# MarQuisCheshire/Pets-Face-Recognition

Measured on AMD Instinct MI355X. Metric: FE train images/sec @224^2 bs=256/GPU, higher is better.
Workload: dtype bf16; 1 GPU; resnet50 FE + ArcFace(s=64,m=0.5) + CE, 10000 ids, 224x224x3, fwd+bwd+SGD(momentum 0.9, param groups of the reference recipe); global_batch=256, per_gpu_batch=256, parallelism=dp1, rccl_ranks=0

## Files before the change

### include/pfr_hip.h

```cpp
#ifndef PFR_HIP_H
#define PFR_HIP_H
#include <stddef.h>
#include <stdint.h>

#ifdef __cplusplus
extern "C" {
#endif

#define PFR_F32 0
#define PFR_BF16 1
#define PFR_I8 2
#define PFR_OK 0
#define PFR_ERR_ARG (-1)
#define PFR_ERR_HIP (-2)
#define PFR_ERR_UNSUPPORTED (-3)

typedef void* pfr_stream_t;

const char* pfr_last_error(void);
int pfr_version(void);
int pfr_device_arch(char* buf, int buflen);
int pfr_set_tuning(const char* key, int value);
int pfr_get_tuning(const char* key, int* value);
int pfr_tuning_epoch(void);

int pfr_plan_thunk_index(const char* name);
void* pfr_plan_create(int n_events);
int pfr_plan_destroy(void* plan);
int pfr_plan_append(void* plan, int kind, int thunk, int ev, const unsigned long long* args, int nargs);
int pfr_plan_size(void* plan);
int pfr_plan_run(void* plan, int begin, int end, pfr_stream_t main_stream, pfr_stream_t side_stream, int hook_stops);

int pfr_conv2d_mtile(int N, int H, int W, int C, int Cout, int R, int S, int stride, int pad, int OH, int OW, int dtype,
                     int out_dtype, int fused_prologue);
int pfr_gemm_act_mtile(long M, int K, int N, int dtype);
int pfr_conv2d_fwd(const void* x, const void* w, void* y, int dtype, int out_dtype, int N, int H, int W, int C,
                   int Cout, int R, int S, int stride, int pad, int idil_log2, int OH, int OW, int ldy,
                   const float* bias, const void* residual, int accumulate, int out_relu, const float* pro_scale,
                   const float* pro_shift, int pro_relu, float* stats_part, pfr_stream_t stream);
int pfr_conv2d_dgrad_join(const void* dy, const void* wt, void* dx, int dtype, int N, int H, int W, int C, int Cout, int R,
                          int S, int pad, int idil_log2, int OH, int OW, const void* res, const unsigned char* res_mask,
                          pfr_stream_t stream);

int pfr_conv2d_dgrad_bn_parts(int dtype, int N, int H, int W, int C, int Cout, int R, int S, int idil_log2, int OH, int OW);
int pfr_conv2d_dgrad_bn(const void* dy, const void* wt, void* dx, int dtype, int N, int H, int W, int C, int Cout, int R, int S,
                        int pad, int idil_log2, int OH, int OW, const void* res, const unsigned char* res_mask, int accumulate,
                        const void* bn_x, const float* bn_coef, const unsigned char* bn_mask, float* bn_part, const void* bn2_x,
                        const float* bn2_coef, float* bn2_part, pfr_stream_t stream);

int pfr_conv2d_dgrad_bn_sub(const void* dy, const void* wt, void* dx, int dtype, int N, int H, int W, int C, int Cout, int OH, int OW,
                            const void* res_compact, const void* bn_x, const float* bn_coef, const unsigned char* bn_mask,
                            float* bn_part, pfr_stream_t stream);

int pfr_conv1x1_tail_mtile(int dtype, int N, int H, int W, int C, int Cout);
int pfr_conv1x1_stats(const void* x, const void* w, int dtype, int N, int H, int W, int C, int Cout, float* stats_part,
                      pfr_stream_t stream);
int pfr_conv1x1_bn_tail(const void* x, const void* w, void* y, unsigned char* mask, int dtype, int N, int H, int W, int C, int Cout,
                        const float* a1, const float* b1, const void* res, const float* a2, const float* b2, pfr_stream_t stream);

int pfr_conv2d_dgrad_bn_ex(const void* dy, const void* wt, void* dx, int dtype, int N, int H, int W, int C, int Cout, int R, int S,
                           int pad, int idil_log2, int OH, int OW, const void* res, const unsigned char* res_mask, int accumulate,
                           const void* bn_x, const float* bn_coef, const unsigned char* bn_mask, float* bn_part, const void* bn2_x,
                           const float* bn2_coef, float* bn2_part, int flags, pfr_stream_t stream);
int pfr_conv2d_dgrad_bn_sub_ex(const void* dy, const void* wt, void* dx, int dtype, int N, int H, int W, int C, int Cout, int OH, int OW,
                               const void* res_compact, const void* bn_x, const float* bn_coef, const unsigned char* bn_mask,
                               float* bn_part, int flags, pfr_stream_t stream);

int pfr_bn3_bwd_coef(const float* part, int nparts, const float* G1, const float* zsum, const void* W, int wdtype, const float* gamma,
                     const float* invstd, int C, int K, float count, float* dgamma, float* dbeta, float* coef, int accumulate,
                     pfr_stream_t stream);
int pfr_bn3_bwd_weights(const float* coef, const float* G1, const float* G2, const float* zsum, const void* W, int wdtype, int C, int K, float count,
                        float* dW, void* wa_t, void* S, float* bias, int accumulate, pfr_stream_t stream);
int pfr_conv1x1_dgrad2_bn_parts(int dtype, int N, int H, int W, int C1, int C2, int Cout);
int pfr_conv1x1_dgrad2_bn(const void* g, const void* z, const void* wcat, const float* bias, void* dx, int dtype, int N, int H, int W,
                          int C1, int C2, int Cout, const void* bn_x, const float* bn_coef, float* bn_part, pfr_stream_t stream);

int pfr_bn_stats_from_gram(const float* gram, const void* W, int dtype, int C, int K, float count, float* part, float eps, int* cancel_flag,
                           pfr_stream_t stream);
int pfr_bn_finalize_from_gram(const float* gram, const void* W, int dtype, int C, int K, float count, const float* gamma, const float* beta,
                              float eps, float momentum, float* running_mean, float* running_var, float* mean, float* invstd, float* scale,
                              float* shift, int* cancel_flag, pfr_stream_t stream);
long pfr_gram_ws_floats(long M, int Q);
int pfr_gram_colsum(const void* x, int dtype, long M, int Q, float* out, float* workspace, pfr_stream_t stream);

int pfr_conv2d_wgrad_splits(int M, int Cout, int KK);
int pfr_conv2d_wgrad(const void* x, const void* dy, float* dw, float* workspace, int dtype, int N, int H, int W, int C,
                     int Cout, int R, int S, int stride, int pad, int OH, int OW, int lddy, const float* pro_scale,
                     const float* pro_shift, int pro_relu, float scale, int accumulate, pfr_stream_t stream);

int pfr_nchw_to_nhwc(const float* x, void* y, int dtype, int N, int C, int H, int W, int Cp, pfr_stream_t stream);
int pfr_cast(const void* x, int src_dtype, void* y, int dst_dtype, size_t n, pfr_stream_t stream);
int pfr_weight_dgrad_layout(const void* w, void* wt, int dtype, int O, int R, int S, int I, pfr_stream_t stream);
int pfr_weight_dgrad_layout_batch(const void* descs, int n_layers, int dtype, pfr_stream_t stream);
int pfr_add(const void* a, const void* b, void* y, int dtype, size_t n, pfr_stream_t stream);
long pfr_colsum_ws_floats(long rows, int C);
int pfr_colsum(const void* x, int dtype, long rows, int C, float* out, int accumulate, float* workspace, pfr_stream_t stream);
int pfr_colsum_parts(int dtype, long rows, int C);
int pfr_colsum_partial(const void* x, int dtype, long rows, int C, float* workspace, pfr_stream_t stream);
int pfr_colsum_final_batch(const void* descs, int n, int max_C, pfr_stream_t stream);
int pfr_copy2d_f32(const float* src, int ld_src, float* dst, int ld_dst, long rows, int cols, float scale, int accumulate,
                   pfr_stream_t stream);

int pfr_colreduce_blocks(int C, int dtype, long rows);
int pfr_bn_stats(const void* x, int dtype, long rows, int C, float* part, pfr_stream_t stream);
long pfr_bn_stats_rows_per_part(int C, int dtype, long rows);
long pfr_bn_finalize_ws_floats(int nparts, int C);
int pfr_bn_finalize(const float* part, int nparts, long rows_per_part, int C, float count, const float* gamma,
                    const float* beta, float eps, float momentum, float* running_mean, float* running_var, float* mean,
                    float* invstd, float* scale, float* shift, float* workspace, pfr_stream_t stream);
int pfr_fold_bn(const void* descs, int ndesc, int dtype, pfr_stream_t stream);
int pfr_fold_bn_cached(const void* descs, int ndesc, int dtype, const float* master, size_t n_master, void* shadow,
                       unsigned long long* state, pfr_stream_t stream);
int pfr_bn_eval_coeff(int C, const float* gamma, const float* beta, const float* running_mean, const float* running_var,
                      float eps, float* scale, float* shift, pfr_stream_t stream);
int pfr_bn_act(const void* x1, const float* a1, const float* b1, const void* x2, const float* a2, const float* b2, void* y,
               int dtype, long rows, int C, int relu, pfr_stream_t stream);
int pfr_bn_act_mask(const void* x1, const float* a1, const float* b1, const void* x2, const float* a2, const float* b2,
                    void* y, unsigned char* mask, int dtype, long rows, int C, int relu, pfr_stream_t stream);
int pfr_bn_bwd_reduce(const void* dout, const void* out, const void* x, const float* mean, const float* invstd,
                      const float* scale, const float* shift, int mask_mode, int dtype, long rows, int C, float* part,
                      pfr_stream_t stream);
int pfr_bn_bwd_finalize(const float* part, int nparts, int C, float count, const float* gamma, const float* mean,
                        const float* invstd, float* dgamma, float* dbeta, float* coef, int accumulate, pfr_stream_t stream);
int pfr_bn_bwd_apply(const void* dout, const void* out, const void* x, const float* coef, const float* scale,
                     const float* shift, int mask_mode, void* dx, void* gres, int dtype, long rows, int C,
                     pfr_stream_t stream);

int pfr_bn_relu_maxpool_fwd(const void* x, const float* scale, const float* shift, void* y, uint8_t* idx, int dtype, int N,
                            int H, int W, int C, int relu, pfr_stream_t stream);
int pfr_maxpool_bwd(const void* dy, const uint8_t* idx, void* dz, int dtype, int N, int H, int W, int C, pfr_stream_t stream);
int pfr_avgpool_fwd(const void* x, void* y, int dtype, int N, int HW, int C, pfr_stream_t stream);
int pfr_avgpool_bwd(const void* dy, void* dx, int dtype, int N, int HW, int C, pfr_stream_t stream);

int pfr_s2d_input(const float* x, void* y, int dtype, int N, int C, int H, int W, int Cp, pfr_stream_t stream);
int pfr_s2d_weight(const float* w, void* ws, int dtype, int Cout, int C, int Cp, pfr_stream_t stream);
int pfr_s2d_wgrad(const float* dws, float* dw, int Cout, int C, int Cp, int accumulate, pfr_stream_t stream);
int pfr_transpose2d(const void* x, void* y, int dtype, int rows, int cols, pfr_stream_t stream);
int pfr_l2norm_dual(const float* x, void* xn_bf16, float* xn_f32, float* inv_norm, int rows, int D, float eps,
                    pfr_stream_t stream);
int pfr_l2norm_fwd(const void* x, int in_dtype, void* xn, void* xnT, int out_dtype, float* inv_norm, int rows, int D,
                   int ldt, float eps, pfr_stream_t stream);
int pfr_l2norm_bwd(const void* x, int in_dtype, const float* inv_norm, const float* dxn, void* dx, int out_dtype, int rows,
                   int D, int accumulate, pfr_stream_t stream);
int pfr_margin_ce(const float* cosv, const int64_t* label, int B, int C, int ldc, int mode, float s, float m, float gamma,
                  float grad_scale, const float* grad_scale_dev, float* logits, float* loss_rows, void* dcos, int dcos_dtype,
                  pfr_stream_t stream);
int pfr_margin_bwd(const float* cosv, const int64_t* label, int B, int C, int ldc, int mode, float s, float m,
                   const float* dlogits, void* dcos, int dcos_dtype, pfr_stream_t stream);
int pfr_mean(const float* x, float* out, int n, pfr_stream_t stream);

int pfr_sgd_step(float* p, const float* g, float* mom, void* shadow, int shadow_dtype, size_t n, float lr, float momentum,
                 float weight_decay, float grad_scale, int first_step, pfr_stream_t stream);
int pfr_adamw_step(float* p, const float* g, float* m, float* v, void* shadow, int shadow_dtype, size_t n, float lr,
                   float beta1, float beta2, float eps, float weight_decay, int step, float grad_scale, pfr_stream_t stream);
int pfr_sgd_step_clip(float* p, const float* g, float* mom, void* shadow, int shadow_dtype, size_t n, float lr, float momentum,
                      float weight_decay, float grad_scale, int first_step, const float* clip_coef, float clip_value,
                      pfr_stream_t stream);
int pfr_adamw_step_clip(float* p, const float* g, float* m, float* v, void* shadow, int shadow_dtype, size_t n, float lr,
                        float beta1, float beta2, float eps, float weight_decay, int step, float grad_scale,
                        const float* clip_coef, float clip_value, pfr_stream_t stream);
int pfr_grad_norm_chunk_elems(void);
int pfr_grad_norm(const void* segs, const int* chunk_seg, int nseg, long nchunks, float norm_p, float max_norm, double* ws,
                  float* out, pfr_stream_t stream);

int pfr_layernorm_fwd(const void* x, const float* gamma, const float* beta, void* y, float* mean, float* rstd, int dtype,
                      long rows, int C, float eps, pfr_stream_t stream);
int pfr_layernorm_bwd_blocks(long rows);
int pfr_layernorm_bwd(const void* dy, const void* x, const float* mean, const float* rstd, const float* gamma,
                      const void* dres, void* dx, float* part, int dtype, long rows, int C, pfr_stream_t stream);
int pfr_layernorm_bwd_dxsum(const void* dy, const void* x, const float* mean, const float* rstd, const float* gamma,
                            const void* dres, void* dx, float* part, float* dxsum_part, int dtype, long rows, int C,
                            pfr_stream_t stream);
int pfr_layernorm_bwd_dxsum_ok(int dtype, int C);
int pfr_gelu_fwd(const void* x, void* y, int dtype, size_t n, pfr_stream_t stream);
int pfr_gelu_bwd(const void* x, const void* dy, void* dx, int dtype, size_t n, pfr_stream_t stream);
long pfr_window_bias_table_floats(int window);
int pfr_window_bias_table(const float* pos, float* tab, int window, int shift, pfr_stream_t stream);
int pfr_window_bias_table_batch(const void* descs, int n, pfr_stream_t stream);
int pfr_window_attn_fwd(const void* qkv, const float* pos, void* out, int dtype, int B, int H, int W, int heads, int head_dim,
                        int window, int shift, float scale, pfr_stream_t stream);
int pfr_window_attn_bwd(const void* qkv, const float* pos, const void* dout, void* dqkv, float* dpos_part, int dtype, int B,
                        int H, int W, int heads, int head_dim, int window, int shift, float scale, pfr_stream_t stream);
int pfr_nhwc_to_nchw_f32(const float* x, float* y, int N, int C, int HW, int Cp, int accumulate, pfr_stream_t stream);

long pfr_topk_state_bytes(int rows, int K);
int pfr_topk_reset(void* state, int rows, int K, pfr_stream_t stream);
int pfr_topk_update(const float* scores, int rows, int ld, int n, int col0, int K, void* state, const int* self_idx,
                    pfr_stream_t stream);
int pfr_match_scores_filter(const void* q, const void* g, int dtype, int Q, int n, int D, int col0, int K, void* state,
                            void* cand, int cap, int exclude_self, pfr_stream_t stream);
int pfr_topk_merge(const void* cand, int cap, int rows, int K, void* state, pfr_stream_t stream);
int pfr_quantize_rows_i8(const float* x, void* q, int ldq, float* scale, float* xn_f32, float* inv_norm, int rows, int D, int normalize,
                         float eps, pfr_stream_t stream);
int pfr_match_scores_i8(const void* q, const float* q_scale, const void* g, const float* g_scale, int Q, int n, int Dp, float* out, int ld,
                        pfr_stream_t stream);
int pfr_match_scores_filter_i8(const void* q, const float* q_scale, const void* g, const float* g_scale, int Q, int n, int Dp, int col0,
                               int K, void* state, void* cand, int cap, int exclude_self, pfr_stream_t stream);
int pfr_topk_flags(const void* state, int rows, int K, int* out_host, pfr_stream_t stream);
int pfr_topk_finish(const void* state, int rows, int K, float* out_scores, int* out_idx, pfr_stream_t stream);
int pfr_topk_rescore(const float* q, const float* g, const float* g_scale, int rows, int D, const int* cand, int KC, int K,
                     float* out_scores, int* out_idx, pfr_stream_t stream);
int pfr_topk_rescore_cert(const float* q, const float* g, const float* g_scale, int rows, int D, const int* cand, const float* cand_scores,
                          int KC, int K, float* out_scores, int* out_idx, float* cert, pfr_stream_t stream);
int pfr_pair_similarity(const float* emb, int D, const long* idx_a, const long* idx_b, int P, float eps, float* out,
                        pfr_stream_t stream);

long pfr_pair_curve_ws_bytes(int P);
int pfr_pair_curve(const float* scores, const int* labels, int P, void* workspace, float* sorted_scores, int* cum_tp,
                   unsigned char* run_end, pfr_stream_t stream);

int pfr_card_centroids(const float* emb, const long* seg, int ncards, int D, float eps, float* cent32, void* cent,
                       int cent_dtype, pfr_stream_t stream);

int pfr_card_fuse_scores(float* head_scores, const float* body_scores, int rows, int ld, int n, int col0,
                         const unsigned char* q_flags, const unsigned char* g_flags, const float* thresholds, int n_types,
                         pfr_stream_t stream);

int pfr_augment_params(const int* flags, const float* angles, int N, int out_w, int out_h, int* records);
long pfr_augment_ws_bytes(int N, int H, int W);
int pfr_augment_train(const unsigned char* x, int N, int H, int W, int crop_h, int crop_w, int out_h, int out_w,
                      const int* records, float* y, void* ws, pfr_stream_t stream);

int pfr_gemm_act(const void* x, const void* w, void* y, int dtype, long M, int K, int N, const float* bias, int act,
                 void* y2, pfr_stream_t stream);
int pfr_gemm_act_colstats(const void* x, const void* w, void* y, int dtype, long M, int K, int N, const float* bias, int act,
                          void* y2, float* stats_part, pfr_stream_t stream);
int pfr_gemm_act_colsum_parts(long M, int K, int N, int dtype);
int pfr_gemm_act_colsums(const void* x, const void* w, void* y, int dtype, long M, int K, int N, void* y2, float* sums_part,
                         pfr_stream_t stream);

int pfr_comm_unique_id(void* id128);
void* pfr_comm_init(int rank, int world, const void* id128);
int pfr_comm_allreduce(void* comm, void* buf, size_t count, int dtype, int average, pfr_stream_t stream);
int pfr_comm_destroy(void* comm);

#ifdef __cplusplus
}
#endif
#endif
```

### pets-face-recognition_amd/_hip/lib.py

```python
import ctypes
import os
import re

PFR_F32, PFR_BF16, PFR_I8 = 0, 1, 2

_HERE = os.path.dirname(os.path.abspath(__file__))
_PKG = os.path.dirname(_HERE)
_ROOT = os.path.dirname(_PKG)
LIB_PATH = os.environ.get("PFR_LIB_PATH") or os.path.join(_PKG, "csrc", "libpfr_hip.so")
HEADER_PATH = os.path.join(_ROOT, "include", "pfr_hip.h")


class PfrError(RuntimeError):
    pass


_CTYPES = {
    "int": ctypes.c_int,
    "long": ctypes.c_long,
    "size_t": ctypes.c_size_t,
    "float": ctypes.c_float,
    "pfr_stream_t": ctypes.c_void_p,
}


def _ctype_of(decl: str):
    decl = decl.strip()
    if "*" in decl:
        if decl.replace("const", "").strip().startswith("char"):
            return ctypes.c_char_p
        return ctypes.c_void_p
    base = decl.replace("const", "").split()[0]
    return _CTYPES[base]


def parse_header(path=HEADER_PATH):
    src = open(path).read()
    src = re.sub(r"/\*.*?\*/", "", src, flags=re.S)
    src = re.sub(r"//[^\n]*", "", src)
    protos = {}
    for m in re.finditer(r"(const\s+char\s*\*|void\s*\*|int|long)\s+(pfr_\w+)\s*\(([^)]*)\)\s*;", src):
        ret, name, args = m.group(1), m.group(2), m.group(3).strip()
        restype = ctypes.c_char_p if "char" in ret else (ctypes.c_void_p if "void" in ret else (ctypes.c_long if ret == "long" else ctypes.c_int))
        argtypes, argnames = [], []
        if args and args != "void":
            for a in args.split(","):
                a = a.strip()
                nm = re.search(r"(\w+)$", a).group(1)
                argnames.append(nm)
                argtypes.append(_ctype_of(a[: -len(nm)]))
        protos[name] = (restype, argtypes, argnames)
    return protos


class _Lib:
    def __init__(self):
        self._dll = None
        self._protos = None

    def _load(self):
        if self._dll is not None:
            return
        if not os.path.exists(LIB_PATH):
            raise PfrError(
                f"{LIB_PATH} not found: build it with `python -c 'import __graft_entry__ as g; g.build()'` "
                f"(or pets-face-recognition_amd/csrc/build.sh). There is no CPU/PyTorch fallback for the HIP path."
            )
        import torch
        self._dll = ctypes.CDLL(LIB_PATH)
        self._protos = parse_header()
        for name, (restype, argtypes, _names) in self._protos.items():
            try:
                fn = getattr(self._dll, name)
            except AttributeError as e:
                raise PfrError(f"libpfr_hip.so does not export {name} declared in include/pfr_hip.h") from e
            fn.restype = restype
            fn.argtypes = argtypes
        for item in filter(None, (os.environ.get("PFR_TUNING") or "").replace(";", ",").split(",")):
            k, _, v = item.partition("=")
            if self._dll.pfr_set_tuning(k.strip().encode(), int(v)) != 0:
                raise PfrError(f"PFR_TUNING: {self._dll.pfr_last_error().decode()}")

    def __getattr__(self, name):
        if name.startswith("_"):
            raise AttributeError(name)
        self._load()
        if name not in self._protos:
            raise AttributeError(f"{name} is not declared in include/pfr_hip.h")
        fn = getattr(self._dll, name)
        if self._protos[name][0] is ctypes.c_int and name not in _NO_CHECK:
            def checked(*args, _fn=fn, _name=name):
                tr = _TRACER[0]
                if tr is not None:
                    tr.before(_name, args)
                rc = _fn(*args)
                if tr is not None:
                    tr.after(_name, args)
                if rc != 0:
                    raise PfrError(f"{_name} failed (rc={rc}): {self._dll.pfr_last_error().decode()}")
                return rc
            checked.__name__ = name
            setattr(self, name, checked)
            return checked
        setattr(self, name, fn)
        return fn

    def symbols(self):
        self._load()
        return dict(self._protos)


_NO_CHECK = {"pfr_version", "pfr_grad_norm_chunk_elems", "pfr_conv1x1_dgrad2_bn_parts", "pfr_tuning_epoch", "pfr_gram_ws_floats", "pfr_conv1x1_tail_mtile", "pfr_bn_stats_rows_per_part", "pfr_bn_finalize_ws_floats", "pfr_topk_state_bytes", "pfr_layernorm_bwd_blocks", "pfr_window_bias_table_floats", "pfr_colsum_ws_floats", "pfr_conv2d_mtile", "pfr_gemm_act_mtile", "pfr_conv2d_dgrad_bn_parts", "pfr_plan_thunk_index", "pfr_plan_size", "pfr_plan_run", "pfr_conv2d_wgrad_splits", "pfr_colreduce_blocks", "pfr_match_ws_bytes", "pfr_pair_curve_ws_bytes", "pfr_augment_ws_bytes", "pfr_colsum_parts", "pfr_layernorm_bwd_dxsum_ok", "pfr_gemm_act_colsum_parts"}

lib = _Lib()

_TRACER = [None]


def set_tracer(tracer):
    _TRACER[0] = tracer


class EventTracer:

    def __init__(self):
        import torch
        self._torch = torch
        self.records = []

    def before(self, name, args):
        e = self._torch.cuda.Event(enable_timing=True)
        e.record()
        self._cur = e

    def after(self, name, args):
        e = self._torch.cuda.Event(enable_timing=True)
        e.record()
        self.records.append((name, args, self._cur, e))

    def summary(self):
        self._torch.cuda.synchronize()
        out = {}
        for name, args, a, b in self.records:
            o = out.setdefault(name, [0, 0.0])
            o[0] += 1
            o[1] += a.elapsed_time(b)
        return out


def is_available() -> bool:
    return os.path.exists(LIB_PATH)


def dtype_id(torch_dtype_):
    import torch

    if torch_dtype_ == torch.float32:
        return PFR_F32
    if torch_dtype_ == torch.bfloat16:
        return PFR_BF16
    if torch_dtype_ == torch.int8:
        return PFR_I8
    raise PfrError(f"unsupported dtype {torch_dtype_}")


def torch_dtype(dtype_id_):
    import torch

    return {PFR_F32: torch.float32, PFR_BF16: torch.bfloat16, PFR_I8: torch.int8}[dtype_id_]
```

### pets-face-recognition_amd/_hip/ops.py

```python
import torch

from .lib import lib, dtype_id, PFR_F32, PFR_BF16, PfrError


def _p(t):
    return 0 if t is None else t.data_ptr()


def _stream():
    return torch.cuda.current_stream().cuda_stream


def _chk(t, name):
    if t is not None:
        if not t.is_cuda:
            raise PfrError(f"{name}: expected a CUDA (HIP) tensor — the HIP path has no CPU fallback")
        if not t.is_contiguous():
            raise PfrError(f"{name}: tensor must be contiguous")


def kpack(dtype):
    return 8 if dtype == torch.bfloat16 else 4


def conv_out_hw(H, W, R, S, stride, pad):
    return (H + 2 * pad - R) // stride + 1, (W + 2 * pad - S) // stride + 1


def conv2d_fwd(x, w, stride=1, pad=0, idil_log2=0, out_hw=None, out=None, out_dtype=None, bias=None, accumulate=False,
               out_relu=False, pro=None, stats=False, stats_buf=None, residual=None):
    _chk(x, "x"); _chk(w, "w")
    N, H, W, C = x.shape
    Cout, R, S, Cw = w.shape
    assert Cw == C, (Cw, C)
    if out_hw is None:
        OH, OW = conv_out_hw(H, W, R, S, stride, pad)
    else:
        OH, OW = out_hw
    odt = out_dtype or x.dtype
    if out is None:
        out = torch.empty((N, OH, OW, Cout), dtype=odt, device=x.device)
    ldy = out.shape[-1]
    M = N * OH * OW
    part = None
    if stats:
        mt = lib.pfr_conv2d_mtile(N, H, W, C, Cout, R, S, stride, pad, OH, OW, dtype_id(x.dtype), dtype_id(out.dtype), int(pro is not None))
        nt = (M + mt - 1) // mt
        conv2d_fwd.last_mt = mt
        part = stats_buf if stats_buf is not None else torch.empty((nt, 2, Cout), dtype=torch.float32, device=x.device)
        assert part.numel() >= nt * 2 * Cout
    ps = psh = None
    prelu = 0
    if pro is not None:
        ps, psh, prelu = pro
    lib.pfr_conv2d_fwd(_p(x), _p(w), _p(out), dtype_id(x.dtype), dtype_id(out.dtype), N, H, W, C, Cout, R, S, stride, pad,
                       idil_log2, OH, OW, ldy, _p(bias), _p(residual), int(accumulate), int(out_relu), _p(ps), _p(psh), int(prelu),
                       _p(part), _stream())
    return out, part


def conv2d_dgrad(dy, wt, in_hw, stride, pad, R, S, out=None, accumulate=False, out_dtype=None):
    H, W = in_hw
    log2 = {1: 0, 2: 1, 4: 2}[stride]
    y, _ = conv2d_fwd(dy, wt, stride=1, pad=R - 1 - pad, idil_log2=log2, out_hw=(H, W), out=out, accumulate=accumulate,
                      out_dtype=out_dtype)
    return y


def _conv2d_dgrad_geom_check(dy, in_hw, stride, pad, R):
    return True


def weight_dgrad_layout(w, out=None):
    O, R, S, I = w.shape
    if out is None:
        out = torch.empty((I, R, S, O), dtype=w.dtype, device=w.device)
    lib.pfr_weight_dgrad_layout(_p(w), _p(out), dtype_id(w.dtype), O, R, S, I, _stream())
    return out


def conv2d_wgrad(x, dy, R, S, stride, pad, out=None, pro=None, scale=1.0, accumulate=False, workspace=None):
    _chk(x, "x"); _chk(dy, "dy")
    N, H, W, C = x.shape
    _, OH, OW, Cout = dy.shape
    if out is None:
        out = torch.empty((Cout, R, S, C), dtype=torch.float32, device=x.device)
    KK = R * S * C
    splits = lib.pfr_conv2d_wgrad_splits(N * OH * OW, Cout, KK)
    need = splits * Cout * KK
    if workspace is None or workspace.numel() < need:
        workspace = torch.empty(need, dtype=torch.float32, device=x.device)
    ps = psh = None
    prelu = 0
    if pro is not None:
        ps, psh, prelu = pro
    lib.pfr_conv2d_wgrad(_p(x), _p(dy), _p(out), _p(workspace), dtype_id(x.dtype), N, H, W, C, Cout, R, S, stride, pad, OH,
                         OW, Cout, _p(ps), _p(psh), int(prelu), float(scale), int(accumulate), _stream())
    return out


def nchw_to_nhwc(x, dtype, cpad):
    N, C, H, W = x.shape
    assert x.dtype == torch.float32
    _chk(x, "x")
    y = torch.empty((N, H, W, cpad), dtype=dtype, device=x.device)
    lib.pfr_nchw_to_nhwc(_p(x), _p(y), dtype_id(dtype), N, C, H, W, cpad, _stream())
    return y


def cast(x, dtype, out=None):
    if out is None:
        out = torch.empty(x.shape, dtype=dtype, device=x.device)
    lib.pfr_cast(_p(x), dtype_id(x.dtype), _p(out), dtype_id(dtype), x.numel(), _stream())
    return out


def add(a, b, out=None):
    if out is None:
        out = torch.empty_like(a)
    lib.pfr_add(_p(a), _p(b), _p(out), dtype_id(a.dtype), a.numel(), _stream())
    return out


def colsum(x, out=None, accumulate=False):
    rows, C = x.shape
    if out is None:
        out = torch.empty(C, dtype=torch.float32, device=x.device)
    nws = lib.pfr_colsum_ws_floats(rows, C)
    ws = torch.empty(nws, dtype=torch.float32, device=x.device) if nws else None
    lib.pfr_colsum(_p(x), dtype_id(x.dtype), rows, C, _p(out), int(accumulate), _p(ws), _stream())
    return out


def bn_stats(x):
    C = x.shape[-1]
    rows = x.numel() // C
    nb = lib.pfr_colreduce_blocks(C, dtype_id(x.dtype), rows)
    part = torch.empty((nb, 2, C), dtype=torch.float32, device=x.device)
    lib.pfr_bn_stats(_p(x), dtype_id(x.dtype), rows, C, _p(part), _stream())
    return part, lib.pfr_bn_stats_rows_per_part(C, dtype_id(x.dtype), rows)


def bn_finalize(part, rows_per_part, count, gamma, beta, eps, momentum, running_mean, running_var, out=None):
    C = part.shape[-1]
    nparts = part.numel() // (2 * C)
    if out is None:
        out = torch.empty((4, C), dtype=torch.float32, device=part.device)
    nws = lib.pfr_bn_finalize_ws_floats(nparts, C)
    ws = torch.empty(nws, dtype=torch.float32, device=part.device) if nws else None
    lib.pfr_bn_finalize(_p(part), nparts, int(rows_per_part), C, float(count), _p(gamma), _p(beta), float(eps), float(momentum),
                        _p(running_mean), _p(running_var), _p(out[0]), _p(out[1]), _p(out[2]), _p(out[3]), _p(ws), _stream())
    return out


def bn_eval_coeff(gamma, beta, running_mean, running_var, eps, out=None):
    C = running_mean.numel()
    if out is None:
        out = torch.empty((2, C), dtype=torch.float32, device=running_mean.device)
    lib.pfr_bn_eval_coeff(C, _p(gamma), _p(beta), _p(running_mean), _p(running_var), float(eps), _p(out[0]), _p(out[1]), _stream())
    return out


def bn_act(x1, a1, b1, x2=None, a2=None, b2=None, relu=True, out=None, want_mask=False):
    C = x1.shape[-1]
    rows = x1.numel() // C
    if out is None:
        out = torch.empty_like(x1)
    if want_mask:
        kp = 8 if x1.dtype == torch.bfloat16 else 4
        mask = torch.empty((rows, C // kp), dtype=torch.uint8, device=x1.device)
        lib.pfr_bn_act_mask(_p(x1), _p(a1), _p(b1), _p(x2), _p(a2), _p(b2), _p(out), _p(mask), dtype_id(x1.dtype), rows, C,
                            int(relu), _stream())
        return out, mask
    lib.pfr_bn_act(_p(x1), _p(a1), _p(b1), _p(x2), _p(a2), _p(b2), _p(out), dtype_id(x1.dtype), rows, C, int(relu), _stream())
    return out


def bn_bwd(dout, x, mean, invstd, gamma, count, mask_mode=0, out_act=None, scale=None, shift=None, dgamma=None,
           dbeta=None, want_gres=False, dx=None, gres=None, accumulate_param_grads=False):
    C = x.shape[-1]
    rows = x.numel() // C
    did = dtype_id(x.dtype)
    nb = lib.pfr_colreduce_blocks(C, did, rows)
    part = torch.empty((nb, 2, C), dtype=torch.float32, device=x.device)
    lib.pfr_bn_bwd_reduce(_p(dout), _p(out_act), _p(x), _p(mean), _p(invstd), _p(scale), _p(shift), mask_mode, did, rows, C,
                          _p(part), _stream())
    coef = torch.empty((3, C), dtype=torch.float32, device=x.device)
    if dgamma is None:
        dgamma = torch.empty(C, dtype=torch.float32, device=x.device)
    if dbeta is None:
        dbeta = torch.empty(C, dtype=torch.float32, device=x.device)
    lib.pfr_bn_bwd_finalize(_p(part), nb, C, float(count), _p(gamma), _p(mean), _p(invstd), _p(dgamma), _p(dbeta), _p(coef),
                            int(accumulate_param_grads), _stream())
    if dx is None:
        dx = torch.empty_like(x)
    if want_gres and gres is None:
        gres = torch.empty_like(x)
    lib.pfr_bn_bwd_apply(_p(dout), _p(out_act), _p(x), _p(coef), _p(scale), _p(shift), mask_mode, _p(dx), _p(gres), did, rows,
                         C, _stream())
    return dx, gres, dgamma, dbeta


def bn_relu_maxpool_fwd(x, scale, shift, relu=True, want_idx=True):
    N, H, W, C = x.shape
    OH, OW = (H + 2 - 3) // 2 + 1, (W + 2 - 3) // 2 + 1
    y = torch.empty((N, OH, OW, C), dtype=x.dtype, device=x.device)
    idx = torch.empty((N, OH, OW, C), dtype=torch.uint8, device=x.device) if want_idx else None
    lib.pfr_bn_relu_maxpool_fwd(_p(x), _p(scale), _p(shift), _p(y), _p(idx), dtype_id(x.dtype), N, H, W, C, int(relu), _stream())
    return y, idx


def maxpool_bwd(dy, idx, in_hw):
    N, OH, OW, C = dy.shape
    H, W = in_hw
    dz = torch.empty((N, H, W, C), dtype=dy.dtype, device=dy.device)
    lib.pfr_maxpool_bwd(_p(dy), _p(idx), _p(dz), dtype_id(dy.dtype), N, H, W, C, _stream())
    return dz


def avgpool_fwd(x):
    N, H, W, C = x.shape
    y = torch.empty((N, C), dtype=x.dtype, device=x.device)
    lib.pfr_avgpool_fwd(_p(x), _p(y), dtype_id(x.dtype), N, H * W, C, _stream())
    return y


def avgpool_bwd(dy, hw):
    N, C = dy.shape
    H, W = hw
    dx = torch.empty((N, H, W, C), dtype=dy.dtype, device=dy.device)
    lib.pfr_avgpool_bwd(_p(dy), _p(dx), dtype_id(dy.dtype), N, H * W, C, _stream())
    return dx


def l2norm_fwd(x, out_dtype, want_t=False, ldt=None, xn=None, xnT=None, inv=None):
    rows, D = x.shape
    if xn is None:
        xn = torch.empty((rows, D), dtype=out_dtype, device=x.device)
    if want_t and xnT is None:
        xnT = torch.zeros((D, ldt or rows), dtype=out_dtype, device=x.device)
    if inv is None:
        inv = torch.empty(rows, dtype=torch.float32, device=x.device)
    lib.pfr_l2norm_fwd(_p(x), dtype_id(x.dtype), _p(xn), _p(xnT), dtype_id(out_dtype), _p(inv), rows, D,
                       0 if xnT is None else xnT.shape[1], 1e-12, _stream())
    return xn, xnT, inv


def l2norm_bwd(x, inv, dxn, out_dtype, out=None, accumulate=False):
    rows, D = x.shape
    assert dxn.dtype == torch.float32
    if out is None:
        out = torch.empty((rows, D), dtype=out_dtype, device=x.device)
    lib.pfr_l2norm_bwd(_p(x), dtype_id(x.dtype), _p(inv), _p(dxn), _p(out), dtype_id(out.dtype), rows, D, int(accumulate), _stream())
    return out


MARGIN_MODES = {"arc": 0, "arc_easy": 1, "cos": 2, "none": 3}


def margin_ce(cosv, label, C, mode, s, m, gamma=0.0, grad_scale=1.0, grad_scale_dev=None, want_logits=True, dcos_dtype=None, dcos=None,
              logits=None, loss_rows=None):
    B, ldc = cosv.shape
    assert cosv.dtype == torch.float32 and label.dtype == torch.int64
    if want_logits and logits is None:
        logits = torch.empty((B, C), dtype=torch.float32, device=cosv.device)
    if loss_rows is None:
        loss_rows = torch.empty(B, dtype=torch.float32, device=cosv.device)
    if dcos_dtype is not None and dcos is None:
        dcos = torch.zeros((B, ldc), dtype=dcos_dtype, device=cosv.device)
    lib.pfr_margin_ce(_p(cosv), _p(label), B, C, ldc, MARGIN_MODES[mode], float(s), float(m), float(gamma), float(grad_scale),
                      _p(grad_scale_dev), _p(logits), _p(loss_rows), _p(dcos), PFR_F32 if dcos is None else dtype_id(dcos.dtype), _stream())
    return logits, loss_rows, dcos


def mean(x, out=None):
    if out is None:
        out = torch.empty((), dtype=torch.float32, device=x.device)
    lib.pfr_mean(_p(x), _p(out), x.numel(), _stream())
    return out


def sgd_step(p, g, mom, shadow, lr, momentum, weight_decay, grad_scale=1.0, first_step=False):
    lib.pfr_sgd_step(_p(p), _p(g), _p(mom), _p(shadow), PFR_F32 if shadow is None else dtype_id(shadow.dtype), p.numel(),
                     float(lr), float(momentum), float(weight_decay), float(grad_scale), int(first_step), _stream())


def adamw_step(p, g, m, v, shadow, lr, beta1, beta2, eps, weight_decay, step, grad_scale=1.0):
    lib.pfr_adamw_step(_p(p), _p(g), _p(m), _p(v), _p(shadow), PFR_F32 if shadow is None else dtype_id(shadow.dtype), p.numel(),
                       float(lr), float(beta1), float(beta2), float(eps), float(weight_decay), int(step), float(grad_scale),
                       _stream())


def sgd_step_clip(p, g, mom, shadow, lr, momentum, weight_decay, clip_coef, clip_value, grad_scale=1.0, first_step=False):
    lib.pfr_sgd_step_clip(_p(p), _p(g), _p(mom), _p(shadow), PFR_F32 if shadow is None else dtype_id(shadow.dtype), p.numel(),
                          float(lr), float(momentum), float(weight_decay), float(grad_scale), int(first_step), _p(clip_coef),
                          float(clip_value), _stream())


def adamw_step_clip(p, g, m, v, shadow, lr, beta1, beta2, eps, weight_decay, step, clip_coef, clip_value, grad_scale=1.0):
    lib.pfr_adamw_step_clip(_p(p), _p(g), _p(m), _p(v), _p(shadow), PFR_F32 if shadow is None else dtype_id(shadow.dtype),
                            p.numel(), float(lr), float(beta1), float(beta2), float(eps), float(weight_decay), int(step),
                            float(grad_scale), _p(clip_coef), float(clip_value), _stream())


def grad_norm(segs, chunk_seg, nseg, nchunks, norm_p, max_norm, ws, out):
    assert ws.dtype == torch.float64 and ws.numel() >= nchunks + nseg and out.dtype == torch.float32 and out.numel() >= nseg + 2
    lib.pfr_grad_norm(_p(segs), _p(chunk_seg), int(nseg), int(nchunks), float(norm_p), float(max_norm), _p(ws), _p(out), _stream())


def grad_norm_chunk_elems():
    return lib.pfr_grad_norm_chunk_elems()
```

### pets-face-recognition_amd/csrc/pfr_api.hip

```cpp
#include "pfr_common.h"
#include <stdarg.h>
#include <string.h>

static thread_local char g_err[512] = "";

thread_local hipEvent_t pfr_tls_stop_event = nullptr;

void pfr_set_error(const char* fmt, ...) {
  va_list ap;
  va_start(ap, fmt);
  vsnprintf(g_err, sizeof(g_err), fmt, ap);
  va_end(ap);
}

extern "C" const char* pfr_last_error(void) { return g_err; }
extern "C" int pfr_version(void) { return 100; }

extern "C" int pfr_device_arch(char* buf, int buflen) {
  int dev = 0;
  if (hipGetDevice(&dev) != hipSuccess) { pfr_set_error("pfr_device_arch: no HIP device"); return PFR_ERR_HIP; }
  hipDeviceProp_t prop;
  if (hipGetDeviceProperties(&prop, dev) != hipSuccess) { pfr_set_error("pfr_device_arch: hipGetDeviceProperties failed"); return PFR_ERR_HIP; }
  strncpy(buf, prop.gcnArchName, buflen - 1);
  buf[buflen - 1] = 0;
  return PFR_OK;
}

static const struct { const char* name; int def; } kKnobs[KNOB_COUNT] = {
  {"igemm_p", 1}, {"igemm_ptile", -1}, {"igemm_pkch", 8}, {"igemm_ppf", 0}, {"igemm_tile", -1}, {"igemm_kch", 0}, {"igemm_big", 1},
  {"sconv", 1}, {"sconv3", 1}, {"bnb", 0}, {"swgrad", 1}, {"wgrad_big", 0}, {"wgrad_tile", -1}, {"wgrad_splits", 0}, {"wgrad9", 1},
  {"wgrad9_slots", 256}, {"attn_mfma", 1}, {"bnb_tile3", 0}, {"slin", 1}, {"slin_np", 0}, {"match_order", 1},
  {"ln_rb", 4}, {"sstem", 1}, {"igemm_dma", 0x101}, {"igemm_krot", 0},
};
int g_pfr_knob[KNOB_COUNT];
static const bool g_knobs_ready = [] { for (int k = 0; k < KNOB_COUNT; ++k) g_pfr_knob[k] = kKnobs[k].def; return true; }();
static int g_tuning_epoch = 0;
extern "C" int pfr_tuning_epoch(void) { return g_tuning_epoch; }
extern "C" int pfr_set_tuning(const char* key, int value) {
  PFR_CHECK_ARG(key, "pfr_set_tuning: null key");
  for (int k = 0; k < KNOB_COUNT; ++k)
    if (!strcmp(kKnobs[k].name, key)) {
      if (g_pfr_knob[k] != value) { g_pfr_knob[k] = value; ++g_tuning_epoch; }
      return PFR_OK;
    }
  pfr_set_error("pfr_set_tuning: unknown key %s", key);
  return PFR_ERR_ARG;
}
extern "C" int pfr_get_tuning(const char* key, int* value) {
  PFR_CHECK_ARG(key && value, "pfr_get_tuning: null pointer");
  for (int k = 0; k < KNOB_COUNT; ++k)
    if (!strcmp(kKnobs[k].name, key)) { *value = g_pfr_knob[k]; return PFR_OK; }
  pfr_set_error("pfr_get_tuning: unknown key %s", key);
  return PFR_ERR_ARG;
}
```

### pets-face-recognition_amd/csrc/pfr_common.h

```cpp
#pragma once
#include <hip/hip_runtime.h>
#include <stdint.h>
#include <stdio.h>

typedef __bf16 bf16_t;
typedef __bf16 bf16x8 __attribute__((ext_vector_type(8)));
typedef __bf16 bf16x4 __attribute__((ext_vector_type(4)));
typedef __bf16 bf16x2 __attribute__((ext_vector_type(2)));
typedef float f32x2 __attribute__((ext_vector_type(2)));
typedef float f32x4 __attribute__((ext_vector_type(4)));
typedef float f32x16 __attribute__((ext_vector_type(16)));
typedef uint32_t u32x4 __attribute__((ext_vector_type(4)));
typedef int32_t i32x4 __attribute__((ext_vector_type(4)));
typedef int32_t i32x16 __attribute__((ext_vector_type(16)));
typedef uint32_t u32x2 __attribute__((ext_vector_type(2)));

#define PFR_F32 0
#define PFR_BF16 1
#define PFR_I8 2

#define PFR_OK 0
#define PFR_ERR_ARG (-1)
#define PFR_ERR_HIP (-2)
#define PFR_ERR_UNSUPPORTED (-3)

void pfr_set_error(const char* fmt, ...);

enum PfrKnob {
  KNOB_IGEMM_P,
  KNOB_IGEMM_PTILE,
  KNOB_IGEMM_PKCH,
  KNOB_IGEMM_PPF,
  KNOB_IGEMM_TILE,
  KNOB_IGEMM_KCH,
  KNOB_IGEMM_BIG,
  KNOB_SCONV,
  KNOB_SCONV3,
  KNOB_BNB,
  KNOB_SWGRAD,
  KNOB_WGRAD_BIG,
  KNOB_WGRAD_TILE,
  KNOB_WGRAD_SPLITS,
  KNOB_WGRAD9,
  KNOB_WGRAD9_SLOTS,
  KNOB_ATTN_MFMA,
  KNOB_BNB_TILE3,
  KNOB_SLIN,
  KNOB_SLIN_NP,
  KNOB_MATCH_ORDER,
  KNOB_LN_RB,
  KNOB_SSTEM,
  KNOB_IGEMM_DMA,
  KNOB_IGEMM_KROT,
  KNOB_COUNT
};
extern int g_pfr_knob[KNOB_COUNT];
static inline int pfr_knob(int k) { return g_pfr_knob[k]; }

#include <atomic>
static inline bool pfr_lds_attr_needed(std::atomic<unsigned long long>& done, unsigned long long* bit) {
  int dev = 0;
  (void)hipGetDevice(&dev);
  *bit = 1ull << (dev & 63);
  return !(done.load(std::memory_order_acquire) & *bit);
}
#define PFR_MAX_LDS_ONCE(done, bytes, ...)                                                                          \
  do {                                                                                                              \
    unsigned long long bit_;                                                                                        \
    if (pfr_lds_attr_needed(done, &bit_)) {                                                                         \
      const void* fns_[] = {__VA_ARGS__};                                                                           \
      for (const void* f_ : fns_) (void)hipFuncSetAttribute(f_, hipFuncAttributeMaxDynamicSharedMemorySize, bytes); \
      done.fetch_or(bit_, std::memory_order_release);                                                               \
    }                                                                                                               \
  } while (0)

extern thread_local hipEvent_t pfr_tls_stop_event;

#define PFR_CHECK_ARG(cond, ...)            \
  do {                                      \
    if (!(cond)) {                          \
      pfr_set_error(__VA_ARGS__);           \
      return PFR_ERR_ARG;                   \
    }                                       \
  } while (0)

#define PFR_CHECK_LAUNCH()                                            \
  do {                                                                \
    hipError_t e_ = hipGetLastError();                                \
    if (e_ != hipSuccess) {                                           \
      pfr_set_error("%s:%d: %s", __FILE__, __LINE__, hipGetErrorString(e_)); \
      return PFR_ERR_HIP;                                             \
    }                                                                 \
  } while (0)

__device__ __forceinline__ void gelu_cdf_pdf(float z, float& cdf, float& pdf) {
  const float ax = fabsf(z) * 0.70710678118654752f;
  const float ex = __expf(-ax * ax);
  const float t = __builtin_amdgcn_rcpf(fmaf(0.3275911f, ax, 1.f));
  float p = fmaf(1.061405429f, t, -1.453152027f);
  p = fmaf(p, t, 1.421413741f);
  p = fmaf(p, t, -0.284496736f);
  p = fmaf(p, t, 0.254829592f);
  const float half_erfc = 0.5f * p * t * ex;
  cdf = z >= 0.f ? 1.f - half_erfc : half_erfc;
  pdf = 0.3989422804014327f * ex;
}

template <typename T> struct DT;
template <> struct DT<float> {
  static constexpr int KPACK = 4;
  static constexpr int ID = PFR_F32;
};
template <> struct DT<bf16_t> {
  static constexpr int KPACK = 8;
  static constexpr int ID = PFR_BF16;
};
template <> struct DT<int8_t> {
  static constexpr int KPACK = 16;
  static constexpr int ID = PFR_I8;
};

__device__ __forceinline__ float to_f32(float v) { return v; }
__device__ __forceinline__ float to_f32(bf16_t v) { return (float)v; }
template <typename T> __device__ __forceinline__ T from_f32(float v);
template <> __device__ __forceinline__ float from_f32<float>(float v) { return v; }
template <> __device__ __forceinline__ bf16_t from_f32<bf16_t>(float v) { return (bf16_t)v; }

template <typename T> struct Chunk;
template <> struct Chunk<float> {
  static constexpr int N = 4;
  __device__ __forceinline__ static void unpack(const u32x4& c, float* f) {
    f[0] = __uint_as_float(c[0]); f[1] = __uint_as_float(c[1]);
    f[2] = __uint_as_float(c[2]); f[3] = __uint_as_float(c[3]);
  }
  __device__ __forceinline__ static u32x4 pack(const float* f) {
    u32x4 c;
    c[0] = __float_as_uint(f[0]); c[1] = __float_as_uint(f[1]);
    c[2] = __float_as_uint(f[2]); c[3] = __float_as_uint(f[3]);
    return c;
  }
};
template <> struct Chunk<bf16_t> {
  static constexpr int N = 8;
  __device__ __forceinline__ static void unpack(const u32x4& c, float* f) {
#pragma unroll
    for (int i = 0; i < 4; ++i) {
      f[2 * i] = __uint_as_float(c[i] << 16);
      f[2 * i + 1] = __uint_as_float(c[i] & 0xffff0000u);
    }
  }
  __device__ __forceinline__ static u32x4 pack(const float* f) {
    u32x4 c;
#pragma unroll
    for (int i = 0; i < 4; ++i) {
      bf16x2 p;
      p[0] = (bf16_t)f[2 * i];
      p[1] = (bf16_t)f[2 * i + 1];
      c[i] = __builtin_bit_cast(uint32_t, p);
    }
    return c;
  }
};

__device__ __forceinline__ uint32_t fkey(float s) {
  const uint32_t u = __float_as_uint(s);
  return (u & 0x80000000u) ? ~u : (u | 0x80000000u);
}
__device__ __forceinline__ float fkey_inv(uint32_t k) {
  const uint32_t u = (k & 0x80000000u) ? (k & 0x7fffffffu) : ~k;
  return __uint_as_float(u);
}
struct TopkState {
  unsigned long long* cur;
  int* cur_n;
  int* flags;
  uint32_t* thrk;
  int* ccnt;
};
__host__ __device__ __forceinline__ TopkState topk_state(void* state, int rows, int K) {
  TopkState t;
  char* b = reinterpret_cast<char*>(state);
  t.cur = reinterpret_cast<unsigned long long*>(b);
  t.cur_n = reinterpret_cast<int*>(b + (size_t)rows * K * 8);
  t.flags = t.cur_n + rows;
  t.thrk = reinterpret_cast<uint32_t*>(reinterpret_cast<char*>(t.flags) + 64);
  t.ccnt = reinterpret_cast<int*>(t.thrk + rows);
  return t;
}

__device__ __forceinline__ u32x4 ld16(const void* p) { return *reinterpret_cast<const u32x4*>(p); }
__device__ __forceinline__ void st16(void* p, const u32x4& v) { *reinterpret_cast<u32x4*>(p) = v; }
#ifdef PFR_NO_NT
__device__ __forceinline__ u32x4 ld16_nt(const void* p) { return *reinterpret_cast<const u32x4*>(p); }
#else
__device__ __forceinline__ u32x4 ld16_nt(const void* p) { return __builtin_nontemporal_load(reinterpret_cast<const u32x4*>(p)); }
#endif

__device__ __forceinline__ float wave_sum(float v) {
#pragma unroll
  for (int o = 32; o > 0; o >>= 1) v += __shfl_xor(v, o, 64);
  return v;
}
__device__ __forceinline__ float wave_max(float v) {
#pragma unroll
  for (int o = 32; o > 0; o >>= 1) v = fmaxf(v, __shfl_xor(v, o, 64));
  return v;
}

struct FastDiv {
  uint32_t d, mul, shr;
};
static inline FastDiv make_fastdiv(uint32_t d) {
  FastDiv f;
  f.d = d;
  if (d == 1) { f.mul = 0; f.shr = 0; return f; }
  uint32_t l = 0;
  while ((1u << l) < d) ++l;
  uint64_t m = ((uint64_t(1) << (32 + l)) + d - 1) / d;
  f.mul = (uint32_t)(m - (uint64_t(1) << 32));
  f.shr = l;
  return f;
}
__device__ __forceinline__ uint32_t fdiv(uint32_t n, const FastDiv& f) {
  if (f.d == 1) return n;
  uint32_t t = __umulhi(n, f.mul);
  return (uint32_t)(((uint64_t)t + n) >> f.shr);
}

__device__ __forceinline__ uint32_t xcd_remap(uint32_t bid, uint32_t nblk) {
  const uint32_t NX = 8;
  uint32_t xcd = bid % NX, q = nblk / NX, r = nblk % NX;
  uint32_t base = (xcd < r) ? xcd * (q + 1) : r * (q + 1) + (xcd - r) * q;
  return base + bid / NX;
}
```

### pets-face-recognition_amd/csrc/pfr_elementwise.hip

```cpp
#include "pfr_common.h"
#include <hip/hip_ext.h>

template <typename T>
__global__ void nchw_to_nhwc_kernel(const float* __restrict__ x, T* __restrict__ y, int N, int C, int HW, int Cp) {
  constexpr int KP = DT<T>::KPACK;
  const size_t i = (size_t)blockIdx.x * blockDim.x + threadIdx.x;
  if (Cp % KP == 0) {
    const int cpr = Cp / KP;
    if (i >= (size_t)N * HW * cpr) return;
    const int chunk = (int)(i % cpr);
    const size_t np = i / cpr, n = np / HW, pix = np % HW;
    const int c0 = chunk * KP;
    float v[KP];
    if (C == 3) {
      const float* src = x + n * 3 * HW + pix;
      const float r = src[0], g = src[HW], b = src[2 * (size_t)HW];
#pragma unroll
      for (int e = 0; e < KP; ++e) v[e] = 0.f;
      v[0] = r; v[1] = g; v[2] = b;
      st16(y + np * Cp + c0, Chunk<T>::pack(v));
      return;
    }
#pragma unroll
    for (int e = 0; e < KP; ++e) v[e] = x[(n * C + min(c0 + e, C - 1)) * HW + pix];
// ... 829 lines not shown
  const int kp = dtype == PFR_BF16 ? 8 : 4;
  PFR_CHECK_ARG(C % kp == 0, "pfr_bn_bwd_apply: C %% %d != 0", kp);
  ColGeom g = col_geom(C, kp, (size_t)rows, 256);
  hipEvent_t stop = pfr_tls_stop_event;
  pfr_tls_stop_event = nullptr;
#define PFR_BNA(TT, M)                                                                                                                        \
  do {                                                                                                                                        \
    if (stop) hipExtLaunchKernelGGL((bn_bwd_apply_kernel<TT, M>), dim3(g.gx, g.gy), dim3(256), 0, st, nullptr, stop, 0, (const TT*)dout, (const TT*)out, (const TT*)x, coef, scale, shift, (TT*)dx, (TT*)gres, (size_t)rows, C, g.cw, g.rl, g.cpr); \
    else hipLaunchKernelGGL((bn_bwd_apply_kernel<TT, M>), dim3(g.gx, g.gy), dim3(256), 0, st, (const TT*)dout, (const TT*)out, (const TT*)x, coef, scale, shift, (TT*)dx, (TT*)gres, (size_t)rows, C, g.cw, g.rl, g.cpr); \
  } while (0)
#define PFR_BNA4(TT) do { switch (mask_mode) { case 0: PFR_BNA(TT, 0); break; case 1: PFR_BNA(TT, 1); break; case 2: PFR_BNA(TT, 2); break; default: PFR_BNA(TT, 3); } } while (0)
  if (dtype == PFR_BF16) PFR_BNA4(bf16_t); else PFR_BNA4(float);
#undef PFR_BNA4
#undef PFR_BNA
  PFR_CHECK_LAUNCH();
  return PFR_OK;
}

template <typename T>
__global__ __launch_bounds__(256) void transpose2d_kernel(const T* __restrict__ x, T* __restrict__ y, int rows, int cols) {
  __shared__ T tile[64][65];
  const int r0 = blockIdx.y * 64, c0 = blockIdx.x * 64;
  const int tx = threadIdx.x & 63, ty = threadIdx.x >> 6;
  for (int i = ty; i < 64; i += 4)
    if (r0 + i < rows && c0 + tx < cols) tile[i][tx] = x[(size_t)(r0 + i) * cols + c0 + tx];
  __syncthreads();
  for (int i = ty; i < 64; i += 4)
    if (c0 + i < cols && r0 + tx < rows) y[(size_t)(c0 + i) * rows + r0 + tx] = tile[tx][i];
}
extern "C" int pfr_transpose2d(const void* x, void* y, int dtype, int rows, int cols, hipStream_t st) {
  PFR_CHECK_ARG(x && y && rows > 0 && cols > 0, "pfr_transpose2d: bad args");
  const dim3 grid((cols + 63) / 64, (rows + 63) / 64);
  if (dtype == PFR_BF16) hipLaunchKernelGGL(transpose2d_kernel<bf16_t>, grid, dim3(256), 0, st, (const bf16_t*)x, (bf16_t*)y, rows, cols);
  else hipLaunchKernelGGL(transpose2d_kernel<float>, grid, dim3(256), 0, st, (const float*)x, (float*)y, rows, cols);
  PFR_CHECK_LAUNCH();
  return PFR_OK;
}

template <typename T>
__global__ __launch_bounds__(256) void s2d_input_kernel(const float* __restrict__ x, T* __restrict__ y, int N, int C, int H, int W,
                                                        int Cp) {
  const int H2 = H >> 1, W2 = W >> 1;
  const size_t npix = (size_t)N * H2 * W2;
  for (size_t i = (size_t)blockIdx.x * 256 + threadIdx.x; i < npix; i += (size_t)gridDim.x * 256) {
    const int j2 = (int)(i % W2);
    const int i2 = (int)((i / W2) % H2);
    const size_t n = i / ((size_t)W2 * H2);
    constexpr int KP = DT<T>::KPACK;
    T* o = y + i * Cp;
    for (int c0 = 0; c0 < Cp; c0 += KP) {
      float v[KP];
#pragma unroll
      for (int e = 0; e < KP; ++e) {
        const int ch = c0 + e;
        v[e] = 0.f;
        if (ch < 4 * C) {
          const int pq = ch / C, c = ch - pq * C;
          v[e] = x[((n * C + c) * H + 2 * i2 + (pq >> 1)) * W + 2 * j2 + (pq & 1)];
        }
      }
      st16(o + c0, Chunk<T>::pack(v));
    }
  }
}
__global__ __launch_bounds__(256) void s2d_input3_kernel(const float* __restrict__ x, bf16_t* __restrict__ y, int N, int H, int W) {
  const int H2 = H >> 1, W4 = W >> 2;
  const size_t npair = (size_t)N * H2 * W4;
  for (size_t i = (size_t)blockIdx.x * 256 + threadIdx.x; i < npair; i += (size_t)gridDim.x * 256) {
    const int j4 = (int)(i % W4);
    const int i2 = (int)((i / W4) % H2);
    const size_t n = i / ((size_t)W4 * H2);
    f32x4 v[3][2];
#pragma unroll
    for (int c = 0; c < 3; ++c)
#pragma unroll
      for (int r = 0; r < 2; ++r)
        v[c][r] = __builtin_nontemporal_load(reinterpret_cast<const f32x4*>(x + ((n * 3 + c) * H + 2 * i2 + r) * W + 4 * j4));
    bf16_t* o = y + ((n * H2 + i2) * (size_t)(W >> 1) + 2 * j4) * 16;
#pragma unroll
    for (int px = 0; px < 2; ++px) {
      float a[8], b[8];
#pragma unroll
      for (int ch = 0; ch < 16; ++ch) {
        float val = 0.f;
        if (ch < 12) {
          const int pq = ch / 3, c = ch - pq * 3;
          val = v[c][pq >> 1][2 * px + (pq & 1)];
        }
        if (ch < 8) a[ch] = val; else b[ch - 8] = val;
      }
      st16(o + px * 16, Chunk<bf16_t>::pack(a));
      st16(o + px * 16 + 8, Chunk<bf16_t>::pack(b));
    }
  }
}
template <typename T>
__global__ void s2d_weight_kernel(const float* __restrict__ w, T* __restrict__ ws, int Co, int C, int Cp) {
  const int i = blockIdx.x * blockDim.x + threadIdx.x;
  if (i >= Co * 16 * Cp) return;
  const int ch = i % Cp, b = (i / Cp) % 4, a = (i / (4 * Cp)) % 4, co = i / (16 * Cp);
  float v = 0.f;
  if (ch < 4 * C) {
    const int pq = ch / C, c = ch - pq * C;
    const int r = 2 * a + (pq >> 1) - 1, s = 2 * b + (pq & 1) - 1;
    if (r >= 0 && r < 7 && s >= 0 && s < 7) v = w[((co * 7 + r) * 7 + s) * C + c];
  }
  ws[i] = from_f32<T>(v);
}
__global__ void s2d_wgrad_kernel(const float* __restrict__ dws, float* __restrict__ dw, int Co, int C, int Cp, int accumulate) {
  const int i = blockIdx.x * blockDim.x + threadIdx.x;
  if (i >= Co * 49 * C) return;
  const int c = i % C, s = (i / C) % 7, r = (i / (7 * C)) % 7, co = i / (49 * C);
  const int a = (r + 1) >> 1, p = (r + 1) & 1, b = (s + 1) >> 1, q = (s + 1) & 1;
  const float v = dws[((co * 4 + a) * 4 + b) * Cp + (p * 2 + q) * C + c];
  dw[i] = accumulate ? dw[i] + v : v;
}
extern "C" int pfr_s2d_input(const float* x, void* y, int dtype, int N, int C, int H, int W, int Cp, hipStream_t st) {
  PFR_CHECK_ARG(x && y && N > 0 && C > 0 && H > 0 && W > 0 && (H % 2) == 0 && (W % 2) == 0 && Cp >= 4 * C && Cp % (dtype == PFR_BF16 ? 8 : 4) == 0, "pfr_s2d_input: bad geometry");
  const size_t npix = (size_t)N * (H / 2) * (W / 2);
  unsigned blocks = (unsigned)((npix + 255) / 256);
  if (blocks > 16384) blocks = 16384;
  if (dtype == PFR_BF16 && C == 3 && Cp == 16 && W % 4 == 0 && H % 2 == 0) {
    const size_t npair = npix / 2;
    unsigned b2 = (unsigned)((npair + 255) / 256);
    if (b2 > 16384) b2 = 16384;
    hipLaunchKernelGGL(s2d_input3_kernel, dim3(b2), dim3(256), 0, st, x, (bf16_t*)y, N, H, W);
  } else if (dtype == PFR_BF16) hipLaunchKernelGGL(s2d_input_kernel<bf16_t>, dim3(blocks), dim3(256), 0, st, x, (bf16_t*)y, N, C, H, W, Cp);
  else hipLaunchKernelGGL(s2d_input_kernel<float>, dim3(blocks), dim3(256), 0, st, x, (float*)y, N, C, H, W, Cp);
  PFR_CHECK_LAUNCH();
  return PFR_OK;
}
extern "C" int pfr_s2d_weight(const float* w, void* ws, int dtype, int Cout, int C, int Cp, hipStream_t st) {
  PFR_CHECK_ARG(w && ws && Cout > 0 && C > 0 && Cp >= 4 * C, "pfr_s2d_weight: bad args");
  const int n = Cout * 16 * Cp;
  if (dtype == PFR_BF16) hipLaunchKernelGGL(s2d_weight_kernel<bf16_t>, dim3((n + 255) / 256), dim3(256), 0, st, w, (bf16_t*)ws, Cout, C, Cp);
  else hipLaunchKernelGGL(s2d_weight_kernel<float>, dim3((n + 255) / 256), dim3(256), 0, st, w, (float*)ws, Cout, C, Cp);
  PFR_CHECK_LAUNCH();
  return PFR_OK;
}
extern "C" int pfr_s2d_wgrad(const float* dws, float* dw, int Cout, int C, int Cp, int accumulate, hipStream_t st) {
  PFR_CHECK_ARG(dws && dw && Cout > 0 && C > 0 && Cp >= 4 * C, "pfr_s2d_wgrad: bad args");
  const int n = Cout * 49 * C;
  hipLaunchKernelGGL(s2d_wgrad_kernel, dim3((n + 255) / 256), dim3(256), 0, st, dws, dw, Cout, C, Cp, accumulate);
  PFR_CHECK_LAUNCH();
  return PFR_OK;
}

template <typename T>
__global__ void add_kernel(const T* __restrict__ a, const T* __restrict__ b, T* __restrict__ y, size_t nchunks) {
  constexpr int KP = DT<T>::KPACK;
  size_t i = (size_t)blockIdx.x * blockDim.x + threadIdx.x;
  const size_t stride = (size_t)gridDim.x * blockDim.x;
  for (; i < nchunks; i += stride) {
    float f[KP], g[KP];
    Chunk<T>::unpack(ld16(a + i * KP), f);
    Chunk<T>::unpack(ld16(b + i * KP), g);
#pragma unroll
    for (int e = 0; e < KP; ++e) f[e] += g[e];
    st16(y + i * KP, Chunk<T>::pack(f));
  }
}
extern "C" int pfr_add(const void* a, const void* b, void* y, int dtype, size_t n, hipStream_t st) {
  PFR_CHECK_ARG(a && b && y, "pfr_add: null pointer");
  const int kp = dtype == PFR_BF16 ? 8 : 4;
  PFR_CHECK_ARG(n % kp == 0, "pfr_add: n %% %d != 0", kp);
  const size_t nch = n / kp;
  unsigned blocks = (unsigned)((nch + 255) / 256);
  if (blocks > 8192) blocks = 8192;
  if (dtype == PFR_BF16)
    hipLaunchKernelGGL(add_kernel<bf16_t>, dim3(blocks), dim3(256), 0, st, (const bf16_t*)a, (const bf16_t*)b, (bf16_t*)y, nch);
  else
    hipLaunchKernelGGL(add_kernel<float>, dim3(blocks), dim3(256), 0, st, (const float*)a, (const float*)b, (float*)y, nch);
  PFR_CHECK_LAUNCH();
  return PFR_OK;
}

template <typename T>
__global__ __launch_bounds__(256) void bn_relu_maxpool_fwd_kernel(const T* __restrict__ x, const float* __restrict__ scale,
                                                                  const float* __restrict__ shift, T* __restrict__ y,
                                                                  uint8_t* __restrict__ idx, int N, int H, int W, int C,
                                                                  int OH, int OW, int relu) {
  constexpr int KP = DT<T>::KPACK;
  const int cpr = C / KP;
  const size_t nch = (size_t)N * OH * OW * cpr;
  size_t i = (size_t)blockIdx.x * blockDim.x + threadIdx.x;
  const size_t stride = (size_t)gridDim.x * blockDim.x;
  for (; i < nch; i += stride) {
    const int cc = (int)(i % cpr);
    size_t pix = i / cpr;
    const int ow = (int)(pix % OW); pix /= OW;
    const int oh = (int)(pix % OH);
    const int n = (int)(pix / OH);
    float best[KP], sc[KP], sh[KP];
    int bi[KP];
#pragma unroll
    for (int e = 0; e < KP; ++e) {
      best[e] = -INFINITY; bi[e] = 0;
      sc[e] = scale ? scale[cc * KP + e] : 1.f;
      sh[e] = shift ? shift[cc * KP + e] : 0.f;
    }
    u32x4 tv[9];
    bool tok[9];
#pragma unroll
    for (int t = 0; t < 9; ++t) {
      const int ih = oh * 2 - 1 + t / 3, iw = ow * 2 - 1 + t % 3;
      tok[t] = (unsigned)ih < (unsigned)H && (unsigned)iw < (unsigned)W;
      const int ihc = min(max(ih, 0), H - 1), iwc = min(max(iw, 0), W - 1);
      tv[t] = ld16(x + (((size_t)n * H + ihc) * W + iwc) * C + cc * KP);
    }
#pragma unroll
    for (int t = 0; t < 9; ++t) {
      float f[KP];
      Chunk<T>::unpack(tv[t], f);
#pragma unroll
      for (int e = 0; e < KP; ++e) {
        float z = fmaf(f[e], sc[e], sh[e]);
        if (relu) z = fmaxf(z, 0.f);
        z = to_f32(from_f32<T>(z));
        if (tok[t] && z > best[e]) { best[e] = z; bi[e] = t; }
      }
    }
    st16(y + i * KP, Chunk<T>::pack(best));
    if (idx) {
      if constexpr (KP == 8) {
        uint64_t pk = 0;
#pragma unroll
        for (int e = 0; e < 8; ++e) pk |= (uint64_t)bi[e] << (8 * e);
        *reinterpret_cast<uint64_t*>(idx + i * 8) = pk;
      } else {
        uint32_t pk = 0;
#pragma unroll
        for (int e = 0; e < 4; ++e) pk |= (uint32_t)bi[e] << (8 * e);
        *reinterpret_cast<uint32_t*>(idx + i * 4) = pk;
      }
    }
  }
}

extern "C" int pfr_bn_relu_maxpool_fwd(const void* x, const float* scale, const float* shift, void* y, uint8_t* idx,
                                       int dtype, int N, int H, int W, int C, int relu, hipStream_t st) {
  PFR_CHECK_ARG(x && y, "pfr_bn_relu_maxpool_fwd: null pointer");
  const int kp = dtype == PFR_BF16 ? 8 : 4;
  PFR_CHECK_ARG(C % kp == 0, "pfr_bn_relu_maxpool_fwd: C %% %d != 0", kp);
  const int OH = (H + 2 - 3) / 2 + 1, OW = (W + 2 - 3) / 2 + 1;
  const size_t nch = (size_t)N * OH * OW * (C / kp);
  unsigned blocks = (unsigned)((nch + 255) / 256);
  if (blocks > 16384) blocks = 16384;
  if (dtype == PFR_BF16)
    hipLaunchKernelGGL(bn_relu_maxpool_fwd_kernel<bf16_t>, dim3(blocks), dim3(256), 0, st, (const bf16_t*)x, scale, shift, (bf16_t*)y, idx, N, H, W, C, OH, OW, relu);
  else
    hipLaunchKernelGGL(bn_relu_maxpool_fwd_kernel<float>, dim3(blocks), dim3(256), 0, st, (const float*)x, scale, shift, (float*)y, idx, N, H, W, C, OH, OW, relu);
  PFR_CHECK_LAUNCH();
  return PFR_OK;
}

template <typename T>
__global__ __launch_bounds__(256) void maxpool_bwd_kernel(const T* __restrict__ dy, const uint8_t* __restrict__ idx,
                                                          T* __restrict__ dz, int N, int H, int W, int C, int OH, int OW) {
  constexpr int KP = DT<T>::KPACK;
  const int cpr = C / KP;
  const size_t nch = (size_t)N * H * W * cpr;
  size_t i = (size_t)blockIdx.x * blockDim.x + threadIdx.x;
  const size_t stride = (size_t)gridDim.x * blockDim.x;
  for (; i < nch; i += stride) {
    const int cc = (int)(i % cpr);
    size_t pix = i / cpr;
    const int w = (int)(pix % W); pix /= W;
    const int h = (int)(pix % H);
    const int n = (int)(pix / H);
    float acc[KP];
#pragma unroll
    for (int e = 0; e < KP; ++e) acc[e] = 0.f;
    const int oh0 = (h + 1) >> 1, r0 = h + 1 - 2 * oh0, ow0 = (w + 1) >> 1, s0 = w + 1 - 2 * ow0;
    u32x4 gv[4];
    uint64_t pk[4];
    int tap[4];
    bool ok[4];
#pragma unroll
    for (int q = 0; q < 4; ++q) {
      const int dh = q >> 1, dw = q & 1;
      const int oh = oh0 - dh, ow = ow0 - dw;
      const int r = r0 + 2 * dh, sx = s0 + 2 * dw;
      ok[q] = oh >= 0 && oh < OH && ow >= 0 && ow < OW && r < 3 && sx < 3;
      tap[q] = r * 3 + sx;
      const int ohc = min(max(oh, 0), OH - 1), owc = min(max(ow, 0), OW - 1);
      const size_t o = (((size_t)n * OH + ohc) * OW + owc) * cpr + cc;
      gv[q] = ld16(dy + o * KP);
      if constexpr (KP == 8) pk[q] = *reinterpret_cast<const uint64_t*>(idx + o * 8);
      else pk[q] = *reinterpret_cast<const uint32_t*>(idx + o * 4);
    }
#pragma unroll
    for (int q = 0; q < 4; ++q) {
      float g[KP];
      Chunk<T>::unpack(gv[q], g);
#pragma unroll
      for (int e = 0; e < KP; ++e)
        acc[e] += (ok[q] && (int)((pk[q] >> (8 * e)) & 0xff) == tap[q]) ? g[e] : 0.f;
    }
    st16(dz + i * KP, Chunk<T>::pack(acc));
  }
}

template <typename T>
__global__ __launch_bounds__(256) void maxpool_bwd2x2_kernel(const T* __restrict__ dy, const uint8_t* __restrict__ idx,
                                                             T* __restrict__ dz, int N, int H, int W, int C, int OH, int OW) {
  constexpr int KP = DT<T>::KPACK;
  const int cpr = C / KP, H2 = H >> 1, W2 = W >> 1;
  const size_t nblk = (size_t)N * H2 * W2 * cpr;
  size_t i = (size_t)blockIdx.x * blockDim.x + threadIdx.x;
  const size_t stride = (size_t)gridDim.x * blockDim.x;
  for (; i < nblk; i += stride) {
    const int cc = (int)(i % cpr);
    size_t t = i / cpr;
    const int b = (int)(t % W2); t /= W2;
    const int a = (int)(t % H2);
    const int n = (int)(t / H2);
    u32x4 gv[4];
    uint64_t pk[4];
    bool ok[4];
#pragma unroll
    for (int q = 0; q < 4; ++q) {
      const int oh = a + (q >> 1), ow = b + (q & 1);
      ok[q] = oh < OH && ow < OW;
      const size_t o = (((size_t)n * OH + min(oh, OH - 1)) * OW + min(ow, OW - 1)) * cpr + cc;
      gv[q] = ld16(dy + o * KP);
      if constexpr (KP == 8) pk[q] = *reinterpret_cast<const uint64_t*>(idx + o * 8);
      else pk[q] = *reinterpret_cast<const uint32_t*>(idx + o * 4);
    }
    float g[4][KP];
#pragma unroll
    for (int q = 0; q < 4; ++q) Chunk<T>::unpack(gv[q], g[q]);
    constexpr int NWIN[4] = {1, 2, 2, 4};
    constexpr int WIN[4][4] = {{0, 0, 0, 0}, {1, 0, 0, 0}, {2, 0, 0, 0}, {3, 2, 1, 0}};
    constexpr int TAP[4][4] = {{4, 0, 0, 0}, {3, 5, 0, 0}, {1, 7, 0, 0}, {0, 2, 6, 8}};
#pragma unroll
    for (int px = 0; px < 4; ++px) {
      float acc[KP];
#pragma unroll
      for (int e = 0; e < KP; ++e) acc[e] = 0.f;
#pragma unroll
      for (int k = 0; k < NWIN[px]; ++k) {
        const int q = WIN[px][k], tap = TAP[px][k];
#pragma unroll
        for (int e = 0; e < KP; ++e) acc[e] += (ok[q] && (int)((pk[q] >> (8 * e)) & 0xff) == tap) ? g[q][e] : 0.f;
      }
      const size_t o = (((size_t)n * H + 2 * a + (px >> 1)) * W + 2 * b + (px & 1)) * cpr + cc;
      st16(dz + o * KP, Chunk<T>::pack(acc));
    }
  }
}

extern "C" int pfr_maxpool_bwd(const void* dy, const uint8_t* idx, void* dz, int dtype, int N, int H, int W, int C,
                               hipStream_t st) {
  PFR_CHECK_ARG(dy && idx && dz, "pfr_maxpool_bwd: null pointer");
  const int kp = dtype == PFR_BF16 ? 8 : 4;
  const int OH = (H + 2 - 3) / 2 + 1, OW = (W + 2 - 3) / 2 + 1;
  const size_t nch = (size_t)N * H * W * (C / kp);
  unsigned blocks = (unsigned)((nch + 255) / 256);
  if (blocks > 16384) blocks = 16384;
  if (H % 2 == 0 && W % 2 == 0) {
    unsigned b2 = (unsigned)((nch / 4 + 255) / 256);
    if (b2 > 16384) b2 = 16384;
    if (dtype == PFR_BF16)
      hipLaunchKernelGGL(maxpool_bwd2x2_kernel<bf16_t>, dim3(b2), dim3(256), 0, st, (const bf16_t*)dy, idx, (bf16_t*)dz, N, H, W, C, OH, OW);
    else
      hipLaunchKernelGGL(maxpool_bwd2x2_kernel<float>, dim3(b2), dim3(256), 0, st, (const float*)dy, idx, (float*)dz, N, H, W, C, OH, OW);
    PFR_CHECK_LAUNCH();
    return PFR_OK;
  }
  if (dtype == PFR_BF16)
    hipLaunchKernelGGL(maxpool_bwd_kernel<bf16_t>, dim3(blocks), dim3(256), 0, st, (const bf16_t*)dy, idx, (bf16_t*)dz, N, H, W, C, OH, OW);
  else
    hipLaunchKernelGGL(maxpool_bwd_kernel<float>, dim3(blocks), dim3(256), 0, st, (const float*)dy, idx, (float*)dz, N, H, W, C, OH, OW);
  PFR_CHECK_LAUNCH();
  return PFR_OK;
}


template <typename T>
__global__ void avgpool_fwd_kernel(const T* __restrict__ x, T* __restrict__ y, int N, int HW, int C) {
  constexpr int KP = DT<T>::KPACK;
  const int cpr = C / KP;
  const size_t i = (size_t)blockIdx.x * blockDim.x + threadIdx.x;
  if (i >= (size_t)N * cpr) return;
  const int n = (int)(i / cpr), cc = (int)(i % cpr);
  float a[KP];
#pragma unroll
  for (int e = 0; e < KP; ++e) a[e] = 0.f;
  for (int p = 0; p < HW; ++p) {
    float f[KP];
    Chunk<T>::unpack(ld16(x + ((size_t)n * HW + p) * C + cc * KP), f);
#pragma unroll
    for (int e = 0; e < KP; ++e) a[e] += f[e];
  }
  const float inv = 1.f / HW;
#pragma unroll
  for (int e = 0; e < KP; ++e) a[e] *= inv;
  st16(y + i * KP, Chunk<T>::pack(a));
}
template <typename T>
__global__ void avgpool_bwd_kernel(const T* __restrict__ dy, T* __restrict__ dx, int N, int HW, int C) {
  constexpr int KP = DT<T>::KPACK;
  const int cpr = C / KP;
  const size_t nch = (size_t)N * HW * cpr;
  size_t i = (size_t)blockIdx.x * blockDim.x + threadIdx.x;
  const size_t stride = (size_t)gridDim.x * blockDim.x;
  const float inv = 1.f / HW;
  for (; i < nch; i += stride) {
    const int cc = (int)(i % cpr);
    const size_t n = i / ((size_t)HW * cpr);
    float f[KP];
    Chunk<T>::unpack(ld16(dy + (n * cpr + cc) * KP), f);
#pragma unroll
    for (int e = 0; e < KP; ++e) f[e] *= inv;
    st16(dx + i * KP, Chunk<T>::pack(f));
  }
}
extern "C" int pfr_avgpool_fwd(const void* x, void* y, int dtype, int N, int HW, int C, hipStream_t st) {
  PFR_CHECK_ARG(x && y, "pfr_avgpool_fwd: null pointer");
  const int kp = dtype == PFR_BF16 ? 8 : 4;
  const size_t n = (size_t)N * (C / kp);
  const unsigned blocks = (unsigned)((n + 63) / 64);
  if (dtype == PFR_BF16)
    hipLaunchKernelGGL(avgpool_fwd_kernel<bf16_t>, dim3(blocks), dim3(64), 0, st, (const bf16_t*)x, (bf16_t*)y, N, HW, C);
  else
    hipLaunchKernelGGL(avgpool_fwd_kernel<float>, dim3(blocks), dim3(64), 0, st, (const float*)x, (float*)y, N, HW, C);
  PFR_CHECK_LAUNCH();
  return PFR_OK;
}
extern "C" int pfr_avgpool_bwd(const void* dy, void* dx, int dtype, int N, int HW, int C, hipStream_t st) {
  PFR_CHECK_ARG(dy && dx, "pfr_avgpool_bwd: null pointer");
  const int kp = dtype == PFR_BF16 ? 8 : 4;
  const size_t nch = (size_t)N * HW * (C / kp);
  unsigned blocks = (unsigned)((nch + 255) / 256);
  if (blocks > 8192) blocks = 8192;
  if (dtype == PFR_BF16)
    hipLaunchKernelGGL(avgpool_bwd_kernel<bf16_t>, dim3(blocks), dim3(256), 0, st, (const bf16_t*)dy, (bf16_t*)dx, N, HW, C);
  else
    hipLaunchKernelGGL(avgpool_bwd_kernel<float>, dim3(blocks), dim3(256), 0, st, (const float*)dy, (float*)dx, N, HW, C);
  PFR_CHECK_LAUNCH();
  return PFR_OK;
}

template <typename T>
__global__ __launch_bounds__(256) void colsum_kernel(const T* __restrict__ x, float* __restrict__ out, int rows, int C,
                                                     int accumulate) {
  const int c = blockIdx.x * 64 + (threadIdx.x & 63);
  const int rl = threadIdx.x >> 6;
  __shared__ float l[4][64];
  float a = 0.f;
  if (c < C) {
    float a1 = 0.f, a2 = 0.f, a3 = 0.f;
    int r = rl;
    for (; r + 12 < rows; r += 16) {
      a += to_f32(x[(size_t)r * C + c]);
      a1 += to_f32(x[(size_t)(r + 4) * C + c]);
      a2 += to_f32(x[(size_t)(r + 8) * C + c]);
      a3 += to_f32(x[(size_t)(r + 12) * C + c]);
    }
    for (; r < rows; r += 4) a += to_f32(x[(size_t)r * C + c]);
    a = (a + a1) + (a2 + a3);
  }
  l[rl][threadIdx.x & 63] = a;
  __syncthreads();
  if (rl == 0 && c < C) {
    a = l[0][threadIdx.x] + l[1][threadIdx.x] + l[2][threadIdx.x] + l[3][threadIdx.x];
    out[c] = accumulate ? out[c] + a : a;
  }
}
__global__ __launch_bounds__(256) void colsum_final_kernel(const float* __restrict__ part, float* __restrict__ out, int n, int C,
                                                           int accumulate) {
  const int cl = threadIdx.x & 15, rl = threadIdx.x >> 4;
  const int c = blockIdx.x * 16 + cl;
  __shared__ float l[16][17];
  float a0 = 0.f, a1 = 0.f, a2 = 0.f, a3 = 0.f;
  if (c < C) {
    int r = rl;
    for (; r + 48 < n; r += 64) {
      a0 += part[(size_t)r * C + c];
      a1 += part[(size_t)(r + 16) * C + c];
      a2 += part[(size_t)(r + 32) * C + c];
      a3 += part[(size_t)(r + 48) * C + c];
    }
    for (; r < n; r += 16) a0 += part[(size_t)r * C + c];
  }
  l[rl][cl] = (a0 + a1) + (a2 + a3);
  __syncthreads();
  if (rl == 0 && c < C) {
    float a = 0.f;
#pragma unroll
    for (int r = 0; r < 16; ++r) a += l[r][cl];
    out[c] = accumulate ? out[c] + a : a;
  }
}
template <typename T>
__global__ __launch_bounds__(256) void colsum_part_kernel(const T* __restrict__ x, float* __restrict__ part, long rows, int C,
                                                          long rows_per_block) {
  const int c = blockIdx.x * 64 + (threadIdx.x & 63);
  const int rl = threadIdx.x >> 6;
  __shared__ float l[4][64];
  const long r0 = (long)blockIdx.y * rows_per_block;
  const long r1 = r0 + rows_per_block < rows ? r0 + rows_per_block : rows;
  float a0 = 0.f, a1 = 0.f;
  if (c < C) {
    long r = r0 + rl;
    for (; r + 28 < r1; r += 32) {
      float v[8];
#pragma unroll
      for (int k = 0; k < 8; ++k) v[k] = to_f32(x[(size_t)(r + 4 * k) * C + c]);
      __builtin_amdgcn_sched_barrier(0);
#pragma unroll
      for (int k = 0; k < 8; k += 2) { a0 += v[k]; a1 += v[k + 1]; }
    }
    for (; r + 4 < r1; r += 8) {
      a0 += to_f32(x[(size_t)r * C + c]);
      a1 += to_f32(x[(size_t)(r + 4) * C + c]);
    }
    for (; r < r1; r += 4) a0 += to_f32(x[(size_t)r * C + c]);
  }
  l[rl][threadIdx.x & 63] = a0 + a1;
  __syncthreads();
  if (rl == 0 && c < C) part[(size_t)blockIdx.y * C + c] = l[0][threadIdx.x] + l[1][threadIdx.x] + l[2][threadIdx.x] + l[3][threadIdx.x];
}

template <typename T>
__global__ __launch_bounds__(256) void colsum_chunk_kernel(const T* __restrict__ x, float* __restrict__ part, size_t rows, int C,
                                                           int cw, int rl, int cpr) {
  constexpr int KP = DT<T>::KPACK;
  extern __shared__ __attribute__((aligned(16))) float lds[];
  const int col = threadIdx.x % cw, rlane = threadIdx.x / cw;
  const int cglob = blockIdx.y * cw + col;
  float v[2][KP];
#pragma unroll
  for (int e = 0; e < KP; ++e) { v[0][e] = 0.f; v[1][e] = 0.f; }
  if (cglob < cpr) {
    const size_t step = (size_t)gridDim.x * rl;
    size_t r = (size_t)blockIdx.x * rl + rlane;
    for (; r + 3 * step < rows; r += 4 * step) {
      u32x4 q[4];
#pragma unroll
      for (int u = 0; u < 4; ++u) q[u] = ld16(x + (r + u * step) * C + cglob * KP);
#pragma unroll
      for (int u = 0; u < 4; ++u) {
        float a[KP];
        Chunk<T>::unpack(q[u], a);
#pragma unroll
        for (int e = 0; e < KP; ++e) v[u & 1][e] += a[e];
      }
    }
    for (; r < rows; r += step) {
      float a[KP];
      Chunk<T>::unpack(ld16(x + r * C + cglob * KP), a);
#pragma unroll
      for (int e = 0; e < KP; ++e) v[0][e] += a[e];
    }
  }
  float w[1][KP];
#pragma unroll
  for (int e = 0; e < KP; ++e) w[0][e] = v[0][e] + v[1][e];
  col_block_reduce<1, KP>(w, lds, cw, rl, col, rlane, cglob, cpr, part + (size_t)blockIdx.x * C, C);
}

static long colsum_blocks(long rows, int C) {
  if (rows <= 256) return 0;
  long want = 2048 / ((C + 63) / 64);
  if (want < 8) want = 8;
  const long maxb = (rows + 255) / 256;
  return want < maxb ? want : maxb;
}
extern "C" long pfr_colsum_ws_floats(long rows, int C) {
  const long a = colsum_blocks(rows, C);
  return (a > 512 ? a : (a ? 512 : 0)) * C;
}

extern "C" int pfr_colsum(const void* x, int dtype, long rows, int C, float* out, int accumulate, float* workspace,
                          hipStream_t st) {
  PFR_CHECK_ARG(x && out, "pfr_colsum: null pointer");
  const long nblk = (workspace || rows > 2048) ? colsum_blocks(rows, C) : 0;
  if (nblk > 0) {
    PFR_CHECK_ARG(workspace, "pfr_colsum: workspace of pfr_colsum_ws_floats(rows, C) floats required for %ld rows", rows);
    const int kp = dtype == PFR_BF16 ? 8 : 4;
    if (C % kp == 0) {
      ColGeom g = col_geom(C, kp, (size_t)rows, 512);
      const size_t shb = (size_t)256 * kp * sizeof(float);
      if (dtype == PFR_BF16)
        hipLaunchKernelGGL(colsum_chunk_kernel<bf16_t>, dim3(g.gx, g.gy), dim3(256), shb, st, (const bf16_t*)x, workspace, (size_t)rows, C, g.cw, g.rl, g.cpr);
      else
        hipLaunchKernelGGL(colsum_chunk_kernel<float>, dim3(g.gx, g.gy), dim3(256), shb, st, (const float*)x, workspace, (size_t)rows, C, g.cw, g.rl, g.cpr);
      PFR_CHECK_LAUNCH();
      hipLaunchKernelGGL(colsum_final_kernel, dim3((C + 15) / 16), dim3(256), 0, st, (const float*)workspace, out, g.gx, C, accumulate);
      PFR_CHECK_LAUNCH();
      return PFR_OK;
    }
    const long rpb = (rows + nblk - 1) / nblk;
    const dim3 grid((C + 63) / 64, (unsigned)nblk);
    if (dtype == PFR_BF16)
      hipLaunchKernelGGL(colsum_part_kernel<bf16_t>, grid, dim3(256), 0, st, (const bf16_t*)x, workspace, rows, C, rpb);
    else
      hipLaunchKernelGGL(colsum_part_kernel<float>, grid, dim3(256), 0, st, (const float*)x, workspace, rows, C, rpb);
    PFR_CHECK_LAUNCH();
    hipLaunchKernelGGL(colsum_final_kernel, dim3((C + 15) / 16), dim3(256), 0, st, (const float*)workspace, out, (int)nblk, C, accumulate);
    PFR_CHECK_LAUNCH();
    return PFR_OK;
  }
  if (dtype == PFR_BF16)
    hipLaunchKernelGGL(colsum_kernel<bf16_t>, dim3((C + 63) / 64), dim3(256), 0, st, (const bf16_t*)x, out, (int)rows, C, accumulate);
  else
    hipLaunchKernelGGL(colsum_kernel<float>, dim3((C + 63) / 64), dim3(256), 0, st, (const float*)x, out, (int)rows, C, accumulate);
  PFR_CHECK_LAUNCH();
  return PFR_OK;
}

extern "C" int pfr_colsum_parts(int dtype, long rows, int C) {
  const long nblk = colsum_blocks(rows, C);
  if (nblk <= 0) return 0;
  const int kp = dtype == PFR_BF16 ? 8 : 4;
  return C % kp == 0 ? col_geom(C, kp, (size_t)rows, 512).gx : (int)nblk;
}
extern "C" int pfr_colsum_partial(const void* x, int dtype, long rows, int C, float* workspace, hipStream_t st) {
  PFR_CHECK_ARG(x && workspace && colsum_blocks(rows, C) > 0, "pfr_colsum_partial: null pointer or too few rows (%ld) for the partial path", rows);
  const long nblk = colsum_blocks(rows, C);
  const int kp = dtype == PFR_BF16 ? 8 : 4;
  if (C % kp == 0) {
    ColGeom g = col_geom(C, kp, (size_t)rows, 512);
    const size_t shb = (size_t)256 * kp * sizeof(float);
    if (dtype == PFR_BF16)
      hipLaunchKernelGGL(colsum_chunk_kernel<bf16_t>, dim3(g.gx, g.gy), dim3(256), shb, st, (const bf16_t*)x, workspace, (size_t)rows, C, g.cw, g.rl, g.cpr);
    else
      hipLaunchKernelGGL(colsum_chunk_kernel<float>, dim3(g.gx, g.gy), dim3(256), shb, st, (const float*)x, workspace, (size_t)rows, C, g.cw, g.rl, g.cpr);
    PFR_CHECK_LAUNCH();
    return PFR_OK;
  }
  const long rpb = (rows + nblk - 1) / nblk;
  const dim3 grid((C + 63) / 64, (unsigned)nblk);
  if (dtype == PFR_BF16)
    hipLaunchKernelGGL(colsum_part_kernel<bf16_t>, grid, dim3(256), 0, st, (const bf16_t*)x, workspace, rows, C, rpb);
  else
    hipLaunchKernelGGL(colsum_part_kernel<float>, grid, dim3(256), 0, st, (const float*)x, workspace, rows, C, rpb);
  PFR_CHECK_LAUNCH();
  return PFR_OK;
}

struct ColsumDesc {
  const float* part;
  float* out;
  int n, C, accumulate;
  int mt, rows, pad;
};
__global__ __launch_bounds__(256) void colsum_final_batch_kernel(const ColsumDesc* __restrict__ descs) {
  const ColsumDesc d = descs[blockIdx.y];
  const int cl = threadIdx.x & 15, rl = threadIdx.x >> 4;
  const int c = blockIdx.x * 16 + cl;
  if (blockIdx.x * 16 >= d.C) return;
  __shared__ float l[16][17];
  float acc[8];
#pragma unroll
  for (int k = 0; k < 8; ++k) acc[k] = 0.f;
  if (c < d.C) {
    const size_t rs = d.mt > 0 ? (size_t)2 * d.C : (size_t)d.C;
    for (int r0 = rl; r0 < d.n; r0 += 16 * 8) {
      float v[8];
#pragma unroll
      for (int k = 0; k < 8; ++k) v[k] = d.part[(size_t)min(r0 + 16 * k, d.n - 1) * rs + c];
#pragma unroll
      for (int k = 0; k < 8; ++k) {
        const int r = r0 + 16 * k;
        if (r < d.n) acc[k] = d.mt > 0 ? fmaf(v[k], (float)min(d.mt, d.rows - r * d.mt), acc[k]) : acc[k] + v[k];
      }
    }
  }
  const float a0 = acc[0] + acc[1], a1 = acc[2] + acc[3], a2 = acc[4] + acc[5], a3 = acc[6] + acc[7];
  l[rl][cl] = (a0 + a1) + (a2 + a3);
  __syncthreads();
  if (rl == 0 && c < d.C) {
    float a = 0.f;
#pragma unroll
    for (int r = 0; r < 16; ++r) a += l[r][cl];
    d.out[c] = d.accumulate ? d.out[c] + a : a;
  }
}
// ... 328 lines not shown
```

### pets-face-recognition_amd/csrc/pfr_plan.hip

```cpp
#include "pfr_common.h"
#include <stdint.h>
#include <string.h>
#include <vector>

#include "../../include/pfr_hip.h"

struct PlanThunk {
  const char* name;
  int (*fn)(const unsigned long long*, void*);
};
static inline float u2f_(unsigned long long v) {
  const uint32_t b = (uint32_t)v;
  float f;
  memcpy(&f, &b, 4);
  return f;
}
#include "pfr_thunks_gen.inc"

struct PlanOp {
  int kind, thunk, ev, arg;
  unsigned long long a[30];
};
struct Plan {
  std::vector<PlanOp> ops;
  std::vector<hipEvent_t> events;
};

extern "C" int pfr_plan_thunk_index(const char* name) {
  const int n = (int)(sizeof(g_thunks) / sizeof(g_thunks[0]));
  for (int i = 0; i < n; ++i)
    if (!strcmp(g_thunks[i].name, name)) return i;
  return -1;
}

extern "C" void* pfr_plan_create(int n_events) {
  Plan* p = new Plan();
  p->events.resize(n_events > 0 ? n_events : 0);
  for (auto& e : p->events)
    if (hipEventCreateWithFlags(&e, hipEventDisableTiming) != hipSuccess) {
      delete p;
      pfr_set_error("pfr_plan_create: hipEventCreate failed");
      return nullptr;
    }
  return p;
}

extern "C" int pfr_plan_destroy(void* plan) {
  Plan* p = reinterpret_cast<Plan*>(plan);
  if (!p) return PFR_OK;
  for (auto& e : p->events) (void)hipEventDestroy(e);
  delete p;
  return PFR_OK;
}

extern "C" int pfr_plan_append(void* plan, int kind, int thunk, int ev, const unsigned long long* args, int nargs) {
  Plan* p = reinterpret_cast<Plan*>(plan);
  PFR_CHECK_ARG(p && kind >= 0 && kind <= 6, "pfr_plan_append: bad plan / kind");
  PFR_CHECK_ARG(kind >= 2 || (thunk >= 0 && thunk < (int)(sizeof(g_thunks) / sizeof(g_thunks[0])) && nargs >= 0 && nargs <= 30 && args),
                "pfr_plan_append: bad thunk / argument count");
  PFR_CHECK_ARG(kind < 2 || kind == 6 || (ev >= 0 && ev < (int)p->events.size()), "pfr_plan_append: bad event index");
  PlanOp op;
  op.kind = kind; op.thunk = thunk; op.ev = ev; op.arg = nargs;
  if (kind < 2) memcpy(op.a, args, sizeof(unsigned long long) * nargs);
  p->ops.push_back(op);
  return PFR_OK;
}

extern "C" int pfr_plan_size(void* plan) { return plan ? (int)reinterpret_cast<Plan*>(plan)->ops.size() : 0; }

extern "C" int pfr_plan_run(void* plan, int begin, int end, pfr_stream_t main_stream, pfr_stream_t side_stream, int hook_stops) {
  Plan* p = reinterpret_cast<Plan*>(plan);
  if (!p) { pfr_set_error("pfr_plan_run: null plan"); return -2; }
  const int n = (int)p->ops.size();
  if (end < 0 || end > n) end = n;
  hipStream_t ms = (hipStream_t)main_stream, ss = (hipStream_t)side_stream;
  const bool use_side = ss != nullptr;
  static const int apply_thunk = pfr_plan_thunk_index("pfr_bn_bwd_apply");
  int attached = -1;
  for (int i = begin; i < end; ++i) {
    const PlanOp& op = p->ops[i];
    switch (op.kind) {
      case 0:
      case 1: {
        if (op.kind == 0 && use_side && op.thunk == apply_thunk && i + 1 < end && p->ops[i + 1].kind == 2) {
          pfr_tls_stop_event = p->events[p->ops[i + 1].ev];
          attached = i + 1;
        }
        const int rc = g_thunks[op.thunk].fn(op.a, (op.kind == 1 && use_side) ? (void*)ss : (void*)ms);
        if (pfr_tls_stop_event != nullptr) {
          pfr_tls_stop_event = nullptr;
          attached = -1;
        }
        if (rc != PFR_OK) return rc <= -2 ? rc : -2 + (rc < 0 ? rc : 0) - 1;
        break;
      }
      case 2:
        if (use_side) {
          if ((attached != i && hipEventRecord(p->events[op.ev], ms) != hipSuccess) || hipStreamWaitEvent(ss, p->events[op.ev], 0) != hipSuccess) {
            pfr_set_error("pfr_plan_run: fork failed");
            return -2;
          }
        }
        break;
      case 3:
        if (use_side && hipEventRecord(p->events[op.ev], ss) != hipSuccess) { pfr_set_error("pfr_plan_run: record failed"); return -2; }
        break;
      case 5:
        if (hook_stops != 1) break;
        [[fallthrough]];
      case 4:
        if (use_side && hipStreamWaitEvent(ms, p->events[op.ev], 0) != hipSuccess) { pfr_set_error("pfr_plan_run: wait failed"); return -2; }
        break;
      case 6:
        if (hook_stops) return i;
        break;
    }
  }
  return -1;
}
```

### pets-face-recognition_amd/csrc/pfr_thunks_gen.inc

```
static int th_pfr_conv2d_fwd(const unsigned long long* a, void* st) { return pfr_conv2d_fwd((const void*)(uintptr_t)a[0], (const void*)(uintptr_t)a[1], (void*)(uintptr_t)a[2], (int)(long long)a[3], (int)(long long)a[4], (int)(long long)a[5], (int)(long long)a[6], (int)(long long)a[7], (int)(long long)a[8], (int)(long long)a[9], (int)(long long)a[10], (int)(long long)a[11], (int)(long long)a[12], (int)(long long)a[13], (int)(long long)a[14], (int)(long long)a[15], (int)(long long)a[16], (int)(long long)a[17], (const float*)(uintptr_t)a[18], (const void*)(uintptr_t)a[19], (int)(long long)a[20], (int)(long long)a[21], (const float*)(uintptr_t)a[22], (const float*)(uintptr_t)a[23], (int)(long long)a[24], (float*)(uintptr_t)a[25], (hipStream_t)st); }
static int th_pfr_conv2d_dgrad_join(const unsigned long long* a, void* st) { return pfr_conv2d_dgrad_join((const void*)(uintptr_t)a[0], (const void*)(uintptr_t)a[1], (void*)(uintptr_t)a[2], (int)(long long)a[3], (int)(long long)a[4], (int)(long long)a[5], (int)(long long)a[6], (int)(long long)a[7], (int)(long long)a[8], (int)(long long)a[9], (int)(long long)a[10], (int)(long long)a[11], (int)(long long)a[12], (int)(long long)a[13], (int)(long long)a[14], (const void*)(uintptr_t)a[15], (const unsigned char*)(uintptr_t)a[16], (hipStream_t)st); }
static int th_pfr_conv2d_dgrad_bn(const unsigned long long* a, void* st) { return pfr_conv2d_dgrad_bn((const void*)(uintptr_t)a[0], (const void*)(uintptr_t)a[1], (void*)(uintptr_t)a[2], (int)(long long)a[3], (int)(long long)a[4], (int)(long long)a[5], (int)(long long)a[6], (int)(long long)a[7], (int)(long long)a[8], (int)(long long)a[9], (int)(long long)a[10], (int)(long long)a[11], (int)(long long)a[12], (int)(long long)a[13], (int)(long long)a[14], (const void*)(uintptr_t)a[15], (const unsigned char*)(uintptr_t)a[16], (int)(long long)a[17], (const void*)(uintptr_t)a[18], (const float*)(uintptr_t)a[19], (const unsigned char*)(uintptr_t)a[20], (float*)(uintptr_t)a[21], (const void*)(uintptr_t)a[22], (const float*)(uintptr_t)a[23], (float*)(uintptr_t)a[24], (hipStream_t)st); }
static int th_pfr_conv2d_dgrad_bn_sub(const unsigned long long* a, void* st) { return pfr_conv2d_dgrad_bn_sub((const void*)(uintptr_t)a[0], (const void*)(uintptr_t)a[1], (void*)(uintptr_t)a[2], (int)(long long)a[3], (int)(long long)a[4], (int)(long long)a[5], (int)(long long)a[6], (int)(long long)a[7], (int)(long long)a[8], (int)(long long)a[9], (int)(long long)a[10], (const void*)(uintptr_t)a[11], (const void*)(uintptr_t)a[12], (const float*)(uintptr_t)a[13], (const unsigned char*)(uintptr_t)a[14], (float*)(uintptr_t)a[15], (hipStream_t)st); }
static int th_pfr_conv1x1_stats(const unsigned long long* a, void* st) { return pfr_conv1x1_stats((const void*)(uintptr_t)a[0], (const void*)(uintptr_t)a[1], (int)(long long)a[2], (int)(long long)a[3], (int)(long long)a[4], (int)(long long)a[5], (int)(long long)a[6], (int)(long long)a[7], (float*)(uintptr_t)a[8], (hipStream_t)st); }
static int th_pfr_conv1x1_bn_tail(const unsigned long long* a, void* st) { return pfr_conv1x1_bn_tail((const void*)(uintptr_t)a[0], (const void*)(uintptr_t)a[1], (void*)(uintptr_t)a[2], (unsigned char*)(uintptr_t)a[3], (int)(long long)a[4], (int)(long long)a[5], (int)(long long)a[6], (int)(long long)a[7], (int)(long long)a[8], (int)(long long)a[9], (const float*)(uintptr_t)a[10], (const float*)(uintptr_t)a[11], (const void*)(uintptr_t)a[12], (const float*)(uintptr_t)a[13], (const float*)(uintptr_t)a[14], (hipStream_t)st); }
static int th_pfr_conv2d_dgrad_bn_ex(const unsigned long long* a, void* st) { return pfr_conv2d_dgrad_bn_ex((const void*)(uintptr_t)a[0], (const void*)(uintptr_t)a[1], (void*)(uintptr_t)a[2], (int)(long long)a[3], (int)(long long)a[4], (int)(long long)a[5], (int)(long long)a[6], (int)(long long)a[7], (int)(long long)a[8], (int)(long long)a[9], (int)(long long)a[10], (int)(long long)a[11], (int)(long long)a[12], (int)(long long)a[13], (int)(long long)a[14], (const void*)(uintptr_t)a[15], (const unsigned char*)(uintptr_t)a[16], (int)(long long)a[17], (const void*)(uintptr_t)a[18], (const float*)(uintptr_t)a[19], (const unsigned char*)(uintptr_t)a[20], (float*)(uintptr_t)a[21], (const void*)(uintptr_t)a[22], (const float*)(uintptr_t)a[23], (float*)(uintptr_t)a[24], (int)(long long)a[25], (hipStream_t)st); }
static int th_pfr_conv2d_dgrad_bn_sub_ex(const unsigned long long* a, void* st) { return pfr_conv2d_dgrad_bn_sub_ex((const void*)(uintptr_t)a[0], (const void*)(uintptr_t)a[1], (void*)(uintptr_t)a[2], (int)(long long)a[3], (int)(long long)a[4], (int)(long long)a[5], (int)(long long)a[6], (int)(long long)a[7], (int)(long long)a[8], (int)(long long)a[9], (int)(long long)a[10], (const void*)(uintptr_t)a[11], (const void*)(uintptr_t)a[12], (const float*)(uintptr_t)a[13], (const unsigned char*)(uintptr_t)a[14], (float*)(uintptr_t)a[15], (int)(long long)a[16], (hipStream_t)st); }
static int th_pfr_bn3_bwd_coef(const unsigned long long* a, void* st) { return pfr_bn3_bwd_coef((const float*)(uintptr_t)a[0], (int)(long long)a[1], (const float*)(uintptr_t)a[2], (const float*)(uintptr_t)a[3], (const void*)(uintptr_t)a[4], (int)(long long)a[5], (const float*)(uintptr_t)a[6], (const float*)(uintptr_t)a[7], (int)(long long)a[8], (int)(long long)a[9], u2f_(a[10]), (float*)(uintptr_t)a[11], (float*)(uintptr_t)a[12], (float*)(uintptr_t)a[13], (int)(long long)a[14], (hipStream_t)st); }
static int th_pfr_bn3_bwd_weights(const unsigned long long* a, void* st) { return pfr_bn3_bwd_weights((const float*)(uintptr_t)a[0], (const float*)(uintptr_t)a[1], (const float*)(uintptr_t)a[2], (const float*)(uintptr_t)a[3], (const void*)(uintptr_t)a[4], (int)(long long)a[5], (int)(long long)a[6], (int)(long long)a[7], u2f_(a[8]), (float*)(uintptr_t)a[9], (void*)(uintptr_t)a[10], (void*)(uintptr_t)a[11], (float*)(uintptr_t)a[12], (int)(long long)a[13], (hipStream_t)st); }
static int th_pfr_conv1x1_dgrad2_bn(const unsigned long long* a, void* st) { return pfr_conv1x1_dgrad2_bn((const void*)(uintptr_t)a[0], (const void*)(uintptr_t)a[1], (const void*)(uintptr_t)a[2], (const float*)(uintptr_t)a[3], (void*)(uintptr_t)a[4], (int)(long long)a[5], (int)(long long)a[6], (int)(long long)a[7], (int)(long long)a[8], (int)(long long)a[9], (int)(long long)a[10], (int)(long long)a[11], (const void*)(uintptr_t)a[12], (const float*)(uintptr_t)a[13], (float*)(uintptr_t)a[14], (hipStream_t)st); }
static int th_pfr_bn_stats_from_gram(const unsigned long long* a, void* st) { return pfr_bn_stats_from_gram((const float*)(uintptr_t)a[0], (const void*)(uintptr_t)a[1], (int)(long long)a[2], (int)(long long)a[3], (int)(long long)a[4], u2f_(a[5]), (float*)(uintptr_t)a[6], u2f_(a[7]), (int*)(uintptr_t)a[8], (hipStream_t)st); }
static int th_pfr_bn_finalize_from_gram(const unsigned long long* a, void* st) { return pfr_bn_finalize_from_gram((const float*)(uintptr_t)a[0], (const void*)(uintptr_t)a[1], (int)(long long)a[2], (int)(long long)a[3], (int)(long long)a[4], u2f_(a[5]), (const float*)(uintptr_t)a[6], (const float*)(uintptr_t)a[7], u2f_(a[8]), u2f_(a[9]), (float*)(uintptr_t)a[10], (float*)(uintptr_t)a[11], (float*)(uintptr_t)a[12], (float*)(uintptr_t)a[13], (float*)(uintptr_t)a[14], (float*)(uintptr_t)a[15], (int*)(uintptr_t)a[16], (hipStream_t)st); }
static int th_pfr_gram_colsum(const unsigned long long* a, void* st) { return pfr_gram_colsum((const void*)(uintptr_t)a[0], (int)(long long)a[1], (long)(long long)a[2], (int)(long long)a[3], (float*)(uintptr_t)a[4], (float*)(uintptr_t)a[5], (hipStream_t)st); }
static int th_pfr_conv2d_wgrad(const unsigned long long* a, void* st) { return pfr_conv2d_wgrad((const void*)(uintptr_t)a[0], (const void*)(uintptr_t)a[1], (float*)(uintptr_t)a[2], (float*)(uintptr_t)a[3], (int)(long long)a[4], (int)(long long)a[5], (int)(long long)a[6], (int)(long long)a[7], (int)(long long)a[8], (int)(long long)a[9], (int)(long long)a[10], (int)(long long)a[11], (int)(long long)a[12], (int)(long long)a[13], (int)(long long)a[14], (int)(long long)a[15], (int)(long long)a[16], (const float*)(uintptr_t)a[17], (const float*)(uintptr_t)a[18], (int)(long long)a[19], u2f_(a[20]), (int)(long long)a[21], (hipStream_t)st); }
static int th_pfr_nchw_to_nhwc(const unsigned long long* a, void* st) { return pfr_nchw_to_nhwc((const float*)(uintptr_t)a[0], (void*)(uintptr_t)a[1], (int)(long long)a[2], (int)(long long)a[3], (int)(long long)a[4], (int)(long long)a[5], (int)(long long)a[6], (int)(long long)a[7], (hipStream_t)st); }
static int th_pfr_cast(const unsigned long long* a, void* st) { return pfr_cast((const void*)(uintptr_t)a[0], (int)(long long)a[1], (void*)(uintptr_t)a[2], (int)(long long)a[3], (size_t)(long long)a[4], (hipStream_t)st); }
static int th_pfr_weight_dgrad_layout(const unsigned long long* a, void* st) { return pfr_weight_dgrad_layout((const void*)(uintptr_t)a[0], (void*)(uintptr_t)a[1], (int)(long long)a[2], (int)(long long)a[3], (int)(long long)a[4], (int)(long long)a[5], (int)(long long)a[6], (hipStream_t)st); }
static int th_pfr_weight_dgrad_layout_batch(const unsigned long long* a, void* st) { return pfr_weight_dgrad_layout_batch((const void*)(uintptr_t)a[0], (int)(long long)a[1], (int)(long long)a[2], (hipStream_t)st); }
static int th_pfr_add(const unsigned long long* a, void* st) { return pfr_add((const void*)(uintptr_t)a[0], (const void*)(uintptr_t)a[1], (void*)(uintptr_t)a[2], (int)(long long)a[3], (size_t)(long long)a[4], (hipStream_t)st); }
static int th_pfr_colsum(const unsigned long long* a, void* st) { return pfr_colsum((const void*)(uintptr_t)a[0], (int)(long long)a[1], (long)(long long)a[2], (int)(long long)a[3], (float*)(uintptr_t)a[4], (int)(long long)a[5], (float*)(uintptr_t)a[6], (hipStream_t)st); }
static int th_pfr_colsum_partial(const unsigned long long* a, void* st) { return pfr_colsum_partial((const void*)(uintptr_t)a[0], (int)(long long)a[1], (long)(long long)a[2], (int)(long long)a[3], (float*)(uintptr_t)a[4], (hipStream_t)st); }
static int th_pfr_colsum_final_batch(const unsigned long long* a, void* st) { return pfr_colsum_final_batch((const void*)(uintptr_t)a[0], (int)(long long)a[1], (int)(long long)a[2], (hipStream_t)st); }
static int th_pfr_copy2d_f32(const unsigned long long* a, void* st) { return pfr_copy2d_f32((const float*)(uintptr_t)a[0], (int)(long long)a[1], (float*)(uintptr_t)a[2], (int)(long long)a[3], (long)(long long)a[4], (int)(long long)a[5], u2f_(a[6]), (int)(long long)a[7], (hipStream_t)st); }
static int th_pfr_bn_stats(const unsigned long long* a, void* st) { return pfr_bn_stats((const void*)(uintptr_t)a[0], (int)(long long)a[1], (long)(long long)a[2], (int)(long long)a[3], (float*)(uintptr_t)a[4], (hipStream_t)st); }
static int th_pfr_bn_finalize(const unsigned long long* a, void* st) { return pfr_bn_finalize((const float*)(uintptr_t)a[0], (int)(long long)a[1], (long)(long long)a[2], (int)(long long)a[3], u2f_(a[4]), (const float*)(uintptr_t)a[5], (const float*)(uintptr_t)a[6], u2f_(a[7]), u2f_(a[8]), (float*)(uintptr_t)a[9], (float*)(uintptr_t)a[10], (float*)(uintptr_t)a[11], (float*)(uintptr_t)a[12], (float*)(uintptr_t)a[13], (float*)(uintptr_t)a[14], (float*)(uintptr_t)a[15], (hipStream_t)st); }
static int th_pfr_fold_bn(const unsigned long long* a, void* st) { return pfr_fold_bn((const void*)(uintptr_t)a[0], (int)(long long)a[1], (int)(long long)a[2], (hipStream_t)st); }
static int th_pfr_fold_bn_cached(const unsigned long long* a, void* st) { return pfr_fold_bn_cached((const void*)(uintptr_t)a[0], (int)(long long)a[1], (int)(long long)a[2], (const float*)(uintptr_t)a[3], (size_t)(long long)a[4], (void*)(uintptr_t)a[5], (unsigned long long*)(uintptr_t)a[6], (hipStream_t)st); }
static int th_pfr_bn_eval_coeff(const unsigned long long* a, void* st) { return pfr_bn_eval_coeff((int)(long long)a[0], (const float*)(uintptr_t)a[1], (const float*)(uintptr_t)a[2], (const float*)(uintptr_t)a[3], (const float*)(uintptr_t)a[4], u2f_(a[5]), (float*)(uintptr_t)a[6], (float*)(uintptr_t)a[7], (hipStream_t)st); }
static int th_pfr_bn_act(const unsigned long long* a, void* st) { return pfr_bn_act((const void*)(uintptr_t)a[0], (const float*)(uintptr_t)a[1], (const float*)(uintptr_t)a[2], (const void*)(uintptr_t)a[3], (const float*)(uintptr_t)a[4], (const float*)(uintptr_t)a[5], (void*)(uintptr_t)a[6], (int)(long long)a[7], (long)(long long)a[8], (int)(long long)a[9], (int)(long long)a[10], (hipStream_t)st); }
static int th_pfr_bn_act_mask(const unsigned long long* a, void* st) { return pfr_bn_act_mask((const void*)(uintptr_t)a[0], (const float*)(uintptr_t)a[1], (const float*)(uintptr_t)a[2], (const void*)(uintptr_t)a[3], (const float*)(uintptr_t)a[4], (const float*)(uintptr_t)a[5], (void*)(uintptr_t)a[6], (unsigned char*)(uintptr_t)a[7], (int)(long long)a[8], (long)(long long)a[9], (int)(long long)a[10], (int)(long long)a[11], (hipStream_t)st); }
static int th_pfr_bn_bwd_reduce(const unsigned long long* a, void* st) { return pfr_bn_bwd_reduce((const void*)(uintptr_t)a[0], (const void*)(uintptr_t)a[1], (const void*)(uintptr_t)a[2], (const float*)(uintptr_t)a[3], (const float*)(uintptr_t)a[4], (const float*)(uintptr_t)a[5], (const float*)(uintptr_t)a[6], (int)(long long)a[7], (int)(long long)a[8], (long)(long long)a[9], (int)(long long)a[10], (float*)(uintptr_t)a[11], (hipStream_t)st); }
static int th_pfr_bn_bwd_finalize(const unsigned long long* a, void* st) { return pfr_bn_bwd_finalize((const float*)(uintptr_t)a[0], (int)(long long)a[1], (int)(long long)a[2], u2f_(a[3]), (const float*)(uintptr_t)a[4], (const float*)(uintptr_t)a[5], (const float*)(uintptr_t)a[6], (float*)(uintptr_t)a[7], (float*)(uintptr_t)a[8], (float*)(uintptr_t)a[9], (int)(long long)a[10], (hipStream_t)st); }
static int th_pfr_bn_bwd_apply(const unsigned long long* a, void* st) { return pfr_bn_bwd_apply((const void*)(uintptr_t)a[0], (const void*)(uintptr_t)a[1], (const void*)(uintptr_t)a[2], (const float*)(uintptr_t)a[3], (const float*)(uintptr_t)a[4], (const float*)(uintptr_t)a[5], (int)(long long)a[6], (void*)(uintptr_t)a[7], (void*)(uintptr_t)a[8], (int)(long long)a[9], (long)(long long)a[10], (int)(long long)a[11], (hipStream_t)st); }
static int th_pfr_bn_relu_maxpool_fwd(const unsigned long long* a, void* st) { return pfr_bn_relu_maxpool_fwd((const void*)(uintptr_t)a[0], (const float*)(uintptr_t)a[1], (const float*)(uintptr_t)a[2], (void*)(uintptr_t)a[3], (uint8_t*)(uintptr_t)a[4], (int)(long long)a[5], (int)(long long)a[6], (int)(long long)a[7], (int)(long long)a[8], (int)(long long)a[9], (int)(long long)a[10], (hipStream_t)st); }
static int th_pfr_maxpool_bwd(const unsigned long long* a, void* st) { return pfr_maxpool_bwd((const void*)(uintptr_t)a[0], (const uint8_t*)(uintptr_t)a[1], (void*)(uintptr_t)a[2], (int)(long long)a[3], (int)(long long)a[4], (int)(long long)a[5], (int)(long long)a[6], (int)(long long)a[7], (hipStream_t)st); }
static int th_pfr_avgpool_fwd(const unsigned long long* a, void* st) { return pfr_avgpool_fwd((const void*)(uintptr_t)a[0], (void*)(uintptr_t)a[1], (int)(long long)a[2], (int)(long long)a[3], (int)(long long)a[4], (int)(long long)a[5], (hipStream_t)st); }
static int th_pfr_avgpool_bwd(const unsigned long long* a, void* st) { return pfr_avgpool_bwd((const void*)(uintptr_t)a[0], (void*)(uintptr_t)a[1], (int)(long long)a[2], (int)(long long)a[3], (int)(long long)a[4], (int)(long long)a[5], (hipStream_t)st); }
static int th_pfr_s2d_input(const unsigned long long* a, void* st) { return pfr_s2d_input((const float*)(uintptr_t)a[0], (void*)(uintptr_t)a[1], (int)(long long)a[2], (int)(long long)a[3], (int)(long long)a[4], (int)(long long)a[5], (int)(long long)a[6], (int)(long long)a[7], (hipStream_t)st); }
static int th_pfr_s2d_weight(const unsigned long long* a, void* st) { return pfr_s2d_weight((const float*)(uintptr_t)a[0], (void*)(uintptr_t)a[1], (int)(long long)a[2], (int)(long long)a[3], (int)(long long)a[4], (int)(long long)a[5], (hipStream_t)st); }
static int th_pfr_s2d_wgrad(const unsigned long long* a, void* st) { return pfr_s2d_wgrad((const float*)(uintptr_t)a[0], (float*)(uintptr_t)a[1], (int)(long long)a[2], (int)(long long)a[3], (int)(long long)a[4], (int)(long long)a[5], (hipStream_t)st); }
static int th_pfr_transpose2d(const unsigned long long* a, void* st) { return pfr_transpose2d((const void*)(uintptr_t)a[0], (void*)(uintptr_t)a[1], (int)(long long)a[2], (int)(long long)a[3], (int)(long long)a[4], (hipStream_t)st); }
static int th_pfr_l2norm_dual(const unsigned long long* a, void* st) { return pfr_l2norm_dual((const float*)(uintptr_t)a[0], (void*)(uintptr_t)a[1], (float*)(uintptr_t)a[2], (float*)(uintptr_t)a[3], (int)(long long)a[4], (int)(long long)a[5], u2f_(a[6]), (hipStream_t)st); }
static int th_pfr_l2norm_fwd(const unsigned long long* a, void* st) { return pfr_l2norm_fwd((const void*)(uintptr_t)a[0], (int)(long long)a[1], (void*)(uintptr_t)a[2], (void*)(uintptr_t)a[3], (int)(long long)a[4], (float*)(uintptr_t)a[5], (int)(long long)a[6], (int)(long long)a[7], (int)(long long)a[8], u2f_(a[9]), (hipStream_t)st); }
static int th_pfr_l2norm_bwd(const unsigned long long* a, void* st) { return pfr_l2norm_bwd((const void*)(uintptr_t)a[0], (int)(long long)a[1], (const float*)(uintptr_t)a[2], (const float*)(uintptr_t)a[3], (void*)(uintptr_t)a[4], (int)(long long)a[5], (int)(long long)a[6], (int)(long long)a[7], (int)(long long)a[8], (hipStream_t)st); }
static int th_pfr_margin_ce(const unsigned long long* a, void* st) { return pfr_margin_ce((const float*)(uintptr_t)a[0], (const int64_t*)(uintptr_t)a[1], (int)(long long)a[2], (int)(long long)a[3], (int)(long long)a[4], (int)(long long)a[5], u2f_(a[6]), u2f_(a[7]), u2f_(a[8]), u2f_(a[9]), (const float*)(uintptr_t)a[10], (float*)(uintptr_t)a[11], (float*)(uintptr_t)a[12], (void*)(uintptr_t)a[13], (int)(long long)a[14], (hipStream_t)st); }
static int th_pfr_margin_bwd(const unsigned long long* a, void* st) { return pfr_margin_bwd((const float*)(uintptr_t)a[0], (const int64_t*)(uintptr_t)a[1], (int)(long long)a[2], (int)(long long)a[3], (int)(long long)a[4], (int)(long long)a[5], u2f_(a[6]), u2f_(a[7]), (const float*)(uintptr_t)a[8], (void*)(uintptr_t)a[9], (int)(long long)a[10], (hipStream_t)st); }
static int th_pfr_mean(const unsigned long long* a, void* st) { return pfr_mean((const float*)(uintptr_t)a[0], (float*)(uintptr_t)a[1], (int)(long long)a[2], (hipStream_t)st); }
static int th_pfr_sgd_step(const unsigned long long* a, void* st) { return pfr_sgd_step((float*)(uintptr_t)a[0], (const float*)(uintptr_t)a[1], (float*)(uintptr_t)a[2], (void*)(uintptr_t)a[3], (int)(long long)a[4], (size_t)(long long)a[5], u2f_(a[6]), u2f_(a[7]), u2f_(a[8]), u2f_(a[9]), (int)(long long)a[10], (hipStream_t)st); }
static int th_pfr_adamw_step(const unsigned long long* a, void* st) { return pfr_adamw_step((float*)(uintptr_t)a[0], (const float*)(uintptr_t)a[1], (float*)(uintptr_t)a[2], (float*)(uintptr_t)a[3], (void*)(uintptr_t)a[4], (int)(long long)a[5], (size_t)(long long)a[6], u2f_(a[7]), u2f_(a[8]), u2f_(a[9]), u2f_(a[10]), u2f_(a[11]), (int)(long long)a[12], u2f_(a[13]), (hipStream_t)st); }
static int th_pfr_sgd_step_clip(const unsigned long long* a, void* st) { return pfr_sgd_step_clip((float*)(uintptr_t)a[0], (const float*)(uintptr_t)a[1], (float*)(uintptr_t)a[2], (void*)(uintptr_t)a[3], (int)(long long)a[4], (size_t)(long long)a[5], u2f_(a[6]), u2f_(a[7]), u2f_(a[8]), u2f_(a[9]), (int)(long long)a[10], (const float*)(uintptr_t)a[11], u2f_(a[12]), (hipStream_t)st); }
static int th_pfr_adamw_step_clip(const unsigned long long* a, void* st) { return pfr_adamw_step_clip((float*)(uintptr_t)a[0], (const float*)(uintptr_t)a[1], (float*)(uintptr_t)a[2], (float*)(uintptr_t)a[3], (void*)(uintptr_t)a[4], (int)(long long)a[5], (size_t)(long long)a[6], u2f_(a[7]), u2f_(a[8]), u2f_(a[9]), u2f_(a[10]), u2f_(a[11]), (int)(long long)a[12], u2f_(a[13]), (const float*)(uintptr_t)a[14], u2f_(a[15]), (hipStream_t)st); }
static int th_pfr_grad_norm(const unsigned long long* a, void* st) { return pfr_grad_norm((const void*)(uintptr_t)a[0], (const int*)(uintptr_t)a[1], (int)(long long)a[2], (long)(long long)a[3], u2f_(a[4]), u2f_(a[5]), (double*)(uintptr_t)a[6], (float*)(uintptr_t)a[7], (hipStream_t)st); }
static int th_pfr_layernorm_fwd(const unsigned long long* a, void* st) { return pfr_layernorm_fwd((const void*)(uintptr_t)a[0], (const float*)(uintptr_t)a[1], (const float*)(uintptr_t)a[2], (void*)(uintptr_t)a[3], (float*)(uintptr_t)a[4], (float*)(uintptr_t)a[5], (int)(long long)a[6], (long)(long long)a[7], (int)(long long)a[8], u2f_(a[9]), (hipStream_t)st); }
static int th_pfr_layernorm_bwd(const unsigned long long* a, void* st) { return pfr_layernorm_bwd((const void*)(uintptr_t)a[0], (const void*)(uintptr_t)a[1], (const float*)(uintptr_t)a[2], (const float*)(uintptr_t)a[3], (const float*)(uintptr_t)a[4], (const void*)(uintptr_t)a[5], (void*)(uintptr_t)a[6], (float*)(uintptr_t)a[7], (int)(long long)a[8], (long)(long long)a[9], (int)(long long)a[10], (hipStream_t)st); }
static int th_pfr_layernorm_bwd_dxsum(const unsigned long long* a, void* st) { return pfr_layernorm_bwd_dxsum((const void*)(uintptr_t)a[0], (const void*)(uintptr_t)a[1], (const float*)(uintptr_t)a[2], (const float*)(uintptr_t)a[3], (const float*)(uintptr_t)a[4], (const void*)(uintptr_t)a[5], (void*)(uintptr_t)a[6], (float*)(uintptr_t)a[7], (float*)(uintptr_t)a[8], (int)(long long)a[9], (long)(long long)a[10], (int)(long long)a[11], (hipStream_t)st); }
static int th_pfr_gelu_fwd(const unsigned long long* a, void* st) { return pfr_gelu_fwd((const void*)(uintptr_t)a[0], (void*)(uintptr_t)a[1], (int)(long long)a[2], (size_t)(long long)a[3], (hipStream_t)st); }
static int th_pfr_gelu_bwd(const unsigned long long* a, void* st) { return pfr_gelu_bwd((const void*)(uintptr_t)a[0], (const void*)(uintptr_t)a[1], (void*)(uintptr_t)a[2], (int)(long long)a[3], (size_t)(long long)a[4], (hipStream_t)st); }
static int th_pfr_window_bias_table(const unsigned long long* a, void* st) { return pfr_window_bias_table((const float*)(uintptr_t)a[0], (float*)(uintptr_t)a[1], (int)(long long)a[2], (int)(long long)a[3], (hipStream_t)st); }
static int th_pfr_window_bias_table_batch(const unsigned long long* a, void* st) { return pfr_window_bias_table_batch((const void*)(uintptr_t)a[0], (int)(long long)a[1], (hipStream_t)st); }
static int th_pfr_window_attn_fwd(const unsigned long long* a, void* st) { return pfr_window_attn_fwd((const void*)(uintptr_t)a[0], (const float*)(uintptr_t)a[1], (void*)(uintptr_t)a[2], (int)(long long)a[3], (int)(long long)a[4], (int)(long long)a[5], (int)(long long)a[6], (int)(long long)a[7], (int)(long long)a[8], (int)(long long)a[9], (int)(long long)a[10], u2f_(a[11]), (hipStream_t)st); }
static int th_pfr_window_attn_bwd(const unsigned long long* a, void* st) { return pfr_window_attn_bwd((const void*)(uintptr_t)a[0], (const float*)(uintptr_t)a[1], (const void*)(uintptr_t)a[2], (void*)(uintptr_t)a[3], (float*)(uintptr_t)a[4], (int)(long long)a[5], (int)(long long)a[6], (int)(long long)a[7], (int)(long long)a[8], (int)(long long)a[9], (int)(long long)a[10], (int)(long long)a[11], (int)(long long)a[12], u2f_(a[13]), (hipStream_t)st); }
static int th_pfr_nhwc_to_nchw_f32(const unsigned long long* a, void* st) { return pfr_nhwc_to_nchw_f32((const float*)(uintptr_t)a[0], (float*)(uintptr_t)a[1], (int)(long long)a[2], (int)(long long)a[3], (int)(long long)a[4], (int)(long long)a[5], (int)(long long)a[6], (hipStream_t)st); }
static int th_pfr_topk_reset(const unsigned long long* a, void* st) { return pfr_topk_reset((void*)(uintptr_t)a[0], (int)(long long)a[1], (int)(long long)a[2], (hipStream_t)st); }
static int th_pfr_topk_update(const unsigned long long* a, void* st) { return pfr_topk_update((const float*)(uintptr_t)a[0], (int)(long long)a[1], (int)(long long)a[2], (int)(long long)a[3], (int)(long long)a[4], (int)(long long)a[5], (void*)(uintptr_t)a[6], (const int*)(uintptr_t)a[7], (hipStream_t)st); }
static int th_pfr_match_scores_filter(const unsigned long long* a, void* st) { return pfr_match_scores_filter((const void*)(uintptr_t)a[0], (const void*)(uintptr_t)a[1], (int)(long long)a[2], (int)(long long)a[3], (int)(long long)a[4], (int)(long long)a[5], (int)(long long)a[6], (int)(long long)a[7], (void*)(uintptr_t)a[8], (void*)(uintptr_t)a[9], (int)(long long)a[10], (int)(long long)a[11], (hipStream_t)st); }
static int th_pfr_topk_merge(const unsigned long long* a, void* st) { return pfr_topk_merge((const void*)(uintptr_t)a[0], (int)(long long)a[1], (int)(long long)a[2], (int)(long long)a[3], (void*)(uintptr_t)a[4], (hipStream_t)st); }
static int th_pfr_quantize_rows_i8(const unsigned long long* a, void* st) { return pfr_quantize_rows_i8((const float*)(uintptr_t)a[0], (void*)(uintptr_t)a[1], (int)(long long)a[2], (float*)(uintptr_t)a[3], (float*)(uintptr_t)a[4], (float*)(uintptr_t)a[5], (int)(long long)a[6], (int)(long long)a[7], (int)(long long)a[8], u2f_(a[9]), (hipStream_t)st); }
static int th_pfr_match_scores_i8(const unsigned long long* a, void* st) { return pfr_match_scores_i8((const void*)(uintptr_t)a[0], (const float*)(uintptr_t)a[1], (const void*)(uintptr_t)a[2], (const float*)(uintptr_t)a[3], (int)(long long)a[4], (int)(long long)a[5], (int)(long long)a[6], (float*)(uintptr_t)a[7], (int)(long long)a[8], (hipStream_t)st); }
static int th_pfr_match_scores_filter_i8(const unsigned long long* a, void* st) { return pfr_match_scores_filter_i8((const void*)(uintptr_t)a[0], (const float*)(uintptr_t)a[1], (const void*)(uintptr_t)a[2], (const float*)(uintptr_t)a[3], (int)(long long)a[4], (int)(long long)a[5], (int)(long long)a[6], (int)(long long)a[7], (int)(long long)a[8], (void*)(uintptr_t)a[9], (void*)(uintptr_t)a[10], (int)(long long)a[11], (int)(long long)a[12], (hipStream_t)st); }
static int th_pfr_topk_flags(const unsigned long long* a, void* st) { return pfr_topk_flags((const void*)(uintptr_t)a[0], (int)(long long)a[1], (int)(long long)a[2], (int*)(uintptr_t)a[3], (hipStream_t)st); }
static int th_pfr_topk_finish(const unsigned long long* a, void* st) { return pfr_topk_finish((const void*)(uintptr_t)a[0], (int)(long long)a[1], (int)(long long)a[2], (float*)(uintptr_t)a[3], (int*)(uintptr_t)a[4], (hipStream_t)st); }
static int th_pfr_topk_rescore(const unsigned long long* a, void* st) { return pfr_topk_rescore((const float*)(uintptr_t)a[0], (const float*)(uintptr_t)a[1], (const float*)(uintptr_t)a[2], (int)(long long)a[3], (int)(long long)a[4], (const int*)(uintptr_t)a[5], (int)(long long)a[6], (int)(long long)a[7], (float*)(uintptr_t)a[8], (int*)(uintptr_t)a[9], (hipStream_t)st); }
static int th_pfr_topk_rescore_cert(const unsigned long long* a, void* st) { return pfr_topk_rescore_cert((const float*)(uintptr_t)a[0], (const float*)(uintptr_t)a[1], (const float*)(uintptr_t)a[2], (int)(long long)a[3], (int)(long long)a[4], (const int*)(uintptr_t)a[5], (const float*)(uintptr_t)a[6], (int)(long long)a[7], (int)(long long)a[8], (float*)(uintptr_t)a[9], (int*)(uintptr_t)a[10], (float*)(uintptr_t)a[11], (hipStream_t)st); }
static int th_pfr_pair_similarity(const unsigned long long* a, void* st) { return pfr_pair_similarity((const float*)(uintptr_t)a[0], (int)(long long)a[1], (const long*)(uintptr_t)a[2], (const long*)(uintptr_t)a[3], (int)(long long)a[4], u2f_(a[5]), (float*)(uintptr_t)a[6], (hipStream_t)st); }
static int th_pfr_pair_curve(const unsigned long long* a, void* st) { return pfr_pair_curve((const float*)(uintptr_t)a[0], (const int*)(uintptr_t)a[1], (int)(long long)a[2], (void*)(uintptr_t)a[3], (float*)(uintptr_t)a[4], (int*)(uintptr_t)a[5], (unsigned char*)(uintptr_t)a[6], (hipStream_t)st); }
static int th_pfr_card_centroids(const unsigned long long* a, void* st) { return pfr_card_centroids((const float*)(uintptr_t)a[0], (const long*)(uintptr_t)a[1], (int)(long long)a[2], (int)(long long)a[3], u2f_(a[4]), (float*)(uintptr_t)a[5], (void*)(uintptr_t)a[6], (int)(long long)a[7], (hipStream_t)st); }
static int th_pfr_card_fuse_scores(const unsigned long long* a, void* st) { return pfr_card_fuse_scores((float*)(uintptr_t)a[0], (const float*)(uintptr_t)a[1], (int)(long long)a[2], (int)(long long)a[3], (int)(long long)a[4], (int)(long long)a[5], (const unsigned char*)(uintptr_t)a[6], (const unsigned char*)(uintptr_t)a[7], (const float*)(uintptr_t)a[8], (int)(long long)a[9], (hipStream_t)st); }
static int th_pfr_augment_train(const unsigned long long* a, void* st) { return pfr_augment_train((const unsigned char*)(uintptr_t)a[0], (int)(long long)a[1], (int)(long long)a[2], (int)(long long)a[3], (int)(long long)a[4], (int)(long long)a[5], (int)(long long)a[6], (int)(long long)a[7], (const int*)(uintptr_t)a[8], (float*)(uintptr_t)a[9], (void*)(uintptr_t)a[10], (hipStream_t)st); }
static int th_pfr_gemm_act(const unsigned long long* a, void* st) { return pfr_gemm_act((const void*)(uintptr_t)a[0], (const void*)(uintptr_t)a[1], (void*)(uintptr_t)a[2], (int)(long long)a[3], (long)(long long)a[4], (int)(long long)a[5], (int)(long long)a[6], (const float*)(uintptr_t)a[7], (int)(long long)a[8], (void*)(uintptr_t)a[9], (hipStream_t)st); }
static int th_pfr_gemm_act_colstats(const unsigned long long* a, void* st) { return pfr_gemm_act_colstats((const void*)(uintptr_t)a[0], (const void*)(uintptr_t)a[1], (void*)(uintptr_t)a[2], (int)(long long)a[3], (long)(long long)a[4], (int)(long long)a[5], (int)(long long)a[6], (const float*)(uintptr_t)a[7], (int)(long long)a[8], (void*)(uintptr_t)a[9], (float*)(uintptr_t)a[10], (hipStream_t)st); }
static int th_pfr_gemm_act_colsums(const unsigned long long* a, void* st) { return pfr_gemm_act_colsums((const void*)(uintptr_t)a[0], (const void*)(uintptr_t)a[1], (void*)(uintptr_t)a[2], (int)(long long)a[3], (long)(long long)a[4], (int)(long long)a[5], (int)(long long)a[6], (void*)(uintptr_t)a[7], (float*)(uintptr_t)a[8], (hipStream_t)st); }
static int th_pfr_comm_allreduce(const unsigned long long* a, void* st) { return pfr_comm_allreduce((void*)(uintptr_t)a[0], (void*)(uintptr_t)a[1], (size_t)(long long)a[2], (int)(long long)a[3], (int)(long long)a[4], (hipStream_t)st); }
static const PlanThunk g_thunks[] = {
  {"pfr_conv2d_fwd", th_pfr_conv2d_fwd},
  {"pfr_conv2d_dgrad_join", th_pfr_conv2d_dgrad_join},
  {"pfr_conv2d_dgrad_bn", th_pfr_conv2d_dgrad_bn},
  {"pfr_conv2d_dgrad_bn_sub", th_pfr_conv2d_dgrad_bn_sub},
  {"pfr_conv1x1_stats", th_pfr_conv1x1_stats},
  {"pfr_conv1x1_bn_tail", th_pfr_conv1x1_bn_tail},
  {"pfr_conv2d_dgrad_bn_ex", th_pfr_conv2d_dgrad_bn_ex},
  {"pfr_conv2d_dgrad_bn_sub_ex", th_pfr_conv2d_dgrad_bn_sub_ex},
  {"pfr_bn3_bwd_coef", th_pfr_bn3_bwd_coef},
  {"pfr_bn3_bwd_weights", th_pfr_bn3_bwd_weights},
  {"pfr_conv1x1_dgrad2_bn", th_pfr_conv1x1_dgrad2_bn},
  {"pfr_bn_stats_from_gram", th_pfr_bn_stats_from_gram},
  {"pfr_bn_finalize_from_gram", th_pfr_bn_finalize_from_gram},
  {"pfr_gram_colsum", th_pfr_gram_colsum},
  {"pfr_conv2d_wgrad", th_pfr_conv2d_wgrad},
  {"pfr_nchw_to_nhwc", th_pfr_nchw_to_nhwc},
  {"pfr_cast", th_pfr_cast},
  {"pfr_weight_dgrad_layout", th_pfr_weight_dgrad_layout},
  {"pfr_weight_dgrad_layout_batch", th_pfr_weight_dgrad_layout_batch},
  {"pfr_add", th_pfr_add},
  {"pfr_colsum", th_pfr_colsum},
  {"pfr_colsum_partial", th_pfr_colsum_partial},
  {"pfr_colsum_final_batch", th_pfr_colsum_final_batch},
  {"pfr_copy2d_f32", th_pfr_copy2d_f32},
  {"pfr_bn_stats", th_pfr_bn_stats},
  {"pfr_bn_finalize", th_pfr_bn_finalize},
  {"pfr_fold_bn", th_pfr_fold_bn},
  {"pfr_fold_bn_cached", th_pfr_fold_bn_cached},
  {"pfr_bn_eval_coeff", th_pfr_bn_eval_coeff},
  {"pfr_bn_act", th_pfr_bn_act},
  {"pfr_bn_act_mask", th_pfr_bn_act_mask},
  {"pfr_bn_bwd_reduce", th_pfr_bn_bwd_reduce},
  {"pfr_bn_bwd_finalize", th_pfr_bn_bwd_finalize},
  {"pfr_bn_bwd_apply", th_pfr_bn_bwd_apply},
  {"pfr_bn_relu_maxpool_fwd", th_pfr_bn_relu_maxpool_fwd},
  {"pfr_maxpool_bwd", th_pfr_maxpool_bwd},
  {"pfr_avgpool_fwd", th_pfr_avgpool_fwd},
  {"pfr_avgpool_bwd", th_pfr_avgpool_bwd},
  {"pfr_s2d_input", th_pfr_s2d_input},
  {"pfr_s2d_weight", th_pfr_s2d_weight},
  {"pfr_s2d_wgrad", th_pfr_s2d_wgrad},
  {"pfr_transpose2d", th_pfr_transpose2d},
  {"pfr_l2norm_dual", th_pfr_l2norm_dual},
  {"pfr_l2norm_fwd", th_pfr_l2norm_fwd},
  {"pfr_l2norm_bwd", th_pfr_l2norm_bwd},
  {"pfr_margin_ce", th_pfr_margin_ce},
  {"pfr_margin_bwd", th_pfr_margin_bwd},
  {"pfr_mean", th_pfr_mean},
  {"pfr_sgd_step", th_pfr_sgd_step},
  {"pfr_adamw_step", th_pfr_adamw_step},
  {"pfr_sgd_step_clip", th_pfr_sgd_step_clip},
  {"pfr_adamw_step_clip", th_pfr_adamw_step_clip},
  {"pfr_grad_norm", th_pfr_grad_norm},
  {"pfr_layernorm_fwd", th_pfr_layernorm_fwd},
  {"pfr_layernorm_bwd", th_pfr_layernorm_bwd},
  {"pfr_layernorm_bwd_dxsum", th_pfr_layernorm_bwd_dxsum},
  {"pfr_gelu_fwd", th_pfr_gelu_fwd},
  {"pfr_gelu_bwd", th_pfr_gelu_bwd},
  {"pfr_window_bias_table", th_pfr_window_bias_table},
  {"pfr_window_bias_table_batch", th_pfr_window_bias_table_batch},
  {"pfr_window_attn_fwd", th_pfr_window_attn_fwd},
  {"pfr_window_attn_bwd", th_pfr_window_attn_bwd},
  {"pfr_nhwc_to_nchw_f32", th_pfr_nhwc_to_nchw_f32},
  {"pfr_topk_reset", th_pfr_topk_reset},
  {"pfr_topk_update", th_pfr_topk_update},
  {"pfr_match_scores_filter", th_pfr_match_scores_filter},
  {"pfr_topk_merge", th_pfr_topk_merge},
  {"pfr_quantize_rows_i8", th_pfr_quantize_rows_i8},
  {"pfr_match_scores_i8", th_pfr_match_scores_i8},
  {"pfr_match_scores_filter_i8", th_pfr_match_scores_filter_i8},
  {"pfr_topk_flags", th_pfr_topk_flags},
  {"pfr_topk_finish", th_pfr_topk_finish},
  {"pfr_topk_rescore", th_pfr_topk_rescore},
  {"pfr_topk_rescore_cert", th_pfr_topk_rescore_cert},
  {"pfr_pair_similarity", th_pfr_pair_similarity},
  {"pfr_pair_curve", th_pfr_pair_curve},
  {"pfr_card_centroids", th_pfr_card_centroids},
  {"pfr_card_fuse_scores", th_pfr_card_fuse_scores},
  {"pfr_augment_train", th_pfr_augment_train},
  {"pfr_gemm_act", th_pfr_gemm_act},
  {"pfr_gemm_act_colstats", th_pfr_gemm_act_colstats},
  {"pfr_gemm_act_colsums", th_pfr_gemm_act_colsums},
  {"pfr_comm_allreduce", th_pfr_comm_allreduce},
};
```

### pets-face-recognition_amd/models/_fe_engine.py

```python
import os
import weakref

import torch
import torch.nn as nn

from .._hip import lib, dtype_id, PfrError
from .._hip.lib import _TRACER
from .._hip.ops import conv_out_hw
from .._hip.cplan import CPlan

_ALIGN = 64


def default_compute_dtype():
    v = os.environ.get("PFR_COMPUTE_DTYPE", "bf16").lower()
    return torch.float32 if v in ("f32", "fp32", "float32") else torch.bfloat16


def flat_layout(model):
    offs, total = {}, 0
    for name, p in model.named_parameters():
        offs[name] = total
        total += (p.numel() + _ALIGN - 1) // _ALIGN * _ALIGN
    return offs, total


def grad_ready_marks(model):
    offs, _ = flat_layout(model)
    marks = [offs["fc.weight"]]
    for lname in ("layer4", "layer3", "layer2", "layer1"):
        layer = getattr(model, lname)
        for bi in reversed(range(len(layer))):
            marks.append(offs[f"{lname}.{bi}.conv1.weight"])
    marks.append(0)
    return marks


class _Conv:
    pass


class _BN:
    pass


_SIDE, _FORK, _SREC, _WAIT, _MWAIT = 1, 2, 3, 4, 5


def _side_with_ddp():
    try:
        return int(os.environ.get("GPU_MAX_HW_QUEUES", "4")) >= 8
    except ValueError:
        return False


class PlanTicket:
    __slots__ = ("__weakref__",)


class _Plan:
    __slots__ = ("ops", "bufs", "meta")

    def __init__(self):
        self.ops = []
        self.bufs = {}
        self.meta = {}

    def run(self, stream, hook=None):
        for fn, args in self.ops:
            if fn is None:
                if hook is not None:
                    hook(*args)
            else:
                fn(*args, stream)


class FEEngine:
    def __init__(self, model, device, compute_dtype=None):
        if not str(device).startswith("cuda"):
            raise PfrError("FEEngine runs on the HIP device only (no CPU fallback)")
        lib.pfr_version()
        self.device = torch.device(device)
        self.dtype = compute_dtype or default_compute_dtype()
        self.did = dtype_id(self.dtype)
        self.kp = 8 if self.dtype == torch.bfloat16 else 4
        self.model_id = id(model)
        self.fc_id = id(model.fc)
        self.plans = {}
        self.side = None
        self.side_events = []
        self.fold_eval = True
        self.fold_w = None
        self.fold_cache = True
        self.fold_state = None
        self.graph_eval = os.environ.get("PFR_GRAPH_EVAL", "0") == "1"
        self.wt_fork = self.wt_ready = None
        self.wt_pending = False
        self.side_stream_enabled = os.environ.get("PFR_SIDE_STREAM", "1") != "0"
        self.c_plan = os.environ.get("PFR_C_PLAN", "1") != "0"
        self.fuse_bnb = int(os.environ.get("PFR_FUSE_BNB", "2") or 0)
        lib.pfr_set_tuning(b"bnb", self.fuse_bnb)
        self._tuning_epoch = lib.pfr_tuning_epoch()
        self._bnb_min_rows = 0
        self.bnfree = os.environ.get("PFR_BNFREE", "1") != "0" and self.dtype == torch.bfloat16 and self.fuse_bnb == 2
        self.gram_stats = os.environ.get("PFR_BNFREE_GRAMSTATS", "1") != "0"
        self.gram_flag = torch.zeros(1, dtype=torch.int32).pin_memory()
        self.ws_main = None
        self.grad_ready_hook = None
        self.hook_syncs_side = False
        self.bucket_elems = 6 * 1024 * 1024
        self._adopt(model)

    def _adopt(self, model):
        dev = self.device
        named = list(model.named_parameters())
        offs, total = flat_layout(model)
        self.n_flat = total
        self.master = torch.zeros(total, dtype=torch.float32, device=dev)
        self.grad = torch.zeros(total, dtype=torch.float32, device=dev)
        self.shadow = self.master if self.dtype == torch.float32 else torch.zeros(total, dtype=self.dtype, device=dev)
        self.offs = offs
        self.param_list = []
        self._views = {}
        for name, p in named:
            o, n = offs[name], p.numel()
            if p.dim() == 4:
                O, I, R, S = p.shape
                mv = self.master[o:o + n].view(O, R, S, I)
                mv.copy_(p.data.detach().to(dev).permute(0, 2, 3, 1))
                pv = mv.permute(0, 3, 1, 2)
                gv = self.grad[o:o + n].view(O, R, S, I).permute(0, 3, 1, 2)
            else:
                mv = self.master[o:o + n].view(p.shape)
                mv.copy_(p.data.detach().to(dev))
                pv = mv
                gv = self.grad[o:o + n].view(p.shape)
            p.data = pv
            p.grad = None
            self._views[name] = (p, gv)
            self.param_list.append(p)
        self.first_param = named[0][1]
        bns = [(n, m) for n, m in model.named_modules() if isinstance(m, nn.BatchNorm2d)]
        nstat = sum(m.num_features for _, m in bns)
        self.stats = torch.zeros(2 * nstat, dtype=torch.float32, device=dev)
        self.nbt = torch.zeros(len(bns), dtype=torch.int64, device=dev)
        so = 0
        self._bn_of = {}
        for i, (n, m) in enumerate(bns):
            C = m.num_features
            rm = self.stats[so:so + C]
            rv = self.stats[nstat + so:nstat + so + C]
            rm.copy_(m.running_mean.detach().to(dev))
            rv.copy_(m.running_var.detach().to(dev))
            self.nbt[i] = int(m.num_batches_tracked.item())
            m.running_mean = rm
            m.running_var = rv
            m.num_batches_tracked = self.nbt[i]
            so += C
            b = _BN()
            b.C, b.eps, b.momentum = C, m.eps, (m.momentum if m.momentum is not None else 0.1)
            b.gamma = self.master[offs[n + ".weight"]:offs[n + ".weight"] + C]
            b.beta = self.master[offs[n + ".bias"]:offs[n + ".bias"] + C]
            b.dgamma = self.grad[offs[n + ".weight"]:offs[n + ".weight"] + C]
            b.dbeta = self.grad[offs[n + ".bias"]:offs[n + ".bias"] + C]
            b.g_off = offs[n + ".weight"]
            b.rm, b.rv = rm, rv
            b.coef = torch.zeros((4, C), dtype=torch.float32, device=dev)
            b.bcoef = torch.zeros((3, C), dtype=torch.float32, device=dev)
            self._bn_of[id(m)] = b
        self.bn_list = [self._bn_of[id(m)] for _, m in bns]
        maxc = max(m.num_features for _, m in bns)
        self.bn_ws = torch.empty(max(1, lib.pfr_bn_finalize_ws_floats(1 << 20, maxc)), dtype=torch.float32, device=dev)

        def conv_rec(name, m):
            c = _Conv()
            c.name = name
            c.Cout, c.Cin, c.R, c.S = m.weight.shape
            c.stride, c.pad = m.stride[0], m.padding[0]
            c.off = offs[name + ".weight"]
            n = m.weight.numel()
            c.w = self.shadow[c.off:c.off + n].view(c.Cout, c.R, c.S, c.Cin)
            c.g = self.grad[c.off:c.off + n].view(c.Cout, c.R, c.S, c.Cin)
            c.wt = torch.zeros((c.Cin, c.R, c.S, c.Cout), dtype=self.dtype, device=dev)
            c.need_wt = True
            return c

        self._conv_of = {}
        for n, m in model.named_modules():
            if isinstance(m, nn.Conv2d):
                if m.bias is not None or m.groups != 1 or m.dilation[0] != 1:
                    raise PfrError(f"{n}: only bias-free, dense, undilated convolutions are supported")
                self._conv_of[id(m)] = conv_rec(n, m)
        st = self._conv_of[id(model.conv1)]
        st.need_wt = False
        self.cp = (st.Cin + self.kp - 1) // self.kp * self.kp
        st.w_pad = torch.zeros((st.Cout, st.R, st.S, self.cp), dtype=self.dtype, device=dev)
        st.g_pad = torch.zeros((st.Cout, st.R, st.S, self.cp), dtype=torch.float32, device=dev)
        self.s2d = None
        if (st.R, st.S, st.stride, st.pad) == (7, 7, 2, 3) and self.dtype == torch.bfloat16:
            q = _Conv()
            q.name = st.name + "(s2d)"
            q.Cout, q.Cin, q.R, q.S, q.stride, q.pad = st.Cout, (4 * st.Cin + self.kp - 1) // self.kp * self.kp, 4, 4, 1, 2
            q.w = torch.zeros((q.Cout, 4, 4, q.Cin), dtype=self.dtype, device=dev)
            q.g = torch.zeros((q.Cout, 4, 4, q.Cin), dtype=torch.float32, device=dev)
            q.off, q.need_wt = st.off, False
            self.s2d = q
        self.stem = (st, self._bn_of[id(model.bn1)])
        self.blocks = []
        for layer in (model.layer1, model.layer2, model.layer3, model.layer4):
            for blk in layer:
                convs = []
                i = 1
                while hasattr(blk, f"conv{i}"):
                    convs.append((self._conv_of[id(getattr(blk, f"conv{i}"))], self._bn_of[id(getattr(blk, f"bn{i}"))]))
                    i += 1
                down = None
                if blk.downsample is not None:
                    down = (self._conv_of[id(blk.downsample[0])], self._bn_of[id(blk.downsample[1])])
                self.blocks.append((convs, down))
        fc = model.fc
        if not isinstance(fc, nn.Linear):
            raise PfrError("model.fc must be an nn.Linear")
        f = _Conv()
        f.name = "fc"
        f.Cout, f.Cin, f.R, f.S, f.stride, f.pad = fc.out_features, fc.in_features, 1, 1, 1, 0
        f.off = offs["fc.weight"]
        n = fc.weight.numel()
        f.w = self.shadow[f.off:f.off + n].view(f.Cout, 1, 1, f.Cin)
        f.g = self.grad[f.off:f.off + n].view(f.Cout, 1, 1, f.Cin)
        f.wt = torch.zeros((f.Cin, 1, 1, f.Cout), dtype=self.dtype, device=dev)
        f.need_wt = True
        if fc.bias is not None:
            bo = offs["fc.bias"]
            f.bias = self.master[bo:bo + f.Cout]
            f.dbias = self.grad[bo:bo + f.Cout]
        else:
            f.bias = f.dbias = None
        self.fc = f
        self.emb_dim = f.Cout
        self.all_convs = [c for c in self._conv_of.values()] + [f]
        self.ws = None
        torch.cuda.synchronize(dev)

    def matches(self, model):
        return (id(model) == self.model_id and id(model.fc) == self.fc_id
                and self.first_param.data.data_ptr() == self.master.data_ptr())

    def attach_grads(self):
        for p, gv in self._views.values():
            p.grad = gv

    def flat_ranges(self, params):
        base = self.master.data_ptr()
        spans = []
        for p in params:
            lo = (p.data.data_ptr() - base) // 4
            if lo < 0 or lo >= self.n_flat:
                raise PfrError("parameter does not belong to this engine")
            hi = lo + (p.numel() + _ALIGN - 1) // _ALIGN * _ALIGN
            spans.append((lo, hi))
        spans.sort()
        out = []
        for lo, hi in spans:
            if out and out[-1][1] == lo:
                out[-1] = (out[-1][0], hi)
            else:
                out.append((lo, hi))
        return out

    def _side_ok(self):
        return self.side_stream_enabled and _TRACER[0] is None and (self.grad_ready_hook is None or _side_with_ddp())

    def refresh_weights(self, stream, for_backward=True, cast=True):
        if cast and self.dtype != torch.float32:
            lib.pfr_cast(self.master.data_ptr(), 0, self.shadow.data_ptr(), self.did, self.n_flat, stream)
        st = self.stem[0]
        lib.pfr_nchw_to_nhwc(self.master.data_ptr() + 4 * st.off, st.w_pad.data_ptr(), self.did, st.Cout * st.R * st.S,
                             st.Cin, 1, 1, self.cp, stream)
        if self.s2d is not None:
            lib.pfr_s2d_weight(self.master.data_ptr() + 4 * st.off, self.s2d.w.data_ptr(), self.did, st.Cout, st.Cin, self.s2d.Cin,
                               stream)
        if for_backward:
            sptr = stream
            use_side = self._side_ok()
            if use_side:
                if self.side is None:
                    self.side = torch.cuda.Stream(device=self.device)
                if self.wt_fork is None:
                    self.wt_fork, self.wt_ready = torch.cuda.Event(), torch.cuda.Event()
                self.wt_fork.record(torch.cuda.current_stream())
                self.side.wait_event(self.wt_fork)
                sptr = self.side.cuda_stream
            tab = getattr(self, "_wt_table", None)
            if tab is None:
                import struct
                convs = [c for c in self.all_convs if c.need_wt]
                raw = b"".join(struct.pack("<QQiiii", c.w.data_ptr(), c.wt.data_ptr(), c.Cout, c.R, c.S, c.Cin) for c in convs)
                tab = self._wt_table = (torch.frombuffer(bytearray(raw), dtype=torch.uint8).to(self.device), len(convs))
            lib.pfr_weight_dgrad_layout_batch(tab[0].data_ptr(), tab[1], self.did, sptr)
            self.wt_pending = use_side
            if use_side:
                self.wt_ready.record(self.side)

    def _use_s2d(self, H, W):
        return self.s2d is not None and H % 2 == 0 and W % 2 == 0

    def _input_layout(self, plan, x, stream):
        N, C, H, W = x.shape
        if plan.meta.get("s2d"):
            lib.pfr_s2d_input(x.data_ptr(), plan.meta["x_nhwc"].data_ptr(), self.did, N, C, H, W, self.s2d.Cin, stream)
        else:
            lib.pfr_nchw_to_nhwc(x.data_ptr(), plan.meta["x_nhwc"].data_ptr(), self.did, N, C, H, W, self.cp, stream)

    def _fold_setup(self):
        import struct
        pairs = [self.stem] + [cb for convs, down in self.blocks for cb in convs] + [down for _, down in self.blocks if down]
        if self.s2d is not None:
            pairs.append((self.s2d, self.stem[1]))
        nw = sum((c.w_pad.numel() if c is self.stem[0] else c.w.numel()) for c, _ in pairs)
        nb = sum(c.Cout for c, _ in pairs)
        self.fold_w = torch.empty(nw + _ALIGN * len(pairs), dtype=self.dtype, device=self.device)
        self.fold_b = torch.empty(nb, dtype=torch.float32, device=self.device)
        rec = b""
        wo = bo = 0
        es = self.fold_w.element_size()
        for c, bn in pairs:
            if c is self.stem[0]:
                src, f32, K = c.w_pad.data_ptr(), 0, c.R * c.S * self.cp
            elif c is self.s2d:
                src, f32, K = c.w.data_ptr(), 0, c.R * c.S * c.Cin
            else:
                src, f32, K = self.master.data_ptr() + 4 * c.off, 1, c.R * c.S * c.Cin
            c.wf = self.fold_w[wo:wo + c.Cout * K].view(c.Cout, c.R, c.S, K // (c.R * c.S))
            c.bf = self.fold_b[bo:bo + c.Cout]
            rec += struct.pack("<7q2qfi", src, bn.gamma.data_ptr(), bn.beta.data_ptr(), bn.rm.data_ptr(), bn.rv.data_ptr(),
                               c.wf.data_ptr(), c.bf.data_ptr(), c.Cout, K, float(bn.eps), f32)
            wo += (c.Cout * K + _ALIGN - 1) // _ALIGN * _ALIGN
            bo += c.Cout
        assert len(rec) == 80 * len(pairs)
        self.fold_desc = torch.frombuffer(bytearray(rec), dtype=torch.uint8).to(self.device)
        self.fold_n = len(pairs)
        self.ident = torch.cat([torch.ones(self.stem[0].Cout), torch.zeros(self.stem[0].Cout)]).to(self.device)

    def build_eval_plan(self, N, H, W):
        if getattr(self, "fold_w", None) is None:
            self._fold_setup()
        plan = _Plan()
        ops = plan.ops
        st, _ = self.stem

        def conv(x, xshape, c, relu, residual=None, out_hw=None):
            Nn, Hh, Ww, C = xshape
            OH, OW = out_hw or conv_out_hw(Hh, Ww, c.R, c.S, c.stride, c.pad)
            y = self._A(plan, (Nn, OH, OW, c.Cout))
            ops.append((lib.pfr_conv2d_fwd, (x.data_ptr(), c.wf.data_ptr(), y.data_ptr(), self.did, self.did, Nn, Hh, Ww, C, c.Cout,
                                             c.R, c.S, c.stride, c.pad, 0, OH, OW, c.Cout, c.bf.data_ptr(),
                                             0 if residual is None else residual.data_ptr(), 0, int(relu), 0, 0, 0, 0)))
            return y, (Nn, OH, OW, c.Cout)

        if self._use_s2d(H, W):
            x_nhwc = self._A(plan, (N, H // 2, W // 2, self.s2d.Cin))
            plan.meta["s2d"] = True
            c1, s1 = conv(x_nhwc, (N, H // 2, W // 2, self.s2d.Cin), self.s2d, True, out_hw=(H // 2, W // 2))
        else:
            x_nhwc = self._A(plan, (N, H, W, self.cp))
            c1, s1 = conv(x_nhwc, (N, H, W, self.cp), st, True)
        plan.meta["x_nhwc"] = x_nhwc
        _, H1, W1, _ = s1
        PH, PW = (H1 + 2 - 3) // 2 + 1, (W1 + 2 - 3) // 2 + 1
        cur = self._A(plan, (N, PH, PW, st.Cout))
        ops.append((lib.pfr_bn_relu_maxpool_fwd, (c1.data_ptr(), self.ident.data_ptr(), self.ident.data_ptr() + 4 * st.Cout,
                                                  cur.data_ptr(), 0, self.did, N, H1, W1, st.Cout, 0)))
        cshape = (N, PH, PW, st.Cout)
        for convs, down in self.blocks:
            xin, xshape = cur, cshape
            short = xin
            if down is not None:
                short, _ = conv(xin, xshape, down[0], False)
            z, zs = xin, xshape
            for ci, (c, _) in enumerate(convs):
                last = ci + 1 == len(convs)
                z, zs = conv(z, zs, c, True, residual=short if last else None)
            cur, cshape = z, zs
        Nn, Hh, Ww, Cf = cshape
        gap = self._A(plan, (N, Cf))
        ops.append((lib.pfr_avgpool_fwd, (cur.data_ptr(), gap.data_ptr(), self.did, N, Hh * Ww, Cf)))
        emb = self._A(plan, (N, self.emb_dim), torch.float32)
        f = self.fc
        self._conv_fwd(ops, gap, (N, 1, 1, Cf), f.w, emb, f, 1, 0, 1, 1, bias=f.bias)
        plan.meta["emb"] = emb
        plan.meta["fwd"] = ops
        plan.meta["folded"] = True
        return plan

    def _A(self, plan, shape, dtype=None):
        t = torch.empty(shape, dtype=dtype or self.dtype, device=self.device)
        plan.bufs[len(plan.bufs)] = t
        return t

    def _conv_fwd(self, ops, x, xshape, w, y, c, stride, pad, OH, OW, pro=None, part=None, bias=None, idil=0,
                  accumulate=0, Cout=None, R=None, S=None):
        N, H, W, C = xshape
        Cout = Cout or c.Cout
        R = R or c.R
        S = S or c.S
        ps = psh = 0
# ... 189 lines not shown
                                                      lastbn.coef[3].data_ptr(), res.data_ptr(), a2, b2)))
            elif down is not None:
                dc, dbn = down
                cd, _ = self._conv_bn(plan, ops, xin, xshape, dc, dbn, train)
                ops.append((lib.pfr_bn_act_mask, (src.data_ptr(), lastbn.coef[2].data_ptr(), lastbn.coef[3].data_ptr(),
                                                  cd.data_ptr(), dbn.coef[2].data_ptr(), dbn.coef[3].data_ptr(), out.data_ptr(),
                                                  mptr, self.did, rows, sshape[3], 1)))
            else:
                ops.append((lib.pfr_bn_act_mask, (src.data_ptr(), lastbn.coef[2].data_ptr(), lastbn.coef[3].data_ptr(),
                                                  xin.data_ptr(), 0, 0, out.data_ptr(), mptr, self.did, rows, sshape[3], 1)))
            bsaved.append((xin, xshape, raws, cd, out if rmask is None else rmask, sshape, acts))
            cur, cshape = out, sshape
        Nn, Hh, Ww, Cf = cshape
        gap = self._A(plan, (N, Cf))
        ops.append((lib.pfr_avgpool_fwd, (cur.data_ptr(), gap.data_ptr(), self.did, N, Hh * Ww, Cf)))
        emb = self._A(plan, (N, self.emb_dim), torch.float32)
        f = self.fc
        self._conv_fwd(ops, gap, (N, 1, 1, Cf), f.w, emb, f, 1, 0, 1, 1, bias=f.bias)
        plan.meta["emb"] = emb
        plan.meta["n_fwd"] = len(ops)
        if not with_backward:
            return plan

        pool = {}
        lag = 32
        pending = {}
        nside = [0]

        def G(shape, dtype=None):
            key = (tuple(shape), dtype or T)
            lst = pool.setdefault(key, [])
            for i, t in enumerate(lst):
                k = pending.get(t.data_ptr())
                if k is None or nside[0] - k >= lag:
                    lst.pop(i)
                    if k is not None:
                        del pending[t.data_ptr()]
                        ops.append(("wait", (k,)))
                    return t
            return self._A(plan, shape, dtype)

        def release(t):
            pool.setdefault((tuple(t.shape), t.dtype), []).append(t)

        ws_need = [0]

        def wgrad(x, xshape, dy, dyshape, c, pro=None, out=None, C=None, acc=0):
            Nq, Hq, Wq, Cq = xshape
            _, OH, OW, Co = dyshape
            KK = c.R * c.S * Cq
            splits = lib.pfr_conv2d_wgrad_splits(Nq * OH * OW, Co, KK)
            ws_need[0] = max(ws_need[0], splits * Co * KK)
            ps = psh = 0
            prelu = 0
            if pro is not None:
                ps, psh, prelu = pro[0].data_ptr(), pro[1].data_ptr(), 1
            dst = out if out is not None else c.g
            k = nside[0]
            nside[0] += 1
            ops.append(("fork", (k,)))
            ops.append(("wgrad_noacc" if out is not None else "wgrad", (x.data_ptr(), dy.data_ptr(), dst.data_ptr(), None, self.did, Nq, Hq, Wq, Cq, Co, c.R, c.S,
                                  c.stride, c.pad, OH, OW, Co, ps, psh, prelu, 1.0, acc)))
            ops.append(("srec", (k,)))
            pending[dy.data_ptr()] = k

        ws_main_need = [0]

        def wgrad_main(x, xshape, dy, dyshape, c, out):
            Nq, Hq, Wq, Cq = xshape
            _, OH, OW, Co = dyshape
            KK = c.R * c.S * Cq
            splits = lib.pfr_conv2d_wgrad_splits(Nq * OH * OW, Co, KK)
            ws_main_need[0] = max(ws_main_need[0], splits * Co * KK)
            ops.append(("wgrad_main", (x.data_ptr(), dy.data_ptr(), out.data_ptr(), None, self.did, Nq, Hq, Wq, Cq, Co, c.R, c.S,
                                       c.stride, c.pad, OH, OW, Co, 0, 0, 0, 1.0, 0)))

        def side_op(fn, args):
            k = nside[0]
            nside[0] += 1
            ops.append(("fork", (k,)))
            ops.append(("sideop", (fn, args)))
            ops.append(("srec", (k,)))
            return k

        def dgrad(dy, dyshape, c, dx, dxshape, accumulate=0):
            log2 = {1: 0, 2: 1}[c.stride]
            self._conv_fwd(ops, dy, dyshape, c.wt, dx, c, 1, c.R - 1 - c.pad, dxshape[1], dxshape[2], idil=log2,
                           accumulate=accumulate, Cout=c.Cin)

        def bn_bwd(dout, out_act, x, xshape, bn, mask_mode, dx, gres, acc, pre=None):
            rows = xshape[0] * xshape[1] * xshape[2]
            C = xshape[3]
            oa = 0 if out_act is None else out_act.data_ptr()
            if pre is not None:
                part, nb = pre
            else:
                nb = lib.pfr_colreduce_blocks(C, self.did, rows)
                part = G((nb, 2, C), torch.float32)
                ops.append((lib.pfr_bn_bwd_reduce, (dout.data_ptr(), oa, x.data_ptr(), bn.coef[0].data_ptr(), bn.coef[1].data_ptr(),
                                                    bn.coef[2].data_ptr(), bn.coef[3].data_ptr(), mask_mode, self.did, rows, C,
                                                    part.data_ptr())))
            ops.append((lib.pfr_bn_bwd_finalize, (part.data_ptr(), nb, C, float(rows), bn.gamma.data_ptr(), bn.coef[0].data_ptr(),
                                                  bn.coef[1].data_ptr(), bn.dgamma.data_ptr(), bn.dbeta.data_ptr(),
                                                  bn.bcoef.data_ptr(), acc)))
            ops.append((lib.pfr_bn_bwd_apply, (dout.data_ptr(), oa, x.data_ptr(), bn.bcoef.data_ptr(), bn.coef[2].data_ptr(),
                                               bn.coef[3].data_ptr(), mask_mode, dx.data_ptr(),
                                               0 if gres is None else gres.data_ptr(), self.did, rows, C)))
            release(part)

        dgrad_parts = self._dgrad_parts

        def dgrad_bn(dy, dyshape, c, dx, dxshape, bn1, bn2=None, res=None, res_mask=None, accumulate=0, flags=0, wt=None):
            x1, b1, mk, p1 = bn1
            x2p = c2p = p2p = 0
            if bn2 is not None:
                x2p, c2p, p2p = bn2[0].data_ptr(), bn2[1].coef.data_ptr(), bn2[2].data_ptr()
            args = (dy.data_ptr(), (c.wt if wt is None else wt).data_ptr(), dx.data_ptr(), self.did, dyshape[0], dyshape[1],
                    dyshape[2], dyshape[3], c.Cin, c.R, c.S, c.R - 1 - c.pad, {1: 0, 2: 1}[c.stride],
                    dxshape[1], dxshape[2], 0 if res is None else res.data_ptr(),
                    0 if res_mask is None else res_mask.data_ptr(), accumulate, 0 if x1 is None else x1.data_ptr(),
                    b1.coef.data_ptr(), 0 if mk is None else mk.data_ptr(), p1.data_ptr(), x2p, c2p, p2p)
            if flags:
                ops.append((lib.pfr_conv2d_dgrad_bn_ex, args + (flags,)))
            else:
                ops.append((lib.pfr_conv2d_dgrad_bn, args))

        acc = 0
        demb = self._A(plan, (N, self.emb_dim))
        plan.meta["demb"] = demb
        if f.dbias is not None:
            ops.append(("colsum", (demb.data_ptr(), self.did, N, self.emb_dim, f.dbias.data_ptr(), acc)))
        wgrad(gap, (N, 1, 1, Cf), demb, (N, 1, 1, self.emb_dim), f)
        dgap = G((N, Cf))
        dgrad(demb, (N, 1, 1, self.emb_dim), f, dgap, (N, 1, 1, Cf))
        self._mark(ops, f.off)
        dcur = G(cshape)
        ops.append((lib.pfr_avgpool_bwd, (dgap.data_ptr(), dcur.data_ptr(), self.did, N, Hh * Ww, Cf)))
        release(dgap)
        nblk = len(self.blocks)
        pre3 = {}
        bnf = {}
        premasked = {}
        if free_set:
            for k, npart in free_set.items():
                convs, _ = self.blocks[k]
                _, _, raws, _, _, oshape, acts = bsaved[k]
                c3 = convs[2][0]
                zs = raws[1][1]
                rows = zs[0] * zs[1] * zs[2]
                gram = plan.meta.get("gram", {}).get(k)
                if gram is not None:
                    bnf[k] = dict(G2=gram[:c3.Cin * c3.Cin], zsum=gram[c3.Cin * c3.Cin:], side=None, npart=npart)
                    continue
                G2 = self._A(plan, (c3.Cin, c3.Cin), torch.float32)
                zsum = self._A(plan, (c3.Cin,), torch.float32)
                cws = self._A(plan, (max(1, lib.pfr_colsum_ws_floats(rows, c3.Cin)),), torch.float32)
                wgrad(acts[1], zs, acts[1], zs, c3, out=G2)
                kk = side_op(lib.pfr_colsum, (acts[1].data_ptr(), self.did, rows, c3.Cin, zsum.data_ptr(), 0, cws.data_ptr()))
                bnf[k] = dict(G2=G2, zsum=zsum, side=kk, npart=npart)
            if bnf:
                cmax = max(self.blocks[k][0][2][0].Cout for k in bnf)
                kmax = max(self.blocks[k][0][2][0].Cin for k in bnf)
                bnf_G1 = self._A(plan, (cmax * kmax,), torch.float32)
                bnf_coef = self._A(plan, (3 * cmax,), torch.float32)
                bnf_wat = self._A(plan, ((cmax + kmax) * kmax,))
                bnf_S = self._A(plan, (kmax * kmax,))
                bnf_bias = self._A(plan, (kmax,), torch.float32)
        for k in range(nblk - 1, -1, -1):
            convs, down = self.blocks[k]
            xin, xshape, raws, cd, out, oshape, acts = bsaved[k]
            lastc, lastbn = convs[-1]
            ylast, _ = raws[-1]
            p3 = pre3.get(k)
            rmask = out
            free3 = k in bnf
            if free3 and not (premasked.get(k, False) and p3 is not None):
                raise PfrError(f"block {k}: the forward pass dropped conv3's output but its output gradient was not produced masked")
            if free3:
                c3, bn3 = convs[2]
                _, bn2 = convs[1]
                z2, (c2raw, zs) = acts[1], raws[1]
                f = bnf[k]
                C3, K3, rows3 = c3.Cout, c3.Cin, float(oshape[0] * oshape[1] * oshape[2])
                wgrad_main(z2, zs, dcur, oshape, c3, bnf_G1)
                if f["side"] is not None:
                    ops.append(("wait", (f["side"],)))
                part3, np3 = p3[0]
                Wm = c3.w.data_ptr()
                ops.append((lib.pfr_bn3_bwd_coef, (part3.data_ptr(), np3, bnf_G1.data_ptr(), f["zsum"].data_ptr(), Wm, self.did, bn3.gamma.data_ptr(),
                                                   bn3.coef[1].data_ptr(), C3, K3, rows3, bn3.dgamma.data_ptr(), bn3.dbeta.data_ptr(),
                                                   bnf_coef.data_ptr(), acc)))
                np2 = lib.pfr_conv1x1_dgrad2_bn_parts(self.did, zs[0], zs[1], zs[2], C3, K3, K3)
                ops.append((lib.pfr_bn3_bwd_weights, (bnf_coef.data_ptr(), bnf_G1.data_ptr(), f["G2"].data_ptr(), f["zsum"].data_ptr(), Wm, self.did,
                                                      C3, K3, rows3, c3.g.data_ptr(), bnf_wat.data_ptr(), 0 if np2 > 0 else bnf_S.data_ptr(),
                                                      bnf_bias.data_ptr(), acc)))
                release(part3)
                dz2 = G(zs)
                if np2 > 0:
                    part2 = G((np2, 2, K3), torch.float32)
                    ops.append((lib.pfr_conv1x1_dgrad2_bn, (dcur.data_ptr(), z2.data_ptr(), bnf_wat.data_ptr(), bnf_bias.data_ptr(), dz2.data_ptr(),
                                                            self.did, zs[0], zs[1], zs[2], C3, K3, K3, c2raw.data_ptr(), bn2.coef.data_ptr(),
                                                            part2.data_ptr())))
                else:
                    np2 = f["npart"]
                    y1 = G(zs)
                    ops.append((lib.pfr_conv2d_fwd, (z2.data_ptr(), bnf_S.data_ptr(), y1.data_ptr(), self.did, self.did, zs[0], zs[1], zs[2], K3, K3,
                                                     1, 1, 1, 0, 0, zs[1], zs[2], K3, bnf_bias.data_ptr(), 0, 0, 0, 0, 0, 0, 0)))
                    part2 = G((np2, 2, K3), torch.float32)
                    dgrad_bn(dcur, oshape, c3, dz2, zs, (c2raw, bn2, None, part2), res=y1, wt=bnf_wat)
                    release(y1)
                bn_bwd(dz2, None, c2raw, zs, bn2, 2, dz2, None, acc, pre=(part2, np2))
                dy, dyshape = dz2, zs
            else:
                dz3 = G(oshape)
                bn_bwd(dcur, out, ylast, oshape, lastbn, 3, dz3, None, acc, pre=None if p3 is None else p3[0])
                dy, dyshape = dz3, oshape
            for i in range(len(convs) - 1 - (1 if free3 else 0), 0, -1):
                c, bn = convs[i]
                pc, pbn = convs[i - 1]
                xraw, xrs = raws[i - 1]
                wgrad(acts[i - 1], xrs, dy, dyshape, c)
                dz = G(xrs)
                npart = dgrad_parts(dyshape, c, xrs)
                if npart > 0:
                    part = G((npart, 2, xrs[3]), torch.float32)
                    dgrad_bn(dy, dyshape, c, dz, xrs, (xraw, pbn, None, part))
                    release(dy)
                    bn_bwd(dz, None, xraw, xrs, pbn, 2, dz, None, acc, pre=(part, npart))
                else:
                    dgrad(dy, dyshape, c, dz, xrs)
                    release(dy)
                    bn_bwd(dz, None, xraw, xrs, pbn, 2, dz, None, acc)
                dy, dyshape = dz, xrs
            c0, bn0 = convs[0]
            wgrad(xin, xshape, dy, dyshape, c0)
            dxin = G(xshape)
            nxt = None
            if k > 0:
                pconvs, pdown = self.blocks[k - 1]
                _, _, praws, pcd, pmask, poshape, _ = bsaved[k - 1]
                nxt = (praws[-1][0], pconvs[-1][1], pmask, pcd, None if pdown is None else pdown[1])
            if down is not None:
                dc, dbn = down
                dgd = G(oshape)
                bn_bwd(dcur, rmask, cd, oshape, dbn, 3, dgd, None, acc,
                       pre=None if (p3 is None or p3[1] is None) else p3[1])
                release(dcur)
                wgrad(xin, xshape, dgd, oshape, dc)
                npart3 = 0
                if (nxt is not None and self.fuse_bnb == 2 and nxt[3] is None and dc.R == 1 and dc.stride == 2
                        and xshape[1] % 2 == 0 and xshape[2] % 2 == 0):
                    npart3 = dgrad_parts(dyshape, c0, xshape)
                if npart3 > 0:
                    comp = G((xshape[0], oshape[1], oshape[2], xshape[3]))
                    self._conv_fwd(ops, dgd, oshape, dc.wt, comp, dc, 1, 0, oshape[1], oshape[2], idil=0, Cout=dc.Cin)
                    part = G((npart3, 2, xshape[3]), torch.float32)
                    sub_args = (dy.data_ptr(), c0.wt.data_ptr(), dxin.data_ptr(), self.did, dyshape[0], dyshape[1], dyshape[2], dyshape[3],
                                c0.Cin, xshape[1], xshape[2], comp.data_ptr(), 0 if nxt[0] is None else nxt[0].data_ptr(), nxt[1].coef.data_ptr(),
                                nxt[2].data_ptr(), part.data_ptr())
                    if (k - 1) in bnf:
                        ops.append((lib.pfr_conv2d_dgrad_bn_sub_ex, sub_args + (3,)))
                        premasked[k - 1] = True
                    else:
                        ops.append((lib.pfr_conv2d_dgrad_bn_sub, sub_args))
                    pre3[k - 1] = ((part, npart3), None)
                    release(comp)
                    npart = -1
                else:
                    dgrad(dy, dyshape, c0, dxin, xshape)
                    npart = dgrad_parts(oshape, dc, xshape, accumulates=True) if nxt is not None else 0
                if npart < 0:
                    pass
                elif npart > 0:
                    part = G((npart, 2, xshape[3]), torch.float32)
                    part2 = G((npart, 2, xshape[3]), torch.float32) if nxt[3] is not None else None
                    dgrad_bn(dgd, oshape, dc, dxin, xshape, (nxt[0], nxt[1], nxt[2], part),
                             None if part2 is None else (nxt[3], nxt[4], part2), accumulate=1)
                    pre3[k - 1] = ((part, npart), None if part2 is None else (part2, npart))
                else:
                    dgrad(dgd, oshape, dc, dxin, xshape, accumulate=1)
                release(dgd)
            else:
                log2 = {1: 0, 2: 1}[c0.stride]
                npart = dgrad_parts(dyshape, c0, xshape) if nxt is not None else 0
                if npart > 0:
                    part = G((npart, 2, xshape[3]), torch.float32)
                    part2 = G((npart, 2, xshape[3]), torch.float32) if nxt[3] is not None else None
                    dgrad_bn(dy, dyshape, c0, dxin, xshape, (nxt[0], nxt[1], nxt[2], part),
                             None if part2 is None else (nxt[3], nxt[4], part2), res=dcur, res_mask=rmask,
                             flags=3 if (k - 1) in bnf else 0)
                    if (k - 1) in bnf:
                        premasked[k - 1] = True
                    pre3[k - 1] = ((part, npart), None if part2 is None else (part2, npart))
                else:
                    ops.append((lib.pfr_conv2d_dgrad_join, (dy.data_ptr(), c0.wt.data_ptr(), dxin.data_ptr(), self.did, dyshape[0],
                                                            dyshape[1], dyshape[2], dyshape[3], c0.Cin, c0.R, c0.S, c0.R - 1 - c0.pad,
                                                            log2, xshape[1], xshape[2], dcur.data_ptr(), rmask.data_ptr())))
                release(dcur)
            self._mark(ops, c0.off)
            release(dy)
            dcur = dxin
        c1, s1, idx, pshape = saved["stem"]
        dz = G(s1)
        ops.append((lib.pfr_maxpool_bwd, (dcur.data_ptr(), idx.data_ptr(), dz.data_ptr(), self.did, N, s1[1], s1[2], s1[3])))
        release(dcur)
        bn_bwd(dz, None, c1, s1, stbn, 2, dz, None, acc)
        if use_s2d:
            wgrad(x_nhwc, xin_shape, dz, s1, self.s2d, out=self.s2d.g)
            ops.append(("wait", (nside[0] - 1,)))
            ops.append(("s2dunpack", (self.s2d.g.data_ptr(), st.g.data_ptr(), st.Cout, st.Cin, self.s2d.Cin, acc)))
        else:
            wgrad(x_nhwc, xin_shape, dz, s1, st, out=st.g_pad)
            ops.append(("wait", (nside[0] - 1,)))
            ops.append(("copy2d", (st.g_pad.data_ptr(), self.cp, st.g.data_ptr(), st.Cin, st.Cout * st.R * st.S, st.Cin, 1.0, acc)))
        self._mark(ops, 0)
        plan.meta["n_side"] = nside[0]
        if self.ws is None or self.ws.numel() < ws_need[0]:
            self.ws = torch.empty(ws_need[0], dtype=torch.float32, device=self.device)
        plan.meta["ws_need"] = ws_need[0]
        if ws_main_need[0] and (self.ws_main is None or self.ws_main.numel() < ws_main_need[0]):
            self.ws_main = torch.empty(ws_main_need[0], dtype=torch.float32, device=self.device)
        plan.meta["bnfree_blocks"] = sorted(k for k in bnf if premasked.get(k))
        assert plan.meta["bnfree_blocks"] == sorted(free_set), (plan.meta["bnfree_blocks"], sorted(free_set))
        return plan

    def _mark(self, ops, off):
        last = max((a[0] for f, a in ops if f == "srec"), default=None)
        if last is not None:
            ops.append(("wait" if off == 0 else "mwait", (last,)))
        ops.append((None, (off,)))

    def _check_tuning(self):
        ep = lib.pfr_tuning_epoch()
        stale = False
        if self.gram_stats and int(self.gram_flag[0]) != 0:
            import warnings
            warnings.warn("pfr: bn3 statistics from the Gram matrix lost precision to cancellation (a nearly constant conv3 channel); "
                          "falling back to the statistics pass over conv3's output for the rest of the run")
            self.gram_stats = False
            stale = True
        if ep == self._tuning_epoch and not stale:
            return
        lib.pfr_set_tuning(b"bnb", self.fuse_bnb)
        self._tuning_epoch = lib.pfr_tuning_epoch()
        for k, q in list(self.plans.items()):
            if not self._plan_busy(q):
                self.plans.pop(k)

    def get_plan(self, N, H, W, train, with_backward, slot=0):
        self._check_tuning()
        key = (N, H, W, train, with_backward) + ((slot,) if slot else ())
        p = self.plans.get(key)
        if p is None:
            if len(self.plans) >= 8:
                for k, q in list(self.plans.items()):
                    if not self._plan_busy(q):
                        self.plans.pop(k)
                        break
            if not train and not with_backward and self.fold_eval:
                p = self.build_eval_plan(N, H, W)
            else:
                p = self.build_plan(N, H, W, train, with_backward)
                self._finalize_plan(p)
            self.plans[key] = p
        return p

    @staticmethod
    def _plan_busy(plan):
        own = plan.meta.get("owner")
        return own is not None and own() is not None

    def acquire_plan(self, N, H, W, train, with_backward, ticket):
        slot = 0
        while True:
            plan = self.get_plan(N, H, W, train, with_backward, slot)
            if ticket is None or not self._plan_busy(plan):
                break
            slot += 1
            if slot >= 8:
                raise PfrError("more than 8 forward passes of one shape are waiting for their backward pass")
        if ticket is not None:
            plan.meta["owner"] = weakref.ref(ticket)
        return plan

    def _finalize_plan(self, plan):
        fwd = plan.ops[:plan.meta["n_fwd"]]
        bwd = plan.ops[plan.meta["n_fwd"]:]
        plan.meta["fwd"] = fwd
        for acc in (0, 1):
            res = []
            for fn, args in bwd:
                if fn in ("wgrad", "wgrad_noacc"):
                    a = list(args)
                    a[3] = self.ws.data_ptr()
                    a[-1] = acc if fn == "wgrad" else 0
                    res.append((_SIDE, (lib.pfr_conv2d_wgrad, tuple(a))))
                elif fn == "wgrad_main":
                    a = list(args)
                    a[3] = self.ws_main.data_ptr() if self.ws_main is not None else 0
                    res.append((lib.pfr_conv2d_wgrad, tuple(a)))
                elif fn == "sideop":
                    res.append((_SIDE, (args[0], tuple(args[1]))))
                elif fn == "fork":
                    res.append((_FORK, args[0]))
                elif fn == "srec":
                    res.append((_SREC, args[0]))
                elif fn == "wait":
                    res.append((_WAIT, args[0]))
                elif fn == "mwait":
                    res.append((_MWAIT, args[0]))
                elif fn == "colsum":
                    res.append((lib.pfr_colsum, tuple(args[:-1]) + (acc, 0)))
                elif fn == "copy2d":
                    res.append((lib.pfr_copy2d_f32, tuple(args[:-1]) + (acc,)))
                elif fn == "s2dunpack":
                    res.append((lib.pfr_s2d_wgrad, tuple(args[:-1]) + (acc,)))
                elif fn is lib.pfr_bn_bwd_finalize or fn is lib.pfr_bn3_bwd_coef \
                        or fn is lib.pfr_bn3_bwd_weights:
                    res.append((fn, tuple(args[:-1]) + (acc,)))
                else:
                    res.append((fn, args))
            plan.meta["bwd%d" % acc] = res
            plan.meta.pop("c_bwd%d" % acc, None)
        plan.meta["ws_ptr"] = self._ws_key()

    def _ws_key(self):
        return (self.ws.data_ptr() if self.ws is not None else 0, self.ws_main.data_ptr() if self.ws_main is not None else 0)

    def forward(self, x, train, with_backward, ticket=None):
        if x.dim() != 4 or x.shape[1] != self.stem[0].Cin:
            raise PfrError(f"expected NCHW input with {self.stem[0].Cin} channels, got {tuple(x.shape)}")
        if x.dtype != torch.float32:
            x = x.float()
        x = x.contiguous()
        N, _, H, W = x.shape
        plan = self.acquire_plan(N, H, W, train, with_backward, ticket if with_backward else None)
        plan.meta["epoch"] = self._tuning_epoch
        if with_backward and plan.meta.get("ws_ptr", 0) != self._ws_key():
            self._finalize_plan(plan)
        if plan.meta.get("folded") and self.graph_eval and _TRACER[0] is None:
            return self._forward_graphed(plan, x)
        stream = torch.cuda.current_stream().cuda_stream
        if plan.meta.get("folded") and self.fold_cache:
            self.refresh_weights(stream, for_backward=False, cast=False)
            if self.fold_state is None:
                self.fold_state = torch.tensor([0, -1, 0, 0], dtype=torch.int64, device=self.device)
            lib.pfr_fold_bn_cached(self.fold_desc.data_ptr(), self.fold_n, self.did, self.master.data_ptr(), self.n_flat,
                                   self.shadow.data_ptr() if self.dtype != torch.float32 else 0, self.fold_state.data_ptr(), stream)
        else:
            self.refresh_weights(stream, for_backward=with_backward)
            if plan.meta.get("folded"):
                lib.pfr_fold_bn(self.fold_desc.data_ptr(), self.fold_n, self.did, stream)
        self._input_layout(plan, x, stream)
        if not self._run_list(plan, "fwd", stream):
            for fn, args in plan.meta["fwd"]:
                fn(*args, stream)
        if train:
            self.nbt.add_(1)
        self._last_plan = plan
        return plan.meta["emb"]

    def _run_list(self, plan, key, stream, side=0, hook=None, n_events=0):
        if self.c_plan and _TRACER[0] is None:
            ck = "c_" + key
            cp = plan.meta.get(ck, False)
            if cp is False:
                cp = plan.meta[ck] = CPlan.compile(plan.meta[key], n_events)
            if cp is not None:
                cp.run(stream, side, hook, self.hook_syncs_side)
                return True
        return False

    def _eval_launches(self, plan, xin):
        N, _, H, W = xin.shape
        stream = torch.cuda.current_stream().cuda_stream
        self.refresh_weights(stream, for_backward=False)
        lib.pfr_fold_bn(self.fold_desc.data_ptr(), self.fold_n, self.did, stream)
        self._input_layout(plan, xin, stream)
        if not self._run_list(plan, "fwd", stream):
            for fn, args in plan.meta["fwd"]:
                fn(*args, stream)

    def _forward_graphed(self, plan, x):
        m = plan.meta
        if "x_in" not in m:
            m["x_in"] = torch.empty_like(x)
        xin = m["x_in"]
        xin.copy_(x)
        g = m.get("graph")
        if g is None:
            if m.get("warm", 0) < 1:
                m["warm"] = 1
                self._eval_launches(plan, xin)
            else:
                g = torch.cuda.CUDAGraph()
                with torch.cuda.graph(g):
                    self._eval_launches(plan, xin)
                m["graph"] = g
                g.replay()
        else:
            g.replay()
        self._last_plan = plan
        return m["emb"]

    def _run_bwd_ops(self, plan, acc, hook):
        main = torch.cuda.current_stream()
        stream = main.cuda_stream
        use_side = self._side_ok()
        if use_side and self.side is None:
            self.side = torch.cuda.Stream(device=self.device)
        side_handle = self.side.cuda_stream if use_side else 0
        if self._run_list(plan, "bwd%d" % acc, stream, side_handle,
                          (lambda off: hook(off)) if hook is not None else None, 2 * plan.meta.get("n_side", 0)):
            return
        if use_side:
            side, sptr = self.side, self.side.cuda_stream
            ev = self.side_events
            while len(ev) < 2 * plan.meta.get("n_side", 0):
                ev.append(torch.cuda.Event())
        for fn, args in plan.meta["bwd%d" % acc]:
            if fn is None:
                if hook is not None:
                    hook(args[0])
            elif fn.__class__ is int:
                if not use_side:
                    if fn == _SIDE:
                        args[0](*args[1], stream)
                elif fn == _SIDE:
                    args[0](*args[1], sptr)
                elif fn == _FORK:
                    e = ev[2 * args]
                    e.record(main)
                    side.wait_event(e)
                elif fn == _SREC:
                    ev[2 * args + 1].record(side)
                elif fn == _WAIT or (hook is not None and not self.hook_syncs_side):
                    main.wait_event(ev[2 * args + 1])
            else:
                fn(*args, stream)

    def backward(self, demb, plan=None):
        plan = plan if plan is not None else self._last_plan
        if lib.pfr_tuning_epoch() != plan.meta.get("epoch", self._tuning_epoch):
            raise PfrError("a pfr_set_tuning call changed a kernel-selection knob between this forward pass and its backward pass "
                           "(another engine with a different PFR_FUSE_BNB mode, or a host sweep): run forward again")
        stream = torch.cuda.current_stream().cuda_stream
        demb = demb.contiguous()
        if demb.numel() != plan.meta["demb"].numel():
            raise PfrError(f"backward: gradient of {tuple(demb.shape)} does not match the plan's embedding buffer "
                           f"{tuple(plan.meta['demb'].shape)}")
        if plan.meta.get("ws_ptr", 0) != self._ws_key():
            self._finalize_plan(plan)
        lib.pfr_cast(demb.data_ptr(), dtype_id(demb.dtype), plan.meta["demb"].data_ptr(), self.did, demb.numel(), stream)
        acc = 1 if self.first_param.grad is not None else 0
        plan.meta["owner"] = None
        hook = self.grad_ready_hook if not any(self._plan_busy(q) for q in self.plans.values()) else None
        if hook is None and self.grad_ready_hook is not None and not getattr(self, "_warned_hook", False):
            import warnings
            self._warned_hook = True
            warnings.warn("FEEngine.backward: another forward pass of this model still holds its activations (a retained autograd "
                          "graph?), so gradient buckets are reduced after the backward pass instead of overlapped with it")
        main = torch.cuda.current_stream()
        if self.wt_pending:
            main.wait_event(self.wt_ready)
            self.wt_pending = False
        self._run_bwd_ops(plan, acc, hook)
        if not acc:
            self.attach_grads()


class _FEFunction(torch.autograd.Function):
    @staticmethod
    def forward(ctx, x, model, *params):
        eng = model.hip_engine(x.device)
        ctx.ticket = PlanTicket()
        emb = eng.forward(x, model.training, True, ctx.ticket)
        ctx.eng = eng
        ctx.plan = eng._last_plan
        ctx.nparams = len(params)
        return emb.clone()

    @staticmethod
    def backward(ctx, demb):
        if ctx.plan.meta.get("owner") is None or ctx.plan.meta["owner"]() is not ctx.ticket:
            raise PfrError("backward: the activations of this forward pass were released (double backward?)")
        ctx.eng.backward(demb, ctx.plan)
        return (None, None) + (None,) * ctx.nparams


def fe_forward(model, x):
    eng = model.hip_engine(x.device)
    if torch.is_grad_enabled() and any(p.requires_grad for p in eng.param_list):
        return _FEFunction.apply(x, model, *eng.param_list)
    return eng.forward(x, model.training, False).clone()
```

Baseline: 15160 images/sec.

## Fuse stem maxpool backward into BN backward reduce and apply kernels

Replaces the stem's maxpool-backward kernel plus the separate BN backward reduce/apply passes with two fused kernels. Each kernel recomputes the 2x2 max-pool gradient scatter on the fly from the pooled gradient and argmax indices, so the full-resolution pool gradient is never written to and read back from memory. The cost is recomputing the gather in both passes and a larger per-thread working set, which could lower occupancy. The new path is on by default for bf16, and the side-stream stop-event hookup is extended to cover the new apply kernel.

Result: no change. 15260 images/sec, median of 6 (+0.7%).

```diff
diff --git a/include/pfr_hip.h b/include/pfr_hip.h
--- a/include/pfr_hip.h
+++ b/include/pfr_hip.h
@@ -129,6 +129,12 @@
 int pfr_bn_relu_maxpool_fwd(const void* x, const float* scale, const float* shift, void* y, uint8_t* idx, int dtype, int N,
                             int H, int W, int C, int relu, pfr_stream_t stream);
 int pfr_maxpool_bwd(const void* dy, const uint8_t* idx, void* dz, int dtype, int N, int H, int W, int C, pfr_stream_t stream);
+int pfr_bn_bwd_pool_blocks(int C, int dtype, int N, int H, int W);
+int pfr_bn_bwd_reduce_pool(const void* dpool, const uint8_t* idx, const void* x, const float* mean, const float* invstd,
+                           const float* scale, const float* shift, int dtype, int N, int H, int W, int C, float* part,
+                           pfr_stream_t stream);
+int pfr_bn_bwd_apply_pool(const void* dpool, const uint8_t* idx, const void* x, const float* coef, const float* scale,
+                          const float* shift, void* dx, int dtype, int N, int H, int W, int C, pfr_stream_t stream);
 int pfr_avgpool_fwd(const void* x, void* y, int dtype, int N, int HW, int C, pfr_stream_t stream);
 int pfr_avgpool_bwd(const void* dy, void* dx, int dtype, int N, int HW, int C, pfr_stream_t stream);
 
diff --git a/pets-face-recognition_amd/_hip/lib.py b/pets-face-recognition_amd/_hip/lib.py
--- a/pets-face-recognition_amd/_hip/lib.py
+++ b/pets-face-recognition_amd/_hip/lib.py
@@ -110,7 +110,7 @@
         return dict(self._protos)
 
 
-_NO_CHECK = {"pfr_version", "pfr_grad_norm_chunk_elems", "pfr_conv1x1_dgrad2_bn_parts", "pfr_tuning_epoch", "pfr_gram_ws_floats", "pfr_conv1x1_tail_mtile", "pfr_bn_stats_rows_per_part", "pfr_bn_finalize_ws_floats", "pfr_topk_state_bytes", "pfr_layernorm_bwd_blocks", "pfr_window_bias_table_floats", "pfr_colsum_ws_floats", "pfr_conv2d_mtile", "pfr_gemm_act_mtile", "pfr_conv2d_dgrad_bn_parts", "pfr_plan_thunk_index", "pfr_plan_size", "pfr_plan_run", "pfr_conv2d_wgrad_splits", "pfr_colreduce_blocks", "pfr_match_ws_bytes", "pfr_pair_curve_ws_bytes", "pfr_augment_ws_bytes", "pfr_colsum_parts", "pfr_layernorm_bwd_dxsum_ok", "pfr_gemm_act_colsum_parts"}
+_NO_CHECK = {"pfr_version", "pfr_grad_norm_chunk_elems", "pfr_conv1x1_dgrad2_bn_parts", "pfr_tuning_epoch", "pfr_gram_ws_floats", "pfr_conv1x1_tail_mtile", "pfr_bn_stats_rows_per_part", "pfr_bn_finalize_ws_floats", "pfr_topk_state_bytes", "pfr_layernorm_bwd_blocks", "pfr_window_bias_table_floats", "pfr_colsum_ws_floats", "pfr_conv2d_mtile", "pfr_gemm_act_mtile", "pfr_conv2d_dgrad_bn_parts", "pfr_plan_thunk_index", "pfr_plan_size", "pfr_plan_run", "pfr_conv2d_wgrad_splits", "pfr_colreduce_blocks", "pfr_bn_bwd_pool_blocks", "pfr_match_ws_bytes", "pfr_pair_curve_ws_bytes", "pfr_augment_ws_bytes", "pfr_colsum_parts", "pfr_layernorm_bwd_dxsum_ok", "pfr_gemm_act_colsum_parts"}
 
 lib = _Lib()
 
diff --git a/pets-face-recognition_amd/_hip/ops.py b/pets-face-recognition_amd/_hip/ops.py
--- a/pets-face-recognition_amd/_hip/ops.py
+++ b/pets-face-recognition_amd/_hip/ops.py
@@ -218,6 +218,28 @@
     return dz
 
 
+def bn_bwd_pool(dpool, idx, x, mean, invstd, gamma, scale, shift, coef=None):
+    N, H, W, C = x.shape
+    did = dtype_id(x.dtype)
+    dx = torch.empty_like(x)
+    if coef is not None:
+        lib.pfr_bn_bwd_apply_pool(_p(dpool), _p(idx), _p(x), _p(coef), _p(scale), _p(shift), _p(dx), did, N, H, W, C, _stream())
+        return dx
+    nb = lib.pfr_bn_bwd_pool_blocks(C, did, N, H, W)
+    if nb <= 0:
+        raise PfrError(f"bn_bwd_pool: geometry {tuple(x.shape)} not taken (odd H or W)")
+    part = torch.empty((nb, 2, C), dtype=torch.float32, device=x.device)
+    lib.pfr_bn_bwd_reduce_pool(_p(dpool), _p(idx), _p(x), _p(mean), _p(invstd), _p(scale), _p(shift), did, N, H, W, C, _p(part),
+                               _stream())
+    coef = torch.empty((3, C), dtype=torch.float32, device=x.device)
+    dgamma = torch.empty(C, dtype=torch.float32, device=x.device)
+    dbeta = torch.empty(C, dtype=torch.float32, device=x.device)
+    lib.pfr_bn_bwd_finalize(_p(part), nb, C, float(N * H * W), _p(gamma), _p(mean), _p(invstd), _p(dgamma), _p(dbeta), _p(coef), 0,
+                            _stream())
+    lib.pfr_bn_bwd_apply_pool(_p(dpool), _p(idx), _p(x), _p(coef), _p(scale), _p(shift), _p(dx), did, N, H, W, C, _stream())
+    return dx, dgamma, dbeta, coef
+
+
 def avgpool_fwd(x):
     N, H, W, C = x.shape
     y = torch.empty((N, C), dtype=x.dtype, device=x.device)
diff --git a/pets-face-recognition_amd/csrc/pfr_api.hip b/pets-face-recognition_amd/csrc/pfr_api.hip
--- a/pets-face-recognition_amd/csrc/pfr_api.hip
+++ b/pets-face-recognition_amd/csrc/pfr_api.hip
@@ -31,6 +31,7 @@
   {"sconv", 1}, {"sconv3", 1}, {"bnb", 0}, {"swgrad", 1}, {"wgrad_big", 0}, {"wgrad_tile", -1}, {"wgrad_splits", 0}, {"wgrad9", 1},
   {"wgrad9_slots", 256}, {"attn_mfma", 1}, {"bnb_tile3", 0}, {"slin", 1}, {"slin_np", 0}, {"match_order", 1},
   {"ln_rb", 4}, {"sstem", 1}, {"igemm_dma", 0x101}, {"igemm_krot", 0},
+  {"bnpool_rgrid", 512}, {"bnpool_agrid", 512}, {"bnpool_ub", 1},
 };
 int g_pfr_knob[KNOB_COUNT];
 static const bool g_knobs_ready = [] { for (int k = 0; k < KNOB_COUNT; ++k) g_pfr_knob[k] = kKnobs[k].def; return true; }();
diff --git a/pets-face-recognition_amd/csrc/pfr_common.h b/pets-face-recognition_amd/csrc/pfr_common.h
--- a/pets-face-recognition_amd/csrc/pfr_common.h
+++ b/pets-face-recognition_amd/csrc/pfr_common.h
@@ -52,6 +52,9 @@
   KNOB_SSTEM,
   KNOB_IGEMM_DMA,
   KNOB_IGEMM_KROT,
+  KNOB_BNPOOL_RGRID,
+  KNOB_BNPOOL_AGRID,
+  KNOB_BNPOOL_UB,
   KNOB_COUNT
 };
 extern int g_pfr_knob[KNOB_COUNT];
diff --git a/pets-face-recognition_amd/csrc/pfr_elementwise.hip b/pets-face-recognition_amd/csrc/pfr_elementwise.hip
--- a/pets-face-recognition_amd/csrc/pfr_elementwise.hip
+++ b/pets-face-recognition_amd/csrc/pfr_elementwise.hip
@@ -1155,6 +1155,30 @@
 }
 
 template <typename T>
+__device__ __forceinline__ void pool_gather2x2(const u32x4 (&gv)[4], const uint64_t (&pk)[4], const bool (&ok)[4], u32x4 (&gz)[4]) {
+  constexpr int KP = DT<T>::KPACK;
+  float g[4][KP];
+#pragma unroll
+  for (int q = 0; q < 4; ++q) Chunk<T>::unpack(gv[q], g[q]);
+  constexpr int NWIN[4] = {1, 2, 2, 4};
+  constexpr int WIN[4][4] = {{0, 0, 0, 0}, {1, 0, 0, 0}, {2, 0, 0, 0}, {3, 2, 1, 0}};
+  constexpr int TAP[4][4] = {{4, 0, 0, 0}, {3, 5, 0, 0}, {1, 7, 0, 0}, {0, 2, 6, 8}};
+#pragma unroll
+  for (int px = 0; px < 4; ++px) {
+    float acc[KP];
+#pragma unroll
+    for (int e = 0; e < KP; ++e) acc[e] = 0.f;
+#pragma unroll
+    for (int k = 0; k < NWIN[px]; ++k) {
+      const int q = WIN[px][k], tap = TAP[px][k];
+#pragma unroll
+      for (int e = 0; e < KP; ++e) acc[e] += (ok[q] && (int)((pk[q] >> (8 * e)) & 0xff) == tap) ? g[q][e] : 0.f;
+    }
+    gz[px] = Chunk<T>::pack(acc);
+  }
+}
+
+template <typename T>
 __global__ __launch_bounds__(256) void maxpool_bwd2x2_kernel(const T* __restrict__ dy, const uint8_t* __restrict__ idx,
                                                              T* __restrict__ dz, int N, int H, int W, int C, int OH, int OW) {
   constexpr int KP = DT<T>::KPACK;
@@ -1180,25 +1204,12 @@
       if constexpr (KP == 8) pk[q] = *reinterpret_cast<const uint64_t*>(idx + o * 8);
       else pk[q] = *reinterpret_cast<const uint32_t*>(idx + o * 4);
     }
-    float g[4][KP];
-#pragma unroll
-    for (int q = 0; q < 4; ++q) Chunk<T>::unpack(gv[q], g[q]);
-    constexpr int NWIN[4] = {1, 2, 2, 4};
-    constexpr int WIN[4][4] = {{0, 0, 0, 0}, {1, 0, 0, 0}, {2, 0, 0, 0}, {3, 2, 1, 0}};
-    constexpr int TAP[4][4] = {{4, 0, 0, 0}, {3, 5, 0, 0}, {1, 7, 0, 0}, {0, 2, 6, 8}};
+    u32x4 gz[4];
+    pool_gather2x2<T>(gv, pk, ok, gz);
 #pragma unroll
     for (int px = 0; px < 4; ++px) {
-      float acc[KP];
-#pragma unroll
-      for (int e = 0; e < KP; ++e) acc[e] = 0.f;
-#pragma unroll
-      for (int k = 0; k < NWIN[px]; ++k) {
-        const int q = WIN[px][k], tap = TAP[px][k];
-#pragma unroll
-        for (int e = 0; e < KP; ++e) acc[e] += (ok[q] && (int)((pk[q] >> (8 * e)) & 0xff) == tap) ? g[q][e] : 0.f;
-      }
       const size_t o = (((size_t)n * H + 2 * a + (px >> 1)) * W + 2 * b + (px & 1)) * cpr + cc;
-      st16(dz + o * KP, Chunk<T>::pack(acc));
+      st16(dz + o * KP, gz[px]);
     }
   }
 }
@@ -1229,6 +1240,199 @@
   return PFR_OK;
 }
 
+template <typename T>
+struct PoolBlk {
+  u32x4 gv[4], vx[4];
+  uint64_t pk[4];
+  bool ok[4];
+  size_t xo;
+};
+__device__ __forceinline__ size_t pool_px_off(int px, int W, int C) { return ((size_t)(px >> 1) * W + (px & 1)) * C; }
+template <typename T>
+__device__ __forceinline__ void pool_blk_load(PoolBlk<T>& p, unsigned r, const T* __restrict__ dy, const uint8_t* __restrict__ idx,
+                                              const T* __restrict__ x, int H, int W, int C, int cpr, int cglob) {
+  constexpr int KP = DT<T>::KPACK;
+  const unsigned H2 = H >> 1, W2 = W >> 1;
+  const unsigned b = r % W2, t = r / W2, a = t % H2, n = t / H2;
+#pragma unroll
+  for (int q = 0; q < 4; ++q) {
+    const unsigned oh = a + (q >> 1), ow = b + (q & 1);
+    p.ok[q] = oh < H2 && ow < W2;
+    const size_t o = (((size_t)n * H2 + min(oh, H2 - 1)) * W2 + min(ow, W2 - 1)) * cpr + cglob;
+    p.gv[q] = ld16(dy + o * KP);
+    if constexpr (KP == 8) p.pk[q] = *reinterpret_cast<const uint64_t*>(idx + o * 8);
+    else p.pk[q] = *reinterpret_cast<const uint32_t*>(idx + o * 4);
+  }
+  p.xo = (((size_t)n * H + 2 * a) * W + 2 * b) * C + (size_t)cglob * KP;
+#pragma unroll
+  for (int px = 0; px < 4; ++px) p.vx[px] = ld16_nt(x + p.xo + pool_px_off(px, W, C));
+}
+
+template <typename T, int UB>
+__global__ __launch_bounds__(256) void bn_bwd_reduce_pool_kernel(const T* __restrict__ dy, const uint8_t* __restrict__ idx,
+                                                                 const T* __restrict__ x, const float* __restrict__ mean,
+                                                                 const float* __restrict__ invstd, const float* __restrict__ scale,
+                                                                 const float* __restrict__ shift, float* __restrict__ part,
+                                                                 unsigned nblk, int H, int W, int C, int cw, int rl, int cpr) {
+  constexpr int KP = DT<T>::KPACK;
+  extern __shared__ __attribute__((aligned(16))) float lds[];
+  const int col = threadIdx.x % cw, rlane = threadIdx.x / cw;
+  const int cglob = blockIdx.y * cw + col;
+  float v[2][KP];
+#pragma unroll
+  for (int e = 0; e < KP; ++e) { v[0][e] = 0.f; v[1][e] = 0.f; }
+  if (cglob < cpr) {
+    float mu[KP], is[KP], sc[KP], sh[KP];
+#pragma unroll
+    for (int e = 0; e < KP; ++e) {
+      mu[e] = mean[cglob * KP + e];
+      is[e] = invstd[cglob * KP + e];
+      sc[e] = scale[cglob * KP + e];
+      sh[e] = shift[cglob * KP + e];
+    }
+    auto body = [&](const PoolBlk<T>& p) {
+      u32x4 gz[4];
+      pool_gather2x2<T>(p.gv, p.pk, p.ok, gz);
+#pragma unroll
+      for (int px = 0; px < 4; ++px) {
+        float g[KP], xv[KP];
+        Chunk<T>::unpack(gz[px], g);
+        Chunk<T>::unpack(p.vx[px], xv);
+#pragma unroll
+        for (int e = 0; e < KP; ++e) {
+          const float gg = fmaf(xv[e], sc[e], sh[e]) > 0.f ? g[e] : 0.f;
+          v[0][e] += gg;
+          v[1][e] = fmaf(gg, (xv[e] - mu[e]) * is[e], v[1][e]);
+        }
+      }
+    };
+    const unsigned step = gridDim.x * rl;
+    unsigned r = blockIdx.x * rl + rlane;
+    for (; r + (UB - 1) * step < nblk; r += UB * step) {
+      PoolBlk<T> p[UB];
+#pragma unroll
+      for (int u = 0; u < UB; ++u) pool_blk_load<T>(p[u], r + u * step, dy, idx, x, H, W, C, cpr, cglob);
+      __builtin_amdgcn_sched_barrier(0);
+#pragma unroll
+      for (int u = 0; u < UB; ++u) body(p[u]);
+    }
+    for (; r < nblk; r += step) {
+      PoolBlk<T> p;
+      pool_blk_load<T>(p, r, dy, idx, x, H, W, C, cpr, cglob);
+      body(p);
+    }
+  }
+  col_block_reduce<2, KP>(v, lds, cw, rl, col, rlane, cglob, cpr, part + (size_t)blockIdx.x * 2 * C, C);
+}
+
+template <typename T, int UB>
+__global__ __launch_bounds__(256) void bn_bwd_apply_pool_kernel(const T* __restrict__ dy, const uint8_t* __restrict__ idx,
+                                                                const T* __restrict__ x, const float* __restrict__ coef,
+                                                                const float* __restrict__ scale, const float* __restrict__ shift,
+                                                                T* __restrict__ dx, unsigned nblk, int H, int W, int C, int cw, int rl,
+                                                                int cpr) {
+  constexpr int KP = DT<T>::KPACK;
+  const int col = threadIdx.x % cw, rlane = threadIdx.x / cw;
+  const int cglob = blockIdx.y * cw + col;
+  if (cglob >= cpr) return;
+  float cg[KP], cx[KP], c0[KP], sc[KP], sh[KP];
+#pragma unroll
+  for (int e = 0; e < KP; ++e) {
+    const int c = cglob * KP + e;
+    cg[e] = coef[c];
+    cx[e] = coef[C + c];
+    c0[e] = coef[2 * C + c];
+    sc[e] = scale[c];
+    sh[e] = shift[c];
+  }
+  auto body = [&](const PoolBlk<T>& p) {
+    u32x4 gz[4];
+    pool_gather2x2<T>(p.gv, p.pk, p.ok, gz);
+#pragma unroll
+    for (int px = 0; px < 4; ++px) {
+      float g[KP], xv[KP];
+      Chunk<T>::unpack(gz[px], g);
+      Chunk<T>::unpack(p.vx[px], xv);
+#pragma unroll
+      for (int e = 0; e < KP; ++e) {
+        const float gg = fmaf(xv[e], sc[e], sh[e]) > 0.f ? g[e] : 0.f;
+        xv[e] = fmaf(cg[e], gg, fmaf(cx[e], xv[e], c0[e]));
+      }
+      st16(dx + p.xo + pool_px_off(px, W, C), Chunk<T>::pack(xv));
+    }
+  };
+  const unsigned step = gridDim.x * rl;
+  unsigned r = blockIdx.x * rl + rlane;
+  for (; r + (UB - 1) * step < nblk; r += UB * step) {
+    PoolBlk<T> p[UB];
+#pragma unroll
+    for (int u = 0; u < UB; ++u) pool_blk_load<T>(p[u], r + u * step, dy, idx, x, H, W, C, cpr, cglob);
+    __builtin_amdgcn_sched_barrier(0);
+#pragma unroll
+    for (int u = 0; u < UB; ++u) body(p[u]);
+  }
+  for (; r < nblk; r += step) {
+    PoolBlk<T> p;
+    pool_blk_load<T>(p, r, dy, idx, x, H, W, C, cpr, cglob);
+    body(p);
+  }
+}
+
+static bool pool_fused_geom(int dtype, int N, int H, int W, int C, int target, ColGeom* g, unsigned* nblk) {
+  const int kp = dtype == PFR_BF16 ? 8 : 4;
+  if (N <= 0 || H <= 0 || W <= 0 || C <= 0 || (H & 1) || (W & 1) || C % kp) return false;
+  const size_t nb = (size_t)N * (H / 2) * (W / 2);
+  if (nb * 2 >= 0x7fffffffull) return false;
+  *nblk = (unsigned)nb;
+  *g = col_geom(C, kp, nb, (size_t)target);
+  return true;
+}
+static int pool_fused_ub() { return pfr_knob(KNOB_BNPOOL_UB) == 2 ? 2 : 1; }
+
+extern "C" int pfr_bn_bwd_pool_blocks(int C, int dtype, int N, int H, int W) {
+  ColGeom g;
+  unsigned nblk;
+  return pool_fused_geom(dtype, N, H, W, C, pfr_knob(KNOB_BNPOOL_RGRID), &g, &nblk) ? g.gx : 0;
+}
+
+extern "C" int pfr_bn_bwd_reduce_pool(const void* dpool, const uint8_t* idx, const void* x, const float* mean, const float* invstd,
+                                      const float* scale, const float* shift, int dtype, int N, int H, int W, int C, float* part,
+                                      hipStream_t st) {
+  PFR_CHECK_ARG(dpool && idx && x && mean && invstd && scale && shift && part, "pfr_bn_bwd_reduce_pool: null pointer");
+  ColGeom g;
+  unsigned nblk;
+  PFR_CHECK_ARG(pool_fused_geom(dtype, N, H, W, C, pfr_knob(KNOB_BNPOOL_RGRID), &g, &nblk),
+                "pfr_bn_bwd_reduce_pool: needs even H, W and C %% (16 bytes) == 0 (got %d x %d x %d x %d)", N, H, W, C);
+  const size_t shb = (size_t)256 * 2 * (dtype == PFR_BF16 ? 8 : 4) * sizeof(float);
+#define PFR_BNRP(TT, U) hipLaunchKernelGGL((bn_bwd_reduce_pool_kernel<TT, U>), dim3(g.gx, g.gy), dim3(256), shb, st, (const TT*)dpool, idx, (const TT*)x, mean, invstd, scale, shift, part, nblk, H, W, C, g.cw, g.rl, g.cpr)
+  if (dtype == PFR_BF16) { if (pool_fused_ub() == 1) PFR_BNRP(bf16_t, 1); else PFR_BNRP(bf16_t, 2); }
+  else { if (pool_fused_ub() == 1) PFR_BNRP(float, 1); else PFR_BNRP(float, 2); }
+#undef PFR_BNRP
+  PFR_CHECK_LAUNCH();
+  return PFR_OK;
+}
+
+extern "C" int pfr_bn_bwd_apply_pool(const void* dpool, const uint8_t* idx, const void* x, const float* coef, const float* scale,
+                                     const float* shift, void* dx, int dtype, int N, int H, int W, int C, hipStream_t st) {
+  PFR_CHECK_ARG(dpool && idx && x && coef && scale && shift && dx, "pfr_bn_bwd_apply_pool: null pointer");
+  PFR_CHECK_ARG(dx != dpool && dx != x, "pfr_bn_bwd_apply_pool: dx must not alias an input (neighbouring blocks read the same dpool values)");
+  ColGeom g;
+  unsigned nblk;
+  PFR_CHECK_ARG(pool_fused_geom(dtype, N, H, W, C, pfr_knob(KNOB_BNPOOL_AGRID), &g, &nblk),
+                "pfr_bn_bwd_apply_pool: needs even H, W and C %% (16 bytes) == 0 (got %d x %d x %d x %d)", N, H, W, C);
+  hipEvent_t stop = pfr_tls_stop_event;
+  pfr_tls_stop_event = nullptr;
+#define PFR_BNAP(TT, U)                                                                                                                       \
+  do {                                                                                                                                        \
+    if (stop) hipExtLaunchKernelGGL((bn_bwd_apply_pool_kernel<TT, U>), dim3(g.gx, g.gy), dim3(256), 0, st, nullptr, stop, 0, (const TT*)dpool, idx, (const TT*)x, coef, scale, shift, (TT*)dx, nblk, H, W, C, g.cw, g.rl, g.cpr); \
+    else hipLaunchKernelGGL((bn_bwd_apply_pool_kernel<TT, U>), dim3(g.gx, g.gy), dim3(256), 0, st, (const TT*)dpool, idx, (const TT*)x, coef, scale, shift, (TT*)dx, nblk, H, W, C, g.cw, g.rl, g.cpr); \
+  } while (0)
+  if (dtype == PFR_BF16) { if (pool_fused_ub() == 1) PFR_BNAP(bf16_t, 1); else PFR_BNAP(bf16_t, 2); }
+  else { if (pool_fused_ub() == 1) PFR_BNAP(float, 1); else PFR_BNAP(float, 2); }
+#undef PFR_BNAP
+  PFR_CHECK_LAUNCH();
+  return PFR_OK;
+}
 
 template <typename T>
 __global__ void avgpool_fwd_kernel(const T* __restrict__ x, T* __restrict__ y, int N, int HW, int C) {
diff --git a/pets-face-recognition_amd/csrc/pfr_plan.hip b/pets-face-recognition_amd/csrc/pfr_plan.hip
--- a/pets-face-recognition_amd/csrc/pfr_plan.hip
+++ b/pets-face-recognition_amd/csrc/pfr_plan.hip
@@ -76,13 +76,14 @@
   hipStream_t ms = (hipStream_t)main_stream, ss = (hipStream_t)side_stream;
   const bool use_side = ss != nullptr;
   static const int apply_thunk = pfr_plan_thunk_index("pfr_bn_bwd_apply");
+  static const int apply_pool_thunk = pfr_plan_thunk_index("pfr_bn_bwd_apply_pool");
   int attached = -1;
   for (int i = begin; i < end; ++i) {
     const PlanOp& op = p->ops[i];
     switch (op.kind) {
       case 0:
       case 1: {
-        if (op.kind == 0 && use_side && op.thunk == apply_thunk && i + 1 < end && p->ops[i + 1].kind == 2) {
+        if (op.kind == 0 && use_side && (op.thunk == apply_thunk || op.thunk == apply_pool_thunk) && i + 1 < end && p->ops[i + 1].kind == 2) {
           pfr_tls_stop_event = p->events[p->ops[i + 1].ev];
           attached = i + 1;
         }
diff --git a/pets-face-recognition_amd/csrc/pfr_thunks_gen.inc b/pets-face-recognition_amd/csrc/pfr_thunks_gen.inc
--- a/pets-face-recognition_amd/csrc/pfr_thunks_gen.inc
+++ b/pets-face-recognition_amd/csrc/pfr_thunks_gen.inc
@@ -34,6 +34,8 @@
 static int th_pfr_bn_bwd_apply(const unsigned long long* a, void* st) { return pfr_bn_bwd_apply((const void*)(uintptr_t)a[0], (const void*)(uintptr_t)a[1], (const void*)(uintptr_t)a[2], (const float*)(uintptr_t)a[3], (const float*)(uintptr_t)a[4], (const float*)(uintptr_t)a[5], (int)(long long)a[6], (void*)(uintptr_t)a[7], (void*)(uintptr_t)a[8], (int)(long long)a[9], (long)(long long)a[10], (int)(long long)a[11], (hipStream_t)st); }
 static int th_pfr_bn_relu_maxpool_fwd(const unsigned long long* a, void* st) { return pfr_bn_relu_maxpool_fwd((const void*)(uintptr_t)a[0], (const float*)(uintptr_t)a[1], (const float*)(uintptr_t)a[2], (void*)(uintptr_t)a[3], (uint8_t*)(uintptr_t)a[4], (int)(long long)a[5], (int)(long long)a[6], (int)(long long)a[7], (int)(long long)a[8], (int)(long long)a[9], (int)(long long)a[10], (hipStream_t)st); }
 static int th_pfr_maxpool_bwd(const unsigned long long* a, void* st) { return pfr_maxpool_bwd((const void*)(uintptr_t)a[0], (const uint8_t*)(uintptr_t)a[1], (void*)(uintptr_t)a[2], (int)(long long)a[3], (int)(long long)a[4], (int)(long long)a[5], (int)(long long)a[6], (int)(long long)a[7], (hipStream_t)st); }
+static int th_pfr_bn_bwd_reduce_pool(const unsigned long long* a, void* st) { return pfr_bn_bwd_reduce_pool((const void*)(uintptr_t)a[0], (const uint8_t*)(uintptr_t)a[1], (const void*)(uintptr_t)a[2], (const float*)(uintptr_t)a[3], (const float*)(uintptr_t)a[4], (const float*)(uintptr_t)a[5], (const float*)(uintptr_t)a[6], (int)(long long)a[7], (int)(long long)a[8], (int)(long long)a[9], (int)(long long)a[10], (int)(long long)a[11], (float*)(uintptr_t)a[12], (hipStream_t)st); }
+static int th_pfr_bn_bwd_apply_pool(const unsigned long long* a, void* st) { return pfr_bn_bwd_apply_pool((const void*)(uintptr_t)a[0], (const uint8_t*)(uintptr_t)a[1], (const void*)(uintptr_t)a[2], (const float*)(uintptr_t)a[3], (const float*)(uintptr_t)a[4], (const float*)(uintptr_t)a[5], (void*)(uintptr_t)a[6], (int)(long long)a[7], (int)(long long)a[8], (int)(long long)a[9], (int)(long long)a[10], (int)(long long)a[11], (hipStream_t)st); }
 static int th_pfr_avgpool_fwd(const unsigned long long* a, void* st) { return pfr_avgpool_fwd((const void*)(uintptr_t)a[0], (void*)(uintptr_t)a[1], (int)(long long)a[2], (int)(long long)a[3], (int)(long long)a[4], (int)(long long)a[5], (hipStream_t)st); }
 static int th_pfr_avgpool_bwd(const unsigned long long* a, void* st) { return pfr_avgpool_bwd((const void*)(uintptr_t)a[0], (void*)(uintptr_t)a[1], (int)(long long)a[2], (int)(long long)a[3], (int)(long long)a[4], (int)(long long)a[5], (hipStream_t)st); }
 static int th_pfr_s2d_input(const unsigned long long* a, void* st) { return pfr_s2d_input((const float*)(uintptr_t)a[0], (void*)(uintptr_t)a[1], (int)(long long)a[2], (int)(long long)a[3], (int)(long long)a[4], (int)(long long)a[5], (int)(long long)a[6], (int)(long long)a[7], (hipStream_t)st); }
@@ -118,6 +120,8 @@
   {"pfr_bn_bwd_apply", th_pfr_bn_bwd_apply},
   {"pfr_bn_relu_maxpool_fwd", th_pfr_bn_relu_maxpool_fwd},
   {"pfr_maxpool_bwd", th_pfr_maxpool_bwd},
+  {"pfr_bn_bwd_reduce_pool", th_pfr_bn_bwd_reduce_pool},
+  {"pfr_bn_bwd_apply_pool", th_pfr_bn_bwd_apply_pool},
   {"pfr_avgpool_fwd", th_pfr_avgpool_fwd},
   {"pfr_avgpool_bwd", th_pfr_avgpool_bwd},
   {"pfr_s2d_input", th_pfr_s2d_input},
diff --git a/pets-face-recognition_amd/models/_fe_engine.py b/pets-face-recognition_amd/models/_fe_engine.py
--- a/pets-face-recognition_amd/models/_fe_engine.py
+++ b/pets-face-recognition_amd/models/_fe_engine.py
@@ -102,6 +102,7 @@
         lib.pfr_set_tuning(b"bnb", self.fuse_bnb)
         self._tuning_epoch = lib.pfr_tuning_epoch()
         self._bnb_min_rows = 0
+        self.fuse_pool = os.environ.get("PFR_FUSE_POOL", "1") != "0" and self.dtype == torch.bfloat16
         self.bnfree = os.environ.get("PFR_BNFREE", "1") != "0" and self.dtype == torch.bfloat16 and self.fuse_bnb == 2
         self.gram_stats = os.environ.get("PFR_BNFREE_GRAMSTATS", "1") != "0"
         self.gram_flag = torch.zeros(1, dtype=torch.int32).pin_memory()
@@ -897,9 +898,25 @@
             dcur = dxin
         c1, s1, idx, pshape = saved["stem"]
         dz = G(s1)
-        ops.append((lib.pfr_maxpool_bwd, (dcur.data_ptr(), idx.data_ptr(), dz.data_ptr(), self.did, N, s1[1], s1[2], s1[3])))
-        release(dcur)
-        bn_bwd(dz, None, c1, s1, stbn, 2, dz, None, acc)
+        npool = lib.pfr_bn_bwd_pool_blocks(s1[3], self.did, N, s1[1], s1[2]) if self.fuse_pool else 0
+        plan.meta["stem_pool_fused"] = npool > 0
+        if npool > 0:
+            part = G((npool, 2, s1[3]), torch.float32)
+            ops.append((lib.pfr_bn_bwd_reduce_pool, (dcur.data_ptr(), idx.data_ptr(), c1.data_ptr(), stbn.coef[0].data_ptr(),
+                                                     stbn.coef[1].data_ptr(), stbn.coef[2].data_ptr(), stbn.coef[3].data_ptr(),
+                                                     self.did, N, s1[1], s1[2], s1[3], part.data_ptr())))
+            ops.append((lib.pfr_bn_bwd_finalize, (part.data_ptr(), npool, s1[3], float(N * s1[1] * s1[2]), stbn.gamma.data_ptr(),
+                                                  stbn.coef[0].data_ptr(), stbn.coef[1].data_ptr(), stbn.dgamma.data_ptr(),
+                                                  stbn.dbeta.data_ptr(), stbn.bcoef.data_ptr(), acc)))
+            ops.append((lib.pfr_bn_bwd_apply_pool, (dcur.data_ptr(), idx.data_ptr(), c1.data_ptr(), stbn.bcoef.data_ptr(),
+                                                    stbn.coef[2].data_ptr(), stbn.coef[3].data_ptr(), dz.data_ptr(), self.did,
+                                                    N, s1[1], s1[2], s1[3])))
+            release(part)
+            release(dcur)
+        else:
+            ops.append((lib.pfr_maxpool_bwd, (dcur.data_ptr(), idx.data_ptr(), dz.data_ptr(), self.did, N, s1[1], s1[2], s1[3])))
+            release(dcur)
+            bn_bwd(dz, None, c1, s1, stbn, 2, dz, None, acc)
         if use_s2d:
             wgrad(x_nhwc, xin_shape, dz, s1, self.s2d, out=self.s2d.g)
             ops.append(("wait", (nside[0] - 1,)))
```
